# Lcrypto/mod-interleaveavx_multithreads-FAID

Hardware: AMD Instinct MI355X
Metric: decoded Gb/s @ 10 iters, 50G-PON LDPC; FER match vs AVX512 ref (higher is better)
Workload: dtype i8

## Files before the change

### include/lnsfaid.h

```cpp
#ifndef LNSFAID_H
#define LNSFAID_H

#include <stddef.h>
#include <stdint.h>

#ifdef __cplusplus
extern "C" {
#endif

#define LNSFAID_GROUP 32

#define LNSFAID_OK 0
#define LNSFAID_E_INVAL (-1)
#define LNSFAID_E_CODE (-2)
#define LNSFAID_E_NOMEM (-3)
#define LNSFAID_E_HIP (-4)
#define LNSFAID_E_NODEVICE (-5)
#define LNSFAID_E_INTERNAL (-6)

typedef struct lnsfaid_code {
    int32_t n_var;
    int32_t n_check;
    int32_t n_edges;
    int32_t z;
    int32_t puncture_tail;
    int32_t nb_degres;
    const int32_t* deg;
    const int32_t* deg_rows;
    const uint16_t* pos_vn;
} lnsfaid_code;

typedef struct lnsfaid_cfg {
    int32_t decode_method;
    int32_t max_iteration;
    int32_t factor_1;
    int32_t factor_2;
    int32_t floor_err_count;
    int32_t floor_iter_thresh;
    int32_t ef_elimination;
    int32_t max_bf_iter;
    int32_t bf_L0;
    int32_t bf_L1;
    int32_t bf_alpha;
    int32_t bf_delta;
    int32_t regular_col_weight;
    int32_t hard2_threshold;
    int32_t bf_vote_cap;
    int8_t v2c_map[6][4][8];
    int8_t v2c_map_ef[6][4][8];
} lnsfaid_cfg;

typedef struct lnsfaid_group_stats {
    int32_t iterations;
    int32_t bf_iterations;
} lnsfaid_group_stats;

typedef struct lnsfaid_codeword_stats {
    int32_t iterations;
    int32_t bf_iterations;
    int32_t unsatisfied;
} lnsfaid_codeword_stats;

typedef struct lnsfaid_ctx lnsfaid_ctx;


int lnsfaid_code_50gpon(lnsfaid_code* code, uint16_t* pos_vn, int32_t* deg3, int32_t* deg_rows3);

int lnsfaid_cfg_default(lnsfaid_cfg* cfg, int32_t decode_method, int32_t max_iteration);

#define LNSFAID_TABLES_FAID3 0
#define LNSFAID_TABLES_FAID32 1
#define LNSFAID_TABLES_FAID2 2
int lnsfaid_cfg_table_preset(lnsfaid_cfg* cfg, int32_t preset);

int lnsfaid_cfg_ef_elimination(lnsfaid_cfg* cfg, int32_t mode);


int lnsfaid_create(lnsfaid_ctx** ctx, const lnsfaid_code* code, const lnsfaid_cfg* cfg,
                   int32_t device, size_t max_groups);
void lnsfaid_destroy(lnsfaid_ctx* ctx);

int lnsfaid_set_cfg(lnsfaid_ctx* ctx, const lnsfaid_cfg* cfg);


int lnsfaid_decode(lnsfaid_ctx* ctx, const int8_t* fixInput, size_t n_groups,
                   int8_t* decodedBits, lnsfaid_group_stats* stats);

int lnsfaid_decode_device(lnsfaid_ctx* ctx, const int8_t* d_fixInput, size_t n_groups,
                          int8_t* d_decodedBits, lnsfaid_group_stats* d_stats);

#define LNSFAID_STOP_GROUP 0
#define LNSFAID_STOP_CODEWORD 1
int lnsfaid_set_early_stop(lnsfaid_ctx* ctx, int32_t rule);
int lnsfaid_early_stop(const lnsfaid_ctx* ctx);
int lnsfaid_decode_codewords(lnsfaid_ctx* ctx, const int8_t* fixInput, size_t n_groups, int8_t* decodedBits,
                             lnsfaid_codeword_stats* cw_stats);
int lnsfaid_decode_codewords_device(lnsfaid_ctx* ctx, const int8_t* d_fixInput, size_t n_groups, int8_t* d_decodedBits,
                                    lnsfaid_codeword_stats* d_cw_stats);

int lnsfaid_count_errors(lnsfaid_ctx* ctx, const int8_t* decodedBits, const int8_t* inputBits,
                         size_t n_groups, uint64_t out[4]);
int lnsfaid_count_errors_device(lnsfaid_ctx* ctx, const int8_t* d_decodedBits,
                                const int8_t* d_inputBits, size_t n_groups, uint64_t out[4]);

int lnsfaid_decode_packed(lnsfaid_ctx* ctx, const uint8_t* llr4, size_t n_groups, uint32_t* bits, lnsfaid_group_stats* stats);
int lnsfaid_decode_packed_device(lnsfaid_ctx* ctx, const uint8_t* d_llr4, size_t n_groups, uint32_t* d_bits,
                                 lnsfaid_group_stats* d_stats);
int lnsfaid_decode_codewords_packed(lnsfaid_ctx* ctx, const uint8_t* llr4, size_t n_groups, uint32_t* bits,
                                    lnsfaid_codeword_stats* cw_stats);
int lnsfaid_decode_codewords_packed_device(lnsfaid_ctx* ctx, const uint8_t* d_llr4, size_t n_groups, uint32_t* d_bits,
                                           lnsfaid_codeword_stats* d_cw_stats);
int lnsfaid_count_errors_packed(lnsfaid_ctx* ctx, const uint32_t* bits, const uint8_t* msg, size_t n_groups, uint64_t out[4]);
int lnsfaid_count_errors_packed_device(lnsfaid_ctx* ctx, const uint32_t* d_bits, const uint8_t* d_msg, size_t n_groups,
                                       uint64_t out[4]);
int lnsfaid_pack_llr4(const int8_t* fixInput, size_t n_values, uint8_t* llr4);
int lnsfaid_unpack_bits(const uint32_t* bits, size_t n_bits, int8_t* decodedBits);
int lnsfaid_pack_bits(const int8_t* inputBits, size_t n_bits, uint8_t* packed);


int lnsfaid_frontend_device(lnsfaid_ctx* ctx, const uint32_t* seeds, const uint64_t* draws_before, size_t n_streams,
                            int32_t mod_type, float sigma, float scale, const int8_t* codeword, int8_t* d_fixInput);
int lnsfaid_frontend_device_states(lnsfaid_ctx* ctx, const uint32_t* states, const uint64_t* draws_before, size_t n_streams,
                                   int32_t mod_type, float sigma, float scale, const int8_t* codeword, int8_t* d_fixInput);
uint64_t lnsfaid_frontend_draws_per_group(const lnsfaid_ctx* ctx, int32_t mod_type);

int lnsfaid_frontend_set_exact(lnsfaid_ctx* ctx, int32_t exact);
int lnsfaid_frontend_fastpath_bounds(lnsfaid_ctx* ctx, double measured[2], double assumed[2]);

int lnsfaid_frontend_set_interleave(lnsfaid_ctx* ctx, int32_t interleave_mod_type);

int lnsfaid_frontend_set_frames(lnsfaid_ctx* ctx, const int8_t* outputBits, const int8_t* inputBits, size_t n_streams);
int lnsfaid_frontend_input_bits(lnsfaid_ctx* ctx, const int8_t** d_inputBits);

int lnsfaid_demap_device(lnsfaid_ctx* ctx, const float* d_rx, size_t n_groups, int32_t mod_type, float scale, int8_t* d_fixInput);
int lnsfaid_demap_packed_device(lnsfaid_ctx* ctx, const float* d_rx, size_t n_groups, int32_t mod_type, float scale, uint8_t* d_llr4);
int lnsfaid_demap_host(int32_t n_var, int32_t n_check, int32_t interleave_mod_type, const float* rx, size_t n_groups,
                       int32_t mod_type, float scale, int8_t* fixInput);
int lnsfaid_demap_packed_host(int32_t n_var, int32_t n_check, int32_t interleave_mod_type, const float* rx, size_t n_groups,
                              int32_t mod_type, float scale, uint8_t* llr4);


int lnsfaid_code_parity_inverse(const lnsfaid_code* code, uint8_t* circ, size_t bytes);

int lnsfaid_encode_device(lnsfaid_ctx* ctx, const int8_t* d_inputBits, size_t n_groups, int8_t* d_outputBits);
int lnsfaid_encode(lnsfaid_ctx* ctx, const int8_t* inputBits, size_t n_groups, int8_t* outputBits);

int lnsfaid_frontend_random_frames(lnsfaid_ctx* ctx, const uint64_t* keys, size_t n_streams);

int lnsfaid_io_buffers(lnsfaid_ctx* ctx, int8_t** d_fixInput, int8_t** d_decodedBits, lnsfaid_group_stats** d_stats);

int lnsfaid_host_register(void* ptr, size_t bytes);
int lnsfaid_host_unregister(void* ptr);

int lnsfaid_read_stats(lnsfaid_ctx* ctx, lnsfaid_group_stats* stats, size_t n_groups);

#define LNSFAID_COMM_ID_BYTES 128
int lnsfaid_comm_unique_id(uint8_t id[LNSFAID_COMM_ID_BYTES]);
int lnsfaid_comm_init(lnsfaid_ctx* ctx, int32_t n_ranks, int32_t rank, const uint8_t id[LNSFAID_COMM_ID_BYTES]);
int lnsfaid_comm_attach(lnsfaid_ctx* ctx, void* nccl_comm);
int lnsfaid_comm_destroy(lnsfaid_ctx* ctx);
int lnsfaid_allreduce_counters(lnsfaid_ctx* ctx, uint64_t counters[4]);

int lnsfaid_select_kernel(lnsfaid_ctx* ctx, int32_t rows_per_lane);
int lnsfaid_kernel_rows_per_lane(const lnsfaid_ctx* ctx);

int lnsfaid_select_waves(lnsfaid_ctx* ctx, int32_t waves_per_codeword);
int lnsfaid_kernel_waves(const lnsfaid_ctx* ctx);

#define LNSFAID_MSG_REGISTERS 1
#define LNSFAID_MSG_HBM 2
int lnsfaid_select_message_store(lnsfaid_ctx* ctx, int32_t where);
int lnsfaid_message_store(const lnsfaid_ctx* ctx);

int lnsfaid_kernel_residency(lnsfaid_ctx* ctx, int32_t* workgroups_per_cu, int32_t* lds_limit);


int lnsfaid_kernel_time(lnsfaid_ctx* ctx, double* out_ms, uint64_t* out_launches, int32_t reset);

void* lnsfaid_stream(lnsfaid_ctx* ctx);

const char* lnsfaid_strerror(int err);
const char* lnsfaid_last_hip_error(void);
const char* lnsfaid_version(void);

#ifdef __cplusplus
}
#endif
#endif
```

### mod-interleaveavx_multithreads-faid_amd/csrc/lnsfaid_capi.hip

```cpp
#include <hip/hip_runtime.h>

#include <dlfcn.h>
#include <rccl/rccl.h>

#include <cstdio>
#include <cstdlib>
#include <cstring>
#include <new>
#include <vector>

#include "lnsfaid_device.h"
#include "lnsfaid_quantise.h"
#include "lnsfaid_swar.h"

extern "C" hipError_t lf_launch_decode(int method, int uniform_w, const LfKernelArgs* args, size_t lds_bytes,
                                       hipStream_t stream);
extern "C" const void* lf_decode_func(int method, int uniform_w);
extern "C" int lf_decode_threads(void);
extern "C" const void* lf_decode4_func(int method, int ef, int rm);
extern "C" int lf_decode4_threads(void);
extern "C" hipError_t lf_launch_decode4(int method, int ef, int rm, const LfKernelArgs* args, size_t lds_bytes, hipStream_t stream);
extern "C" int lf_decode4_rm_layers(void);
extern "C" const void* lf_decode4cw_func(int method, int ef, int rm);
extern "C" hipError_t lf_launch_decode4cw(int method, int ef, int rm, const LfCwArgs* args, size_t lds_bytes, hipStream_t stream);
extern "C" const void* lf_decode4p_func(int method, int ef, int rm, int per_codeword);
extern "C" hipError_t lf_launch_decode4p(int method, int ef, int rm, const LfKernelArgs* args, size_t lds_bytes, hipStream_t stream);
extern "C" hipError_t lf_launch_decode4pcw(int method, int ef, int rm, const LfCwArgs* args, size_t lds_bytes, hipStream_t stream);
extern "C" hipError_t lf_launch_unpack_llr4(const uint8_t* d_llr4, int8_t* d_fix, size_t n_values, hipStream_t stream);
extern "C" hipError_t lf_launch_pack_bits(const int8_t* d_decoded, uint32_t* d_bits, size_t n_values, hipStream_t stream);
extern "C" hipError_t lf_launch_count_errors_packed(const uint32_t* d_bits, const uint32_t* d_msg, int n_var, int k_info, size_t n_cw,
                                                    unsigned long long* out, hipStream_t stream);
extern "C" const void* lf_decode5_func(int method);
extern "C" int lf_decode5_threads(void);
extern "C" hipError_t lf_launch_decode5(int method, const LfKernelArgs* args, size_t lds_bytes, hipStream_t stream);
extern "C" hipError_t lf_launch_count_errors(const int8_t* decoded, const int8_t* input_bits, int n_var, int k_info,
                                             size_t n_cw, unsigned long long* out, hipStream_t stream);

extern "C" hipError_t lf_launch_frontend(const uint32_t* d_seeds, const unsigned long long* d_draws, int n_streams, int mod_type,
                                         float sigma_ch, float scale, const int8_t* d_codeword, const int8_t* d_frames, int n_var,
                                         int n_check, int interleave, int fast, int8_t* d_fix, hipStream_t stream);
extern "C" hipError_t lf_launch_demap(const float* d_rx, size_t n_groups, int mod_type, float scale, int n_var, int n_check,
                                      int interleave, int packed, void* d_out, hipStream_t stream);
extern "C" hipError_t lf_frontend_fastpath_scan(double* d_out2, hipStream_t stream);
extern "C" void lf_frontend_fastpath_assumed(double* eps2);
extern "C" hipError_t lf_launch_encode(const LfDevCode* d_code, int n_check, const uint32_t* d_bsup, const uint32_t* d_bsup_off,
                                       const int8_t* d_in, const unsigned long long* d_keys, size_t n_groups, int8_t* d_out,
                                       int8_t* d_info, hipStream_t stream);

#include <atomic>
#include <chrono>
#include <condition_variable>
#include <mutex>
#include <thread>
struct LfCombiner;
static thread_local char g_hip_err[256] = "";
static std::atomic<int> g_live_contexts(0);
#define LF_SPIN_CONTEXTS 4
static bool sync_blocking()
{
    static const char* e = getenv("LNSFAID_SYNC");
    if (e && e[0] == 's') return false;
    if (e && e[0] == 'b') return true;
    return g_live_contexts.load(std::memory_order_relaxed) > LF_SPIN_CONTEXTS;
}

static int hip_fail(hipError_t e, const char* what)
{
    snprintf(g_hip_err, sizeof(g_hip_err), "%s: %s", what, hipGetErrorString(e));
    return LNSFAID_E_HIP;
}
#define HIP_TRY(call)                                      \
    do {                                                   \
        hipError_t e_ = (call);                            \
        if (e_ != hipSuccess) return hip_fail(e_, #call);  \
    } while (0)

#define LF_IO_CHUNKS 8
#define LF_MAX_CHAIN 6

struct lnsfaid_ctx {
    int device = 0;
    size_t max_groups = 0;
    LfDevCode hcode;
    LfDevCfg hcfg;
    int n_var = 0, n_check = 0, k_info = 0;
    size_t lds_bytes = 0;
    hipStream_t stream = nullptr;
    hipEvent_t ev0 = nullptr, ev1 = nullptr;
    hipEvent_t ev_chain[LF_MAX_CHAIN + 1] = {};
    hipEvent_t ev_block = nullptr;
    uint32_t slot_seen[LF_MAX_CHAIN] = {};
    int predicted_launches = 1;
    hipStream_t s_in = nullptr, s_out = nullptr;
    hipEvent_t ev_in[LF_IO_CHUNKS] = {};
    LfDevCode* d_code = nullptr;
    LfDevCfg* d_cfg = nullptr;
    int8_t* d_en = nullptr;
    uint4* d_rows = nullptr;
    uint32_t* d_bits = nullptr;
    LfLaneState* d_lane = nullptr;
    int32_t* d_status[2] = { nullptr, nullptr };
    uint32_t* d_remaining = nullptr;
    int32_t* d_live = nullptr;
    unsigned long long* d_counters = nullptr;
    uint32_t* h_remaining = nullptr;
    unsigned long long* h_counters = nullptr;
    int8_t* d_io_in = nullptr;
    int8_t* d_io_out = nullptr;
    lnsfaid_group_stats* d_io_stats = nullptr;
    lnsfaid_codeword_stats* d_io_cw_stats = nullptr;
    uint8_t* d_pk_in = nullptr;
    uint32_t* d_pk_out = nullptr;
    lnsfaid_group_stats* d_pk_stats = nullptr;
    int early_stop = LNSFAID_STOP_GROUP;
    int rows_per_lane = 0;
    int waves_per_cw = 0;
    int msg_store = 0;
    struct LfCombiner* comb = nullptr;
    int comb_slot = -1;
    const void* checked_fn[4] = {};
    int resident_wg[4] = {}, lds_wg[4] = {};
    void* comm = nullptr;
    bool comm_owned = false;
    unsigned long long* d_reduce = nullptr;
    double kernel_ms = 0.0;
    uint64_t kernel_launches = 0;
    uint32_t* d_fe_seeds = nullptr;
    unsigned long long* d_fe_draws = nullptr;
    int8_t* d_fe_codeword = nullptr;
    int8_t* d_fe_frames = nullptr;
    int8_t* d_fe_input = nullptr;
    size_t fe_frames_streams = 0;
    int fe_interleave = 1;
    int fe_exact = 0;
    int enc_state = 0;
    uint32_t* d_enc_sup = nullptr;
    uint32_t* d_enc_off = nullptr;
    unsigned long long* d_fe_keys = nullptr;
};

static int stream_wait(lnsfaid_ctx* ctx)
{
    if (sync_blocking()) {
        HIP_TRY(hipEventRecord(ctx->ev_block, ctx->stream));
        HIP_TRY(hipEventSynchronize(ctx->ev_block));
    } else {
        HIP_TRY(hipStreamSynchronize(ctx->stream));
    }
    return LNSFAID_OK;
}

static int weight_class(int w) { return w == 3 ? 0 : (w == 6 ? 1 : (w == 11 ? 2 : 3)); }

static int build_code(const lnsfaid_code* code, LfDevCode* out)
{
    memset(out, 0, sizeof(*out));
    if (!code || !code->pos_vn || !code->deg || !code->deg_rows) return LNSFAID_E_INVAL;
    const int Z = code->z, N = code->n_var, M = code->n_check, E = code->n_edges;
    if (Z != LF_Z) return LNSFAID_E_CODE;
    if (N <= 0 || M <= 0 || N % Z || M % Z || M >= N) return LNSFAID_E_CODE;
    const int nbr = M / Z, nbc = N / Z, K = N - M;
    if (nbr > LF_MAX_BR || nbc > LF_MAX_BC) return LNSFAID_E_CODE;
    if (K % 4 || M % 4 || N % LF_T) return LNSFAID_E_CODE;
    if (code->puncture_tail < 0 || code->puncture_tail > N) return LNSFAID_E_CODE;
    std::vector<int> row_deg;
    row_deg.reserve(M);
    long e_total = 0;
    for (int k = 0; k < code->nb_degres; ++k) {
        if (code->deg_rows[k] < 0 || code->deg[k] < 2 || code->deg[k] > LF_MAX_DEG) return LNSFAID_E_CODE;
        for (int i = 0; i < code->deg_rows[k]; ++i) { row_deg.push_back(code->deg[k]); e_total += code->deg[k]; }
    }
    if ((int)row_deg.size() != M || e_total != E) return LNSFAID_E_CODE;

    size_t e = 0;
    for (int br = 0; br < nbr; ++br) {
        const int deg = row_deg[(size_t)br * Z];
        out->deg[br] = deg;
        const uint16_t* row0 = code->pos_vn + e;
        for (int j = 0; j < 64; ++j) out->sbtab[br][j] = 0u;
        for (int j = 0; j < 32; ++j) out->sbplain[br][j] = 0u;
        int prev_cb = -1;
        for (int j = 0; j < deg; ++j) {
            const int cb = row0[j] / Z, sh = row0[j] % Z;
            if (row0[j] >= N || cb <= prev_cb) return LNSFAID_E_CODE;
            prev_cb = cb;
            out->circ[br][j].sb = (uint32_t)cb * (uint32_t)Z + (uint32_t)sh;
            out->sbtab[br][LF_JCODE_A(j)] = out->sbtab[br][LF_JCODE_B(j)] = out->circ[br][j].sb;
            out->sbplain[br][j] = (((uint32_t)cb * (uint32_t)Z) << 16) | (((uint32_t)sh) << 2);
            out->s4tab[br][j] = ((uint32_t)sh) << 2;
            out->cbtab[br][j] = (uint32_t)cb * (uint32_t)Z;
            if (out->col_weight[cb] >= LF_MAX_COLW) return LNSFAID_E_CODE;
            out->colcirc[cb][out->col_weight[cb]++] = (uint32_t)br | ((uint32_t)sh << 8);
        }
        for (int i = 0; i < Z; ++i) {
            if (row_deg[(size_t)br * Z + i] != deg) return LNSFAID_E_CODE;
            for (int j = 0; j < deg; ++j) {
                const uint32_t sb = out->circ[br][j].sb;
                const int want = (int)(sb / (uint32_t)Z * (uint32_t)Z + (sb % (uint32_t)Z + (uint32_t)i) % (uint32_t)Z);
                if (code->pos_vn[e + (size_t)i * deg + j] != want) return LNSFAID_E_CODE;
            }
        }
        e += (size_t)deg * Z;
    }
    {
        const int nw = N / 32, pw = M / 32;
        const uint32_t hard0 = lf_lds_off_hard(N), zero = lf_lds_off_zero(N, nw, pw);
        if (lf_lds_bytes(N, nw, pw) > 0xffffu) return LNSFAID_E_CODE;
        for (int br = 0; br < LF_MAX_BR; ++br)
            for (int j = 0; j < LF_MAX_DEG; ++j)
                for (int k = 0; k < 8; ++k) {
                    uint2 e; e.x = zero | (zero << 16); e.y = 0;
                    if (br < nbr && j < out->deg[br]) {
                        const uint32_t sb = out->circ[br][j].sb, cb = sb / (uint32_t)Z, sh = sb % (uint32_t)Z;
                        const uint32_t o = (32u * (uint32_t)k + sh) & 255u, q = o >> 5;
                        e.x = (hard0 + 4u * (cb * 8u + q)) | ((hard0 + 4u * (cb * 8u + ((q + 1u) & 7u))) << 16);
                        e.y = o & 31u;
                    }
                    out->synw[br][j][k] = e;
                }
    }
    for (int br = 0; br < nbr; ++br)
        for (int j = 0; j < out->deg[br]; ++j)
            out->circ[br][j].wclass = (uint32_t)weight_class(out->col_weight[out->circ[br][j].sb / (uint32_t)Z]);
    out->n_var = N; out->n_check = M; out->k_info = K; out->nbr = nbr; out->nbc = nbc;
    out->puncture_tail = code->puncture_tail;
    out->n_words = N / 32; out->p_words = M / 32;
    return LNSFAID_OK;
}

static void build_wcols(LfDevCode* code, int W)
{
    code->n_wcols = 0;
    for (int cb = 0; cb < code->nbc; ++cb)
        if (code->col_weight[cb] == W) code->wcol[code->n_wcols++] = cb;
    bool seen[LF_MAX_BC] = {};
    for (int br = 0; br < LF_MAX_BR; ++br) {
        code->era_edges[br] = 0;
        for (int j = 0; br < code->nbr && j < code->deg[br]; ++j) {
            const int cb = (int)(code->circ[br][j].sb / LF_Z);
            if (code->col_weight[cb] == W && !seen[cb]) { seen[cb] = true; code->era_edges[br] |= 1u << j; }
        }
    }
}

static int build_cfg(const lnsfaid_cfg* cfg, LfDevCfg* out)
{
    if (!cfg) return LNSFAID_E_INVAL;
    if (cfg->decode_method < 0 || cfg->decode_method > 5) return LNSFAID_E_INVAL;
    if (cfg->max_iteration < 0 || cfg->max_iteration > (1 << 20)) return LNSFAID_E_INVAL;
    if (cfg->max_bf_iter < 0 || cfg->max_bf_iter > (1 << 20)) return LNSFAID_E_INVAL;
    if (cfg->regular_col_weight < 0 || cfg->regular_col_weight > LF_MAX_COLW) return LNSFAID_E_INVAL;
    memset(out, 0, sizeof(*out));
    out->method = cfg->decode_method;
    out->max_iter = cfg->max_iteration;
    out->factor_1 = cfg->decode_method == 0 ? (int16_t)cfg->factor_1 : (int8_t)cfg->factor_1;
    out->factor_2 = cfg->decode_method == 0 ? (int16_t)cfg->factor_2 : (int8_t)cfg->factor_2;
    out->floor_err_count = cfg->floor_err_count;
    out->floor_iter_thresh = cfg->floor_iter_thresh;
    out->ef = cfg->ef_elimination;
    out->max_bf = (cfg->decode_method == 0 || cfg->decode_method == 1) ? 0 : cfg->max_bf_iter;
    out->L0 = cfg->bf_L0; out->L1 = cfg->bf_L1; out->alpha = cfg->bf_alpha; out->delta = cfg->bf_delta;
    out->W = cfg->regular_col_weight;
    out->hard2_thr = cfg->hard2_threshold;
    out->vote_cap = (int8_t)cfg->bf_vote_cap;
    if ((cfg->decode_method == 1 || cfg->decode_method == 3 || cfg->decode_method == 4)
        && ((int8_t)cfg->factor_1 < 0 || (int8_t)cfg->factor_2 < 1)) return LNSFAID_E_INVAL;
    if (cfg->decode_method == 5 && cfg->ef_elimination != 1) return LNSFAID_E_INVAL;
    if (cfg->decode_method == 2 && (cfg->ef_elimination < 0 || cfg->ef_elimination > 2)) return LNSFAID_E_INVAL;
    if (cfg->decode_method != 2 && cfg->decode_method != 5 && cfg->ef_elimination != 0) return LNSFAID_E_INVAL;
    out->uniform_w = 1;
    for (int it = 0; it < 6; ++it)
        for (int w = 0; w < 4; ++w) {
            for (int a = 0; a < 8; ++a) {
                const int v = cfg->v2c_map[it][w][a], ve = cfg->v2c_map_ef[it][w][a];
                if ((cfg->decode_method == 2 || cfg->decode_method == 5) && (v < 0 || v > 7)) return LNSFAID_E_INVAL;
                if ((cfg->decode_method == 5 || cfg->ef_elimination >= 1) && (ve < 0 || ve > 7)) return LNSFAID_E_INVAL;
                uint32_t* l = a < 4 ? &out->lut_lo[it][w] : &out->lut_hi[it][w];
                uint32_t* le = a < 4 ? &out->lut_ef_lo[it][w] : &out->lut_ef_hi[it][w];
                *l |= (uint32_t)(v & 0xff) << (8 * (a & 3));
                *le |= (uint32_t)(ve & 0xff) << (8 * (a & 3));
                if (a > 0 && (v < cfg->v2c_map[it][w][a - 1] || ((cfg->decode_method == 5 || cfg->ef_elimination >= 1) && ve < cfg->v2c_map_ef[it][w][a - 1])))
                    out->uniform_w = 0;
            }
            if (out->lut_lo[it][w] != out->lut_lo[it][0] || out->lut_hi[it][w] != out->lut_hi[it][0]) out->uniform_w = 0;
            if ((cfg->decode_method == 5 || cfg->ef_elimination >= 1)
                && (out->lut_ef_lo[it][w] != out->lut_ef_lo[it][0] || out->lut_ef_hi[it][w] != out->lut_ef_hi[it][0]))
                out->uniform_w = 0;
        }
    if (cfg->decode_method == 0) {
        out->uniform_w = (out->factor_1 == out->factor_2) ? 1 : 0;
        out->nms_fits = sw_nms_fits(out->factor_1, out->factor_2) ? 1 : 0;
        if (out->nms_fits) sw_nms_tables(out->factor_1, out->nms_t);
    }
    if (cfg->decode_method == 2 && cfg->ef_elimination >= 1 && !out->uniform_w) return LNSFAID_E_INVAL;
    out->bf_fast = (out->W == 3 && ((int8_t)out->alpha == 0 || (int8_t)out->alpha == 1)) ? 1 : 0;
    return LNSFAID_OK;
}

static int check_code_for_method(const LfDevCode* code, int method)
{
    if (method == 3)
        for (int cb = 0; cb < code->nbc; ++cb)
            if (code->col_weight[cb] > 15) return LNSFAID_E_CODE;
    return LNSFAID_OK;
}

extern "C" int lnsfaid_comm_destroy(lnsfaid_ctx* ctx);
static int comb_join(lnsfaid_ctx* ctx);
static void comb_leave(lnsfaid_ctx* ctx, int slot);
extern "C" void lnsfaid_destroy(lnsfaid_ctx* ctx)
{
    if (!ctx) return;
    if (ctx->comb_slot >= 0) { comb_leave(ctx, ctx->comb_slot); ctx->comb_slot = -1; }
    g_live_contexts.fetch_sub(1, std::memory_order_relaxed);
    (void)hipSetDevice(ctx->device);
    if (ctx->stream) (void)hipStreamSynchronize(ctx->stream);
    (void)lnsfaid_comm_destroy(ctx);
    (void)hipFree(ctx->d_reduce);
    (void)hipFree(ctx->d_code); (void)hipFree(ctx->d_cfg); (void)hipFree(ctx->d_en); (void)hipFree(ctx->d_rows);
    (void)hipFree(ctx->d_bits); (void)hipFree(ctx->d_lane); (void)hipFree(ctx->d_status[0]); (void)hipFree(ctx->d_status[1]);
    (void)hipFree(ctx->d_remaining); (void)hipFree(ctx->d_live); (void)hipFree(ctx->d_counters);
    (void)hipFree(ctx->d_io_in); (void)hipFree(ctx->d_io_out); (void)hipFree(ctx->d_io_stats);
    (void)hipFree(ctx->d_io_cw_stats);
    (void)hipFree(ctx->d_pk_in); (void)hipFree(ctx->d_pk_out); (void)hipFree(ctx->d_pk_stats);
    (void)hipFree(ctx->d_fe_seeds); (void)hipFree(ctx->d_fe_draws); (void)hipFree(ctx->d_fe_codeword);
    (void)hipFree(ctx->d_fe_frames); (void)hipFree(ctx->d_fe_input);
    (void)hipFree(ctx->d_enc_sup); (void)hipFree(ctx->d_enc_off); (void)hipFree(ctx->d_fe_keys);
    if (ctx->h_remaining) (void)hipHostFree(ctx->h_remaining);
    if (ctx->h_counters) (void)hipHostFree(ctx->h_counters);
    if (ctx->ev0) (void)hipEventDestroy(ctx->ev0);
    if (ctx->ev1) (void)hipEventDestroy(ctx->ev1);
    for (auto e : ctx->ev_chain) if (e) (void)hipEventDestroy(e);
    if (ctx->ev_block) (void)hipEventDestroy(ctx->ev_block);
    if (ctx->stream) (void)hipStreamDestroy(ctx->stream);
    if (ctx->s_in) (void)hipStreamDestroy(ctx->s_in);
    if (ctx->s_out) (void)hipStreamDestroy(ctx->s_out);
    for (auto e : ctx->ev_in) if (e) (void)hipEventDestroy(e);
    delete ctx;
}

static int alloc_state(lnsfaid_ctx* ctx);
static int create_impl(lnsfaid_ctx* ctx, const lnsfaid_code* code, const lnsfaid_cfg* cfg)
{
    int rc = build_code(code, &ctx->hcode);
    if (rc) return rc;
    rc = build_cfg(cfg, &ctx->hcfg);
    if (rc) return rc;
    ctx->n_var = ctx->hcode.n_var; ctx->n_check = ctx->hcode.n_check; ctx->k_info = ctx->hcode.k_info;
    rc = check_code_for_method(&ctx->hcode, ctx->hcfg.method);
    if (rc) return rc;
    build_wcols(&ctx->hcode, ctx->hcfg.W);
    return alloc_state(ctx);
}

static int alloc_state(lnsfaid_ctx* ctx)
{
    ctx->n_var = ctx->hcode.n_var; ctx->n_check = ctx->hcode.n_check; ctx->k_info = ctx->hcode.k_info;
    ctx->lds_bytes = lf_lds_bytes(ctx->n_var, ctx->hcode.n_words, ctx->hcode.p_words);
    if (ctx->lds_bytes > 64 * 1024) return LNSFAID_E_CODE;

    int ndev = 0;
    if (hipGetDeviceCount(&ndev) != hipSuccess || ndev <= 0 || ctx->device < 0 || ctx->device >= ndev) {
        snprintf(g_hip_err, sizeof(g_hip_err), "no usable HIP device (count %d, asked for %d)", ndev, ctx->device);
        return LNSFAID_E_NODEVICE;
    }
    HIP_TRY(hipSetDevice(ctx->device));
    HIP_TRY(hipStreamCreateWithFlags(&ctx->stream, hipStreamNonBlocking));
    HIP_TRY(hipEventCreate(&ctx->ev0));
    HIP_TRY(hipEventCreate(&ctx->ev1));
    const size_t n_cw = ctx->max_groups * LNSFAID_GROUP;
    HIP_TRY(hipMalloc(&ctx->d_code, sizeof(LfDevCode)));
    HIP_TRY(hipMalloc(&ctx->d_cfg, sizeof(LfDevCfg)));
    HIP_TRY(hipMalloc(&ctx->d_en, n_cw * (size_t)ctx->n_var));
    HIP_TRY(hipMalloc(&ctx->d_rows, n_cw * (size_t)ctx->hcode.nbr * LF_T * sizeof(uint4)));
    HIP_TRY(hipMalloc(&ctx->d_bits, n_cw * (size_t)3 * ctx->hcode.n_words * sizeof(uint32_t)));
    HIP_TRY(hipMalloc(&ctx->d_lane, n_cw * sizeof(LfLaneState)));
    HIP_TRY(hipMalloc(&ctx->d_status[0], n_cw * sizeof(int32_t)));
    HIP_TRY(hipMalloc(&ctx->d_status[1], n_cw * sizeof(int32_t)));
    HIP_TRY(hipMalloc(&ctx->d_remaining, LF_MAX_CHAIN * sizeof(uint32_t)));
    HIP_TRY(hipMemset(ctx->d_remaining, 0, LF_MAX_CHAIN * sizeof(uint32_t)));
    for (auto& e : ctx->ev_chain) HIP_TRY(hipEventCreate(&e));
    HIP_TRY(hipEventCreateWithFlags(&ctx->ev_block, hipEventBlockingSync | hipEventDisableTiming));
    HIP_TRY(hipMalloc(&ctx->d_live, n_cw * sizeof(int32_t)));
    HIP_TRY(hipMalloc(&ctx->d_counters, 4 * sizeof(unsigned long long)));
    HIP_TRY(hipHostMalloc((void**)&ctx->h_remaining, LF_MAX_CHAIN * sizeof(uint32_t), hipHostMallocDefault));
    HIP_TRY(hipHostMalloc((void**)&ctx->h_counters, 4 * sizeof(unsigned long long), hipHostMallocDefault));
    HIP_TRY(hipMemcpy(ctx->d_code, &ctx->hcode, sizeof(LfDevCode), hipMemcpyHostToDevice));
    HIP_TRY(hipMemcpy(ctx->d_cfg, &ctx->hcfg, sizeof(LfDevCfg), hipMemcpyHostToDevice));
    return LNSFAID_OK;
}

extern "C" int lnsfaid_create(lnsfaid_ctx** out, const lnsfaid_code* code, const lnsfaid_cfg* cfg, int32_t device,
                              size_t max_groups)
{
    if (!out || !code || !cfg || max_groups == 0 || max_groups > ((size_t)1 << 24)) return LNSFAID_E_INVAL;
    *out = nullptr;
    lnsfaid_ctx* ctx = new (std::nothrow) lnsfaid_ctx();
    if (!ctx) return LNSFAID_E_NOMEM;
    ctx->device = device;
    ctx->max_groups = max_groups;
    if (const char* e = getenv("LNSFAID_ROWS_PER_LANE"))
        ctx->rows_per_lane = (e[0] == '2') ? 2 : 0;
    if (const char* e = getenv("LNSFAID_WAVES_PER_CODEWORD"))
        ctx->waves_per_cw = (e[0] == '2') ? 2 : 0;
    if (const char* e = getenv("LNSFAID_FRONTEND_EXACT"))
        ctx->fe_exact = (e[0] == '1') ? 1 : 0;
    if (const char* e = getenv("LNSFAID_MSG_STORE"))
        ctx->msg_store = (e[0] == 'h') ? LNSFAID_MSG_HBM : ((e[0] == 'r') ? LNSFAID_MSG_REGISTERS : 0);
    g_live_contexts.fetch_add(1, std::memory_order_relaxed);
    const int rc = create_impl(ctx, code, cfg);
    if (rc) { lnsfaid_destroy(ctx); return rc; }
    ctx->comb_slot = comb_join(ctx);
    *out = ctx;
    return LNSFAID_OK;
}

extern "C" int lnsfaid_set_cfg(lnsfaid_ctx* ctx, const lnsfaid_cfg* cfg)
{
    if (!ctx || !cfg) return LNSFAID_E_INVAL;
    LfDevCfg n;
    int rc = build_cfg(cfg, &n);
    if (rc) return rc;
    rc = check_code_for_method(&ctx->hcode, n.method);
    if (rc) return rc;
    if (memcmp(&n, &ctx->hcfg, sizeof(n)) == 0) return LNSFAID_OK;
    HIP_TRY(hipSetDevice(ctx->device));
    HIP_TRY(hipStreamSynchronize(ctx->stream));
    if (n.W != ctx->hcfg.W) {
        build_wcols(&ctx->hcode, n.W);
        HIP_TRY(hipMemcpy(ctx->d_code, &ctx->hcode, sizeof(LfDevCode), hipMemcpyHostToDevice));
    }
    ctx->hcfg = n;
    HIP_TRY(hipMemcpy(ctx->d_cfg, &ctx->hcfg, sizeof(LfDevCfg), hipMemcpyHostToDevice));
    return LNSFAID_OK;
}

static void apply_devcfg(lnsfaid_ctx* ctx, const LfDevCfg& n)
{
    (void)hipStreamSynchronize(ctx->stream);
    ctx->hcfg = n;
    (void)hipMemcpy(ctx->d_cfg, &ctx->hcfg, sizeof(LfDevCfg), hipMemcpyHostToDevice);
}

static bool kernel4_possible(const lnsfaid_ctx* ctx)
{
    const int m = ctx->hcfg.method;
    if (m < 0 || m > 5) return false;
    if (m == 0) return ctx->hcfg.nms_fits != 0;
    if ((m == 2 || m == 5) && !ctx->hcfg.uniform_w) return false;
    return true;
}
static bool use_kernel4(const lnsfaid_ctx* ctx)
{
    if (ctx->hcfg.method == 2 && ctx->hcfg.ef >= 1) return true;
    if (ctx->rows_per_lane == 2) return false;
    return kernel4_possible(ctx);
}

extern "C" int lnsfaid_select_kernel(lnsfaid_ctx* ctx, int32_t rows_per_lane)
{
    if (!ctx || (rows_per_lane != 0 && rows_per_lane != 2 && rows_per_lane != 4)) return LNSFAID_E_INVAL;
    if (rows_per_lane == 4 && !kernel4_possible(ctx)) return LNSFAID_E_INVAL;
    if (rows_per_lane == 2 && ctx->hcfg.method == 2 && ctx->hcfg.ef >= 1) return LNSFAID_E_INVAL;
    ctx->rows_per_lane = rows_per_lane;
    return LNSFAID_OK;
}

extern "C" int lnsfaid_kernel_rows_per_lane(const lnsfaid_ctx* ctx) { return ctx ? (use_kernel4(ctx) ? 4 : 2) : LNSFAID_E_INVAL; }

static bool kernel5_possible(const lnsfaid_ctx* ctx)
{
    const int m = ctx->hcfg.method;
    return kernel4_possible(ctx) && m >= 1 && m <= 5 && !(m == 2 && ctx->hcfg.ef == 2) && ctx->hcode.n_words >= 7 * 64;
}
static bool use_kernel5(const lnsfaid_ctx* ctx) { return ctx->waves_per_cw == 2 && use_kernel4(ctx) && kernel5_possible(ctx); }

extern "C" int lnsfaid_select_waves(lnsfaid_ctx* ctx, int32_t waves_per_codeword)
{
    if (!ctx || waves_per_codeword < 0 || waves_per_codeword > 2) return LNSFAID_E_INVAL;
    if (waves_per_codeword == 2 && !(use_kernel4(ctx) && kernel5_possible(ctx))) return LNSFAID_E_INVAL;
    ctx->waves_per_cw = waves_per_codeword;
    return LNSFAID_OK;
}

extern "C" int lnsfaid_kernel_waves(const lnsfaid_ctx* ctx) { return ctx ? (use_kernel5(ctx) ? 2 : 1) : LNSFAID_E_INVAL; }

static bool msg_registers_possible(const lnsfaid_ctx* ctx)
{
    if (ctx->hcfg.method == 0) return false;
    return ctx->hcode.nbr <= lf_decode4_rm_layers() && !(ctx->hcfg.method == 2 && ctx->hcfg.ef == 2);
}
static bool use_msg_registers(const lnsfaid_ctx* ctx)
{
    if (!msg_registers_possible(ctx) || use_kernel5(ctx)) return false;
    return ctx->msg_store != LNSFAID_MSG_HBM;
}

static bool cw_possible(const lnsfaid_ctx* ctx) { return ctx->waves_per_cw != 2 && use_kernel4(ctx); }

static bool packed_kernel(const lnsfaid_ctx* ctx) { return use_kernel4(ctx) && !use_kernel5(ctx); }

static const void* selected_kernel(const lnsfaid_ctx* ctx, int* threads, int rule, bool packed = false)
{
    if (packed) {
        *threads = lf_decode4_threads();
        return lf_decode4p_func(ctx->hcfg.method, ctx->hcfg.ef, use_msg_registers(ctx) ? 1 : 0, rule == LNSFAID_STOP_CODEWORD ? 1 : 0);
    }
    if (rule == LNSFAID_STOP_CODEWORD) {
        *threads = lf_decode4_threads();
        return cw_possible(ctx) ? lf_decode4cw_func(ctx->hcfg.method, ctx->hcfg.ef, use_msg_registers(ctx) ? 1 : 0) : nullptr;
    }
    if (use_kernel5(ctx)) {
        *threads = lf_decode5_threads();
        return lf_decode5_func(ctx->hcfg.method);
    }
    if (use_kernel4(ctx)) {
        *threads = lf_decode4_threads();
        return lf_decode4_func(ctx->hcfg.method, ctx->hcfg.ef, use_msg_registers(ctx) ? 1 : 0);
    }
    *threads = lf_decode_threads();
    return lf_decode_func(ctx->hcfg.method, ctx->hcfg.uniform_w);
}

extern "C" int lnsfaid_select_message_store(lnsfaid_ctx* ctx, int32_t where)
{
    if (!ctx || where < 0 || where > LNSFAID_MSG_HBM) return LNSFAID_E_INVAL;
    if (where == LNSFAID_MSG_REGISTERS && !msg_registers_possible(ctx)) return LNSFAID_E_INVAL;
    ctx->msg_store = where;
    return LNSFAID_OK;
}

extern "C" int lnsfaid_message_store(const lnsfaid_ctx* ctx)
{
    if (!ctx) return LNSFAID_E_INVAL;
    if (!use_kernel4(ctx)) return LNSFAID_MSG_HBM;
    return use_msg_registers(ctx) ? LNSFAID_MSG_REGISTERS : LNSFAID_MSG_HBM;
}

static int kernel_check(lnsfaid_ctx* ctx, int rule, bool packed = false)
{
    int threads = 0;
    const void* fn = selected_kernel(ctx, &threads, rule, packed);
    if (!fn) return rule == LNSFAID_STOP_CODEWORD ? LNSFAID_E_INVAL : LNSFAID_E_INTERNAL;
    const int slot = rule + (packed ? 2 : 0);
    if (fn == ctx->checked_fn[slot]) return LNSFAID_OK;
    hipFuncAttributes at;
    HIP_TRY(hipFuncGetAttributes(&at, fn));
    if (at.sharedSizeBytes != 0) {
        snprintf(g_hip_err, sizeof(g_hip_err), "decode kernel has %zu bytes of static LDS: its En image would not start at LDS offset 0",
                 (size_t)at.sharedSizeBytes);
        return LNSFAID_E_INTERNAL;
    }
    int wg = 0;
    HIP_TRY(hipOccupancyMaxActiveBlocksPerMultiprocessor(&wg, fn, threads, ctx->lds_bytes));
    hipDeviceProp_t prop;
    HIP_TRY(hipGetDeviceProperties(&prop, ctx->device));
    const size_t lds_cu = prop.maxSharedMemoryPerMultiProcessor ? prop.maxSharedMemoryPerMultiProcessor : 160 * 1024;
    const size_t gran = 512;
    int by_lds = (int)(lds_cu / ((ctx->lds_bytes + gran - 1) / gran * gran));
    const int by_waves = 32 / ((threads + 63) / 64);
    if (by_lds > by_waves) by_lds = by_waves;
    ctx->checked_fn[slot] = fn; ctx->resident_wg[slot] = wg; ctx->lds_wg[slot] = by_lds;
    static const bool trace = getenv("LNSFAID_TRACE") != nullptr;
    if (trace)
        fprintf(stderr, "[lnsfaid] decode kernel: %d threads, %d VGPRs, %zu B LDS per workgroup, %d workgroups per CU (LDS alone: %d)%s\n",
                threads, at.numRegs, ctx->lds_bytes, wg, by_lds, wg < by_lds ? "  ** residency lost **" : "");
    return LNSFAID_OK;
}

extern "C" int lnsfaid_kernel_residency(lnsfaid_ctx* ctx, int32_t* workgroups_per_cu, int32_t* lds_limit)
{
    if (!ctx) return LNSFAID_E_INVAL;
    HIP_TRY(hipSetDevice(ctx->device));
    const int rc = kernel_check(ctx, ctx->early_stop);
    if (rc) return rc;
    if (workgroups_per_cu) *workgroups_per_cu = ctx->resident_wg[ctx->early_stop];
    if (lds_limit) *lds_limit = ctx->lds_wg[ctx->early_stop];
    return LNSFAID_OK;
}

static int decode_device_impl(lnsfaid_ctx* ctx, const int8_t* d_fixInput, size_t n_groups, int8_t* d_decodedBits,
                              lnsfaid_group_stats* d_stats, bool status_preloaded, bool packed = false);
static int decode_cw_device_impl(lnsfaid_ctx* ctx, const int8_t* d_fixInput, size_t n_groups, int8_t* d_decodedBits,
                                 lnsfaid_group_stats* d_stats, lnsfaid_codeword_stats* d_cw_stats, bool status_preloaded,
                                 bool packed = false);
static int decode_device_rule(lnsfaid_ctx* ctx, const int8_t* d_fixInput, size_t n_groups, int8_t* d_decodedBits, lnsfaid_group_stats* d_stats,
                              lnsfaid_codeword_stats* d_cw_stats, int rule, bool status_preloaded)
{
    if (rule == LNSFAID_STOP_CODEWORD)
        return decode_cw_device_impl(ctx, d_fixInput, n_groups, d_decodedBits, d_stats, d_cw_stats, status_preloaded);
    return decode_device_impl(ctx, d_fixInput, n_groups, d_decodedBits, d_stats, status_preloaded);
}
extern "C" int lnsfaid_decode_device(lnsfaid_ctx* ctx, const int8_t* d_fixInput, size_t n_groups, int8_t* d_decodedBits,
                                     lnsfaid_group_stats* d_stats)
{
    if (!ctx) return LNSFAID_E_INVAL;
    return decode_device_rule(ctx, d_fixInput, n_groups, d_decodedBits, d_stats, nullptr, ctx->early_stop, false);
}
extern "C" int lnsfaid_decode_codewords_device(lnsfaid_ctx* ctx, const int8_t* d_fixInput, size_t n_groups, int8_t* d_decodedBits,
                                               lnsfaid_codeword_stats* d_cw_stats)
{
    return decode_cw_device_impl(ctx, d_fixInput, n_groups, d_decodedBits, nullptr, d_cw_stats, false);
}

extern "C" int lnsfaid_set_early_stop(lnsfaid_ctx* ctx, int32_t rule)
{
    if (!ctx || (rule != LNSFAID_STOP_GROUP && rule != LNSFAID_STOP_CODEWORD)) return LNSFAID_E_INVAL;
    ctx->early_stop = rule;
    return LNSFAID_OK;
}
extern "C" int lnsfaid_early_stop(const lnsfaid_ctx* ctx) { return ctx ? ctx->early_stop : LNSFAID_E_INVAL; }

static int decode_cw_device_impl(lnsfaid_ctx* ctx, const int8_t* d_fixInput, size_t n_groups, int8_t* d_decodedBits,
                                 lnsfaid_group_stats* d_stats, lnsfaid_codeword_stats* d_cw_stats, bool status_preloaded, bool packed)
{
    if (!ctx || (n_groups && (!d_fixInput || !d_decodedBits))) return LNSFAID_E_INVAL;
    if (n_groups > ctx->max_groups) return LNSFAID_E_INVAL;
    if (!cw_possible(ctx)) return LNSFAID_E_INVAL;
    if (n_groups == 0) return LNSFAID_OK;
    HIP_TRY(hipSetDevice(ctx->device));
    {
        const int rc = kernel_check(ctx, LNSFAID_STOP_CODEWORD, packed);
        if (rc) return rc;
    }
    const size_t n_cw = n_groups * LNSFAID_GROUP;
    LfCwArgs a;
    a.code = ctx->d_code; a.cfg = ctx->d_cfg;
    a.fix_input = d_fixInput; a.decoded = d_decodedBits;
    a.st_rows = ctx->d_rows;
    a.skip = status_preloaded ? ctx->d_status[0] : nullptr;
    a.stats = d_stats; a.cw_stats = d_cw_stats; a.n_cw = (int32_t)n_cw;
    if (d_stats) HIP_TRY(hipMemsetAsync(d_stats, 0, n_groups * sizeof(lnsfaid_group_stats), ctx->stream));
    static const bool trace = getenv("LNSFAID_TRACE") != nullptr;
    HIP_TRY(hipEventRecord(ctx->ev_chain[0], ctx->stream));
    if (packed) HIP_TRY(lf_launch_decode4pcw(ctx->hcfg.method, ctx->hcfg.ef, use_msg_registers(ctx) ? 1 : 0, &a, ctx->lds_bytes, ctx->stream));
    else HIP_TRY(lf_launch_decode4cw(ctx->hcfg.method, ctx->hcfg.ef, use_msg_registers(ctx) ? 1 : 0, &a, ctx->lds_bytes, ctx->stream));
    HIP_TRY(hipEventRecord(ctx->ev_chain[1], ctx->stream));
    { const int rcw = stream_wait(ctx); if (rcw) return rcw; }
    float ms = 0.f;
    HIP_TRY(hipEventElapsedTime(&ms, ctx->ev_chain[0], ctx->ev_chain[1]));
    ctx->kernel_ms += ms;
    ctx->kernel_launches += 1;
    if (trace) fprintf(stderr, "[lnsfaid] per-codeword launch: %.3f ms, %zu codewords\n", ms, n_cw);
    return LNSFAID_OK;
}

static int decode_device_impl(lnsfaid_ctx* ctx, const int8_t* d_fixInput, size_t n_groups, int8_t* d_decodedBits,
                              lnsfaid_group_stats* d_stats, bool status_preloaded, bool packed)
{
    if (!ctx || (n_groups && (!d_fixInput || !d_decodedBits))) return LNSFAID_E_INVAL;
    if (n_groups > ctx->max_groups) return LNSFAID_E_INVAL;
    if (n_groups == 0) return LNSFAID_OK;
    HIP_TRY(hipSetDevice(ctx->device));
    {
        const int rc = kernel_check(ctx, LNSFAID_STOP_GROUP, packed);
        if (rc) return rc;
    }
    const size_t n_cw = n_groups * LNSFAID_GROUP;
#ifdef LF4_LIVE_PROOF
    HIP_TRY(hipMemsetAsync(ctx->d_live, 0, n_cw * sizeof(int32_t), ctx->stream));
#endif

    LfKernelArgs a;
    a.code = ctx->d_code; a.cfg = ctx->d_cfg;
    a.fix_input = d_fixInput; a.decoded = d_decodedBits;
    a.st_en = ctx->d_en; a.st_rows = ctx->d_rows; a.st_bits = ctx->d_bits; a.st_lane = ctx->d_lane;
    a.live = ctx->d_live; a.stats = d_stats; a.n_cw = (int32_t)n_cw;

    const long max_launches = 2L * ((long)ctx->hcfg.max_iter + ctx->hcfg.max_bf + 2) + 2 + LF_MAX_CHAIN;
    static const bool trace = getenv("LNSFAID_TRACE") != nullptr;
    int cur = 0;
    long launch = 0, needed = 0;
    bool done = false;
    while (!done) {
        if (launch >= max_launches) return LNSFAID_E_INTERNAL;
        int chain = launch == 0 ? ctx->predicted_launches : 1;
        if (chain < 1) chain = 1;
        if (chain > LF_MAX_CHAIN) chain = LF_MAX_CHAIN;
        for (int j = 0; j < chain; ++j) {
            a.status_cur = (launch + j == 0 && !status_preloaded) ? nullptr : ctx->d_status[cur];
            a.status_next = ctx->d_status[cur ^ 1];
            a.remaining = ctx->d_remaining + j;
            HIP_TRY(hipEventRecord(ctx->ev_chain[j], ctx->stream));
            if (packed) HIP_TRY(lf_launch_decode4p(ctx->hcfg.method, ctx->hcfg.ef, use_msg_registers(ctx) ? 1 : 0, &a, ctx->lds_bytes, ctx->stream));
            else if (use_kernel5(ctx)) HIP_TRY(lf_launch_decode5(ctx->hcfg.method, &a, ctx->lds_bytes, ctx->stream));
            else if (use_kernel4(ctx)) HIP_TRY(lf_launch_decode4(ctx->hcfg.method, ctx->hcfg.ef, use_msg_registers(ctx) ? 1 : 0, &a, ctx->lds_bytes, ctx->stream));
            else HIP_TRY(lf_launch_decode(ctx->hcfg.method, ctx->hcfg.uniform_w, &a, ctx->lds_bytes, ctx->stream));
            cur ^= 1;
        }
        HIP_TRY(hipEventRecord(ctx->ev_chain[chain], ctx->stream));
        HIP_TRY(hipMemcpyAsync(ctx->h_remaining, ctx->d_remaining, (size_t)chain * sizeof(uint32_t), hipMemcpyDeviceToHost, ctx->stream));
        { const int rcw = stream_wait(ctx); if (rcw) return rcw; }
        for (int j = 0; j < chain; ++j) {
            const uint32_t left = ctx->h_remaining[j] - ctx->slot_seen[j];
            ctx->slot_seen[j] = ctx->h_remaining[j];
            float ms = 0.f;
            HIP_TRY(hipEventElapsedTime(&ms, ctx->ev_chain[j], ctx->ev_chain[j + 1]));
            ctx->kernel_ms += ms;
            ctx->kernel_launches += 1;
            if (trace) fprintf(stderr, "[lnsfaid] launch %ld: %.3f ms, %u codewords left%s\n", launch + j, ms, left, done ? " (queued ahead, batch already complete)" : "");
            if (!done && left == 0) { done = true; needed = launch + j + 1; }
        }
        launch += chain;
    }
    ctx->predicted_launches = (int)needed;
    return LNSFAID_OK;
}

static int ensure_io(lnsfaid_ctx* ctx)
{
    if (ctx->d_io_in) return LNSFAID_OK;
    const size_t bytes = ctx->max_groups * LNSFAID_GROUP * (size_t)ctx->n_var;
    HIP_TRY(hipMalloc(&ctx->d_io_in, bytes));
    HIP_TRY(hipMalloc(&ctx->d_io_out, bytes));
    HIP_TRY(hipMalloc(&ctx->d_io_stats, ctx->max_groups * sizeof(lnsfaid_group_stats)));
    return LNSFAID_OK;
}

#define LF_COMB_SLOTS 128
#define LF_COMB_QUIET_US 150
#define LF_COMB_WINDOW_US 1500
#define LF_COMB_DEVICES 16
#define LF_COMB_WORKERS 4
#define LF_COMB_MIN_MEMBERS 4
enum { LF_SLOT_FREE = 0, LF_SLOT_IDLE, LF_SLOT_PENDING, LF_SLOT_RUNNING, LF_SLOT_DONE };
struct LfSlot {
    int state = LF_SLOT_FREE;
    int rc = 0;
    LfDevCfg cfg;
    int rule = LNSFAID_STOP_GROUP;
    lnsfaid_group_stats stats;
};
struct LfCombiner {
    int device = 0;
    std::mutex m;
    std::condition_variable cv_work, cv_done;
    std::thread worker[LF_COMB_WORKERS];
    bool stop = false, dead = false;
    bool gathering = false;
    int running = 0;
    lnsfaid_ctx* pool[LF_COMB_WORKERS] = {};
    LfDevCode code;
    size_t group_bytes = 0;
    int8_t *h_in = nullptr, *h_out = nullptr;
    int8_t *d_in_map = nullptr, *d_out_map = nullptr;
    int32_t* h_status = nullptr;
    lnsfaid_group_stats* h_stats = nullptr;
    LfSlot slots[LF_COMB_SLOTS];
    int members = 0, pending = 0;
    char err[256] = "";
    uint64_t batches = 0, calls = 0;
    double gather_ms = 0, device_ms = 0;
};
static std::mutex g_comb_mutex;
static LfCombiner* g_comb[LF_COMB_DEVICES] = {};

static int comb_workers()
{
    static const int n = [] {
        const char* e = getenv("LNSFAID_COMB_WORKERS");
        const int v = e ? atoi(e) : 2;
        return v < 1 ? 1 : (v > LF_COMB_WORKERS ? LF_COMB_WORKERS : v);
    }();
    return n;
}

static int comb_batches()
{
    static const int v = [] {
        const char* e = getenv("LNSFAID_COMB_BATCHES");
        const int n = e ? atoi(e) : 0;
        return n > 64 ? 64 : n;
    }();
    return v > comb_workers() ? v : comb_workers();
}

static bool comb_enabled()
{
    static const char* e = getenv("LNSFAID_COALESCE");
    return !(e && e[0] == '0');
}

static void apply_devcfg(lnsfaid_ctx* ctx, const LfDevCfg& n);

static void comb_run_batch(LfCombiner* cb, int w, const int* batch, int nb)
{
    lnsfaid_ctx* P = cb->pool[w];
    int32_t* h_status = cb->h_status + (size_t)w * LF_COMB_SLOTS * LNSFAID_GROUP;
    lnsfaid_group_stats* h_stats = cb->h_stats + (size_t)w * LF_COMB_SLOTS;
    int rc = LNSFAID_OK;
    auto fail = [&](hipError_t e, const char* what) { if (rc == LNSFAID_OK && e != hipSuccess) rc = hip_fail(e, what); };
    int lo = LF_COMB_SLOTS, hi = -1;
    for (int i = 0; i < nb; ++i) { lo = batch[i] < lo ? batch[i] : lo; hi = batch[i] > hi ? batch[i] : hi; }
    const size_t n = (size_t)hi + 1;
    for (size_t g = 0; g < n; ++g) {
        bool active = false;
        for (int i = 0; i < nb; ++i) active = active || (size_t)batch[i] == g;
        for (int l = 0; l < LNSFAID_GROUP; ++l) h_status[g * LNSFAID_GROUP + l] = active ? 0 : LF_DONE;
    }
    fail(hipSetDevice(cb->device), "hipSetDevice");
    if (rc == LNSFAID_OK && memcmp(&P->hcfg, &cb->slots[batch[0]].cfg, sizeof(LfDevCfg)) != 0) apply_devcfg(P, cb->slots[batch[0]].cfg);
    const size_t gb = cb->group_bytes, span = (size_t)(hi - lo + 1);
    fail(hipMemcpyAsync(P->d_status[0], h_status, n * LNSFAID_GROUP * sizeof(int32_t), hipMemcpyHostToDevice, P->stream), "status upload");
    static const bool copy_mode = getenv("LNSFAID_COMB_COPY") != nullptr;
    const int8_t* k_in = cb->d_in_map;
    int8_t* k_out = cb->d_out_map;
    if (copy_mode || !k_in || !k_out) {
        fail(hipMemcpyAsync(P->d_io_in + (size_t)lo * gb, cb->h_in + (size_t)lo * gb, span * gb, hipMemcpyHostToDevice, P->stream), "fixInput upload");
        k_in = P->d_io_in; k_out = P->d_io_out;
    }
    if (rc == LNSFAID_OK) rc = decode_device_rule(P, k_in, n, k_out, P->d_io_stats, nullptr, cb->slots[batch[0]].rule, true);
    if (rc == LNSFAID_OK) {
        if (k_out == P->d_io_out)
            fail(hipMemcpyAsync(cb->h_out + (size_t)lo * gb, P->d_io_out + (size_t)lo * gb, span * gb, hipMemcpyDeviceToHost, P->stream), "decodedBits download");
        fail(hipMemcpyAsync(h_stats + lo, P->d_io_stats + lo, span * sizeof(lnsfaid_group_stats), hipMemcpyDeviceToHost, P->stream), "stats download");
        if (rc == LNSFAID_OK) rc = stream_wait(P);
    }
    std::lock_guard<std::mutex> lk(cb->m);
    if (rc != LNSFAID_OK) snprintf(cb->err, sizeof(cb->err), "%s", g_hip_err);
    for (int i = 0; i < nb; ++i) {
        LfSlot& s = cb->slots[batch[i]];
        s.rc = rc;
        s.stats = h_stats[batch[i]];
        s.state = LF_SLOT_DONE;
    }
    cb->running -= nb;
    cb->batches += 1; cb->calls += (uint64_t)nb;
    cb->cv_done.notify_all();
    cb->cv_work.notify_all();
}

static void comb_worker(LfCombiner* cb, int w)
{
    std::unique_lock<std::mutex> lk(cb->m);
    for (;;) {
        cb->cv_work.wait(lk, [&] { return cb->stop || (cb->pending > 0 && !cb->gathering); });
        if (cb->stop) break;
        cb->gathering = true;
        const auto t_first = std::chrono::steady_clock::now();
        const auto deadline = t_first + std::chrono::microseconds(LF_COMB_WINDOW_US);
        for (;;) {
            const int share = (cb->members + comb_batches() - 1) / comb_batches();
            if (cb->stop || cb->pending >= share || cb->pending + cb->running >= cb->members) break;
            const int seen = cb->pending, seen_running = cb->running;
            auto quiet = std::chrono::steady_clock::now() + std::chrono::microseconds(LF_COMB_QUIET_US);
            if (quiet > deadline) quiet = deadline;
            cb->cv_work.wait_until(lk, quiet, [&] { return cb->pending != seen || cb->running != seen_running || cb->stop; });
            if (cb->pending == seen && cb->running == seen_running) break;
        }
        if (cb->stop) { cb->gathering = false; break; }
        cb->gather_ms += std::chrono::duration<double, std::milli>(std::chrono::steady_clock::now() - t_first).count();
        int batch[LF_COMB_SLOTS], nb = 0;
        const int cap = cb->members > 8 * comb_workers() ? (cb->members + comb_batches() - 1) / comb_batches() : LF_COMB_SLOTS;
        const LfDevCfg* cfg = nullptr;
        int rule = LNSFAID_STOP_GROUP;
        for (int i = 0; i < LF_COMB_SLOTS && nb < cap; ++i) {
            LfSlot& s = cb->slots[i];
            if (s.state != LF_SLOT_PENDING) continue;
            if (!cfg) { cfg = &s.cfg; rule = s.rule; }
            if (memcmp(cfg, &s.cfg, sizeof(LfDevCfg)) != 0 || s.rule != rule) continue;
            s.state = LF_SLOT_RUNNING;
            batch[nb++] = i;
        }
        cb->pending -= nb;
        cb->running += nb;
        cb->gathering = false;
        cb->cv_work.notify_all();
        if (nb == 0) continue;
        if (!cb->pool[w]) {
            lk.unlock();
            int rc = LNSFAID_OK;
            lnsfaid_ctx* P = new (std::nothrow) lnsfaid_ctx();
            if (!P) rc = LNSFAID_E_NOMEM;
            if (!rc) {
                P->device = cb->device; P->max_groups = LF_COMB_SLOTS;
                P->hcode = cb->code; P->hcfg = cb->slots[batch[0]].cfg;
                g_live_contexts.fetch_add(1, std::memory_order_relaxed);
                rc = alloc_state(P);
                if (!rc) rc = ensure_io(P);
                if (rc) { lnsfaid_destroy(P); P = nullptr; }
            }
            lk.lock();
            if (rc) {
                cb->dead = true;
                for (int i = 0; i < nb; ++i) { cb->slots[batch[i]].rc = rc; cb->slots[batch[i]].state = LF_SLOT_DONE; }
                cb->running -= nb;
                cb->cv_done.notify_all();
                continue;
            }
            cb->pool[w] = P;
        }
        lk.unlock();
        const auto t_dev = std::chrono::steady_clock::now();
        comb_run_batch(cb, w, batch, nb);
        lk.lock();
        cb->device_ms += std::chrono::duration<double, std::milli>(std::chrono::steady_clock::now() - t_dev).count();
    }
}

static int comb_join(lnsfaid_ctx* ctx)
{
    if (!comb_enabled() || ctx->max_groups != 1 || ctx->device < 0 || ctx->device >= LF_COMB_DEVICES) return -1;
    std::lock_guard<std::mutex> g(g_comb_mutex);
    LfCombiner* cb = g_comb[ctx->device];
    if (!cb) {
        cb = new (std::nothrow) LfCombiner();
        if (!cb) return -1;
        cb->device = ctx->device;
        cb->code = ctx->hcode;
        cb->group_bytes = (size_t)LNSFAID_GROUP * (size_t)ctx->n_var;
        g_comb[ctx->device] = cb;
    }
    std::lock_guard<std::mutex> lk(cb->m);
    if (cb->dead || memcmp(&cb->code, &ctx->hcode, sizeof(LfDevCode)) != 0) return -1;
    if (cb->members >= 1 && !cb->h_in) {
        const size_t bytes = (size_t)LF_COMB_SLOTS * cb->group_bytes;
        if (hipSetDevice(cb->device) != hipSuccess
            || hipHostMalloc((void**)&cb->h_in, bytes, hipHostMallocMapped) != hipSuccess
            || hipHostMalloc((void**)&cb->h_out, bytes, hipHostMallocMapped) != hipSuccess
            || hipHostMalloc((void**)&cb->h_status, (size_t)LF_COMB_WORKERS * LF_COMB_SLOTS * LNSFAID_GROUP * sizeof(int32_t), hipHostMallocDefault) != hipSuccess
            || hipHostMalloc((void**)&cb->h_stats, (size_t)LF_COMB_WORKERS * LF_COMB_SLOTS * sizeof(lnsfaid_group_stats), hipHostMallocDefault) != hipSuccess) {
            (void)hipGetLastError();
            if (cb->h_in) (void)hipHostFree(cb->h_in);
            if (cb->h_out) (void)hipHostFree(cb->h_out);
            if (cb->h_status) (void)hipHostFree(cb->h_status);
            if (cb->h_stats) (void)hipHostFree(cb->h_stats);
            cb->h_in = cb->h_out = nullptr; cb->h_status = nullptr; cb->h_stats = nullptr;
            cb->dead = true;
            return -1;
        }
        if (hipHostGetDevicePointer((void**)&cb->d_in_map, cb->h_in, 0) != hipSuccess
            || hipHostGetDevicePointer((void**)&cb->d_out_map, cb->h_out, 0) != hipSuccess) {
            (void)hipGetLastError();
            cb->d_in_map = cb->d_out_map = nullptr;
        }
        for (int w = 0; w < comb_workers(); ++w) cb->worker[w] = std::thread(comb_worker, cb, w);
    }
    for (int i = 0; i < LF_COMB_SLOTS; ++i)
        if (cb->slots[i].state == LF_SLOT_FREE) { cb->slots[i].state = LF_SLOT_IDLE; cb->members += 1; ctx->comb = cb; return i; }
    return -1;
}

static void comb_leave(lnsfaid_ctx* ctx, int slot)
{
    LfCombiner* cb = nullptr;
    {
        std::lock_guard<std::mutex> g(g_comb_mutex);
        cb = ctx->comb;
        if (!cb) return;
        bool last;
        {
            std::lock_guard<std::mutex> lk(cb->m);
            cb->slots[slot].state = LF_SLOT_FREE;
            cb->members -= 1;
            last = cb->members == 0;
            if (last) cb->stop = true;
            cb->cv_work.notify_all();
        }
        if (!last) return;
        if (g_comb[cb->device] == cb) g_comb[cb->device] = nullptr;
    }
    for (auto& th : cb->worker) if (th.joinable()) th.join();
    static const bool trace = getenv("LNSFAID_TRACE") != nullptr;
    if (trace && cb->batches)
        fprintf(stderr, "[lnsfaid] call combiner of device %d: %llu calls in %llu batches (%.1f per batch); per batch %.3f ms gathering, %.3f ms copies + decode\n",
                cb->device, (unsigned long long)cb->calls, (unsigned long long)cb->batches, (double)cb->calls / (double)cb->batches,
                cb->gather_ms / (double)cb->batches, cb->device_ms / (double)cb->batches);
    for (auto P : cb->pool) if (P) lnsfaid_destroy(P);
    if (cb->h_in) { (void)hipHostFree(cb->h_in); (void)hipHostFree(cb->h_out); (void)hipHostFree(cb->h_status); (void)hipHostFree(cb->h_stats); }
    delete cb;
}

static int comb_decode(lnsfaid_ctx* ctx, const int8_t* fixInput, int8_t* decodedBits, lnsfaid_group_stats* stats, int rule, int* rc_out)
{
    if (ctx->comb_slot < 0 || ctx->rows_per_lane != 0 || ctx->msg_store != 0 || ctx->waves_per_cw != 0) return 0;
    LfCombiner* cb = ctx->comb;
    const int slot = ctx->comb_slot;
    {
        std::lock_guard<std::mutex> lk(cb->m);
        if (cb->dead || cb->members < LF_COMB_MIN_MEMBERS || !cb->h_in) return 0;
        if (memcmp(&cb->code, &ctx->hcode, sizeof(LfDevCode)) != 0) return 0;
    }
    memcpy(cb->h_in + (size_t)slot * cb->group_bytes, fixInput, cb->group_bytes);
    int rc;
    {
        std::unique_lock<std::mutex> lk(cb->m);
        LfSlot& s = cb->slots[slot];
        s.cfg = ctx->hcfg;
        s.rule = rule;
        s.state = LF_SLOT_PENDING;
        cb->pending += 1;
        cb->cv_work.notify_all();
        if (!cb->cv_done.wait_for(lk, std::chrono::seconds(120), [&] { return s.state == LF_SLOT_DONE; })) {
            snprintf(g_hip_err, sizeof(g_hip_err), "call combiner: no result after 120 s");
            *rc_out = LNSFAID_E_INTERNAL;
            return 1;
        }
        rc = s.rc;
        if (rc != LNSFAID_OK) snprintf(g_hip_err, sizeof(g_hip_err), "%s", cb->err);
        if (stats) *stats = s.stats;
        s.state = LF_SLOT_IDLE;
    }
    if (rc == LNSFAID_OK) memcpy(decodedBits, cb->h_out + (size_t)slot * cb->group_bytes, cb->group_bytes);
    *rc_out = rc;
    return 1;
}


extern "C" int lnsfaid_frontend_set_interleave(lnsfaid_ctx* ctx, int32_t interleave_mod_type)
{
    if (!ctx || interleave_mod_type < 1 || ctx->n_var % interleave_mod_type != 0) return LNSFAID_E_INVAL;
    ctx->fe_interleave = interleave_mod_type;
    return LNSFAID_OK;
}

static int alloc_fe_frames(lnsfaid_ctx* ctx)
{
    if (!ctx->d_fe_frames) {
        HIP_TRY(hipMalloc(&ctx->d_fe_frames, ctx->max_groups * LNSFAID_GROUP * (size_t)ctx->n_var));
        HIP_TRY(hipMalloc(&ctx->d_fe_input, ctx->max_groups * LNSFAID_GROUP * (size_t)ctx->k_info));
    }
    return LNSFAID_OK;
}

extern "C" int lnsfaid_frontend_set_frames(lnsfaid_ctx* ctx, const int8_t* outputBits, const int8_t* inputBits, size_t n_streams)
{
    if (!ctx || n_streams > ctx->max_groups) return LNSFAID_E_INVAL;
    if (!outputBits || n_streams == 0) { ctx->fe_frames_streams = 0; return LNSFAID_OK; }
    if (!inputBits) return LNSFAID_E_INVAL;
    HIP_TRY(hipSetDevice(ctx->device));
    { const int rc = alloc_fe_frames(ctx); if (rc) return rc; }
    HIP_TRY(hipMemcpyAsync(ctx->d_fe_frames, outputBits, n_streams * LNSFAID_GROUP * (size_t)ctx->n_var, hipMemcpyHostToDevice, ctx->stream));
    HIP_TRY(hipMemcpyAsync(ctx->d_fe_input, inputBits, n_streams * LNSFAID_GROUP * (size_t)ctx->k_info, hipMemcpyHostToDevice, ctx->stream));
    HIP_TRY(hipStreamSynchronize(ctx->stream));
    ctx->fe_frames_streams = n_streams;
    return LNSFAID_OK;
}

extern "C" int lnsfaid_frontend_input_bits(lnsfaid_ctx* ctx, const int8_t** d_inputBits)
{
    if (!ctx || !d_inputBits) return LNSFAID_E_INVAL;
    *d_inputBits = ctx->fe_frames_streams ? ctx->d_fe_input : nullptr;
    return LNSFAID_OK;
}

extern "C" int lnsfaid_io_buffers(lnsfaid_ctx* ctx, int8_t** d_fixInput, int8_t** d_decodedBits, lnsfaid_group_stats** d_stats)
{
    if (!ctx) return LNSFAID_E_INVAL;
    HIP_TRY(hipSetDevice(ctx->device));
    const int rc = ensure_io(ctx);
    if (rc) return rc;
    if (d_fixInput) *d_fixInput = ctx->d_io_in;
    if (d_decodedBits) *d_decodedBits = ctx->d_io_out;
    if (d_stats) *d_stats = ctx->d_io_stats;
    return LNSFAID_OK;
}

extern "C" int lnsfaid_read_stats(lnsfaid_ctx* ctx, lnsfaid_group_stats* stats, size_t n_groups)
{
    if (!ctx || (n_groups && !stats) || n_groups > ctx->max_groups) return LNSFAID_E_INVAL;
    if (n_groups == 0) return LNSFAID_OK;
    HIP_TRY(hipSetDevice(ctx->device));
    const int rc = ensure_io(ctx);
    if (rc) return rc;
    HIP_TRY(hipMemcpyAsync(stats, ctx->d_io_stats, n_groups * sizeof(lnsfaid_group_stats), hipMemcpyDeviceToHost, ctx->stream));
    HIP_TRY(hipStreamSynchronize(ctx->stream));
    return LNSFAID_OK;
}

static bool host_pinned(const void* p)
{
    hipPointerAttribute_t at;
    if (hipPointerGetAttributes(&at, p) != hipSuccess) { (void)hipGetLastError(); return false; }
    return at.type == hipMemoryTypeHost;
}

static int decode_host_impl(lnsfaid_ctx* ctx, const int8_t* fixInput, size_t n_groups, int8_t* decodedBits, lnsfaid_group_stats* stats,
                            lnsfaid_codeword_stats* cw_stats, int rule)
{
    if (!ctx || (n_groups && (!fixInput || !decodedBits))) return LNSFAID_E_INVAL;
    if (n_groups > ctx->max_groups) return LNSFAID_E_INVAL;
    if (rule == LNSFAID_STOP_CODEWORD && !cw_possible(ctx)) return LNSFAID_E_INVAL;
    if (n_groups == 0) return LNSFAID_OK;
    if (!cw_stats) {
        int rcc = 0;
        if (comb_decode(ctx, fixInput, decodedBits, stats, rule, &rcc)) return rcc;
    }
    HIP_TRY(hipSetDevice(ctx->device));
    int rc = ensure_io(ctx);
    if (rc) return rc;
    if (cw_stats && !ctx->d_io_cw_stats)
        HIP_TRY(hipMalloc(&ctx->d_io_cw_stats, ctx->max_groups * LNSFAID_GROUP * sizeof(lnsfaid_codeword_stats)));
    lnsfaid_codeword_stats* d_cw = cw_stats ? ctx->d_io_cw_stats : nullptr;
    const size_t group_bytes = LNSFAID_GROUP * (size_t)ctx->n_var;
    const size_t bytes = n_groups * group_bytes;
    size_t chunk = ((n_groups + LF_IO_CHUNKS - 1) / LF_IO_CHUNKS + 63) / 64 * 64;
    if (chunk >= n_groups || !host_pinned(fixInput) || !host_pinned(decodedBits)) {
        HIP_TRY(hipMemcpyAsync(ctx->d_io_in, fixInput, bytes, hipMemcpyHostToDevice, ctx->stream));
        rc = decode_device_rule(ctx, ctx->d_io_in, n_groups, ctx->d_io_out, ctx->d_io_stats, d_cw, rule, false);
        if (rc) return rc;
        HIP_TRY(hipMemcpyAsync(decodedBits, ctx->d_io_out, bytes, hipMemcpyDeviceToHost, ctx->stream));
    } else {
        if (!ctx->s_in) {
            HIP_TRY(hipStreamCreateWithFlags(&ctx->s_in, hipStreamNonBlocking));
            HIP_TRY(hipStreamCreateWithFlags(&ctx->s_out, hipStreamNonBlocking));
            for (auto& e : ctx->ev_in) HIP_TRY(hipEventCreateWithFlags(&e, hipEventDisableTiming));
        }
        const size_t n_chunks = (n_groups + chunk - 1) / chunk;
        for (size_t c = 0; c < n_chunks; ++c) {
            const size_t g0 = c * chunk, ng = g0 + chunk <= n_groups ? chunk : n_groups - g0;
            HIP_TRY(hipMemcpyAsync(ctx->d_io_in + g0 * group_bytes, fixInput + g0 * group_bytes, ng * group_bytes, hipMemcpyHostToDevice, ctx->s_in));
            HIP_TRY(hipEventRecord(ctx->ev_in[c], ctx->s_in));
        }
        for (size_t c = 0; c < n_chunks; ++c) {
            const size_t g0 = c * chunk, ng = g0 + chunk <= n_groups ? chunk : n_groups - g0;
            HIP_TRY(hipStreamWaitEvent(ctx->stream, ctx->ev_in[c], 0));
            rc = decode_device_rule(ctx, ctx->d_io_in + g0 * group_bytes, ng, ctx->d_io_out + g0 * group_bytes, ctx->d_io_stats + g0,
                                    d_cw ? d_cw + g0 * LNSFAID_GROUP : nullptr, rule, false);
            if (rc) { (void)hipStreamSynchronize(ctx->s_in); (void)hipStreamSynchronize(ctx->s_out); return rc; }
            HIP_TRY(hipMemcpyAsync(decodedBits + g0 * group_bytes, ctx->d_io_out + g0 * group_bytes, ng * group_bytes, hipMemcpyDeviceToHost, ctx->s_out));
        }
        HIP_TRY(hipStreamSynchronize(ctx->s_out));
    }
    if (stats)
        HIP_TRY(hipMemcpyAsync(stats, ctx->d_io_stats, n_groups * sizeof(lnsfaid_group_stats), hipMemcpyDeviceToHost,
                               ctx->stream));
    if (cw_stats)
        HIP_TRY(hipMemcpyAsync(cw_stats, d_cw, n_groups * LNSFAID_GROUP * sizeof(lnsfaid_codeword_stats), hipMemcpyDeviceToHost,
                               ctx->stream));
    { const int rcw = stream_wait(ctx); if (rcw) return rcw; }
    return LNSFAID_OK;
}

extern "C" int lnsfaid_decode(lnsfaid_ctx* ctx, const int8_t* fixInput, size_t n_groups, int8_t* decodedBits,
                              lnsfaid_group_stats* stats)
{
    if (!ctx) return LNSFAID_E_INVAL;
    return decode_host_impl(ctx, fixInput, n_groups, decodedBits, stats, nullptr, ctx->early_stop);
}

extern "C" int lnsfaid_decode_codewords(lnsfaid_ctx* ctx, const int8_t* fixInput, size_t n_groups, int8_t* decodedBits,
                                        lnsfaid_codeword_stats* cw_stats)
{
    return decode_host_impl(ctx, fixInput, n_groups, decodedBits, nullptr, cw_stats, LNSFAID_STOP_CODEWORD);
}

extern "C" int lnsfaid_host_register(void* ptr, size_t bytes)
{
    if (!ptr || !bytes) return LNSFAID_E_INVAL;
    HIP_TRY(hipHostRegister(ptr, bytes, hipHostRegisterPortable));
    return LNSFAID_OK;
}

extern "C" int lnsfaid_host_unregister(void* ptr)
{
    if (!ptr) return LNSFAID_E_INVAL;
    HIP_TRY(hipHostUnregister(ptr));
    return LNSFAID_OK;
}

extern "C" int lnsfaid_count_errors_device(lnsfaid_ctx* ctx, const int8_t* d_decodedBits, const int8_t* d_inputBits,
                                           size_t n_groups, uint64_t out[4])
{
    if (!ctx || !out || (n_groups && !d_decodedBits)) return LNSFAID_E_INVAL;
    if (n_groups == 0) return LNSFAID_OK;
    HIP_TRY(hipSetDevice(ctx->device));
    HIP_TRY(hipMemsetAsync(ctx->d_counters, 0, 4 * sizeof(unsigned long long), ctx->stream));
    HIP_TRY(lf_launch_count_errors(d_decodedBits, d_inputBits, ctx->n_var, ctx->k_info, n_groups * LNSFAID_GROUP,
                                   ctx->d_counters, ctx->stream));
    HIP_TRY(hipMemcpyAsync(ctx->h_counters, ctx->d_counters, 4 * sizeof(unsigned long long), hipMemcpyDeviceToHost,
                           ctx->stream));
    { const int rcw = stream_wait(ctx); if (rcw) return rcw; }
    for (int i = 0; i < 4; ++i) out[i] += ctx->h_counters[i];
    return LNSFAID_OK;
}

extern "C" int lnsfaid_count_errors(lnsfaid_ctx* ctx, const int8_t* decodedBits, const int8_t* inputBits, size_t n_groups,
                                    uint64_t out[4])
{
    if (!ctx || !out || (n_groups && !decodedBits)) return LNSFAID_E_INVAL;
    if (n_groups > ctx->max_groups) return LNSFAID_E_INVAL;
    if (n_groups == 0) return LNSFAID_OK;
    HIP_TRY(hipSetDevice(ctx->device));
    int rc = ensure_io(ctx);
    if (rc) return rc;
    const size_t n_cw = n_groups * LNSFAID_GROUP;
    HIP_TRY(hipMemcpyAsync(ctx->d_io_out, decodedBits, n_cw * (size_t)ctx->n_var, hipMemcpyHostToDevice, ctx->stream));
    const int8_t* d_in = nullptr;
    if (inputBits) {
        HIP_TRY(hipMemcpyAsync(ctx->d_io_in, inputBits, n_cw * (size_t)ctx->k_info, hipMemcpyHostToDevice, ctx->stream));
        d_in = ctx->d_io_in;
    }
    return lnsfaid_count_errors_device(ctx, ctx->d_io_out, d_in, n_groups, out);
}

static bool dword_aligned(const void* p) { return ((uintptr_t)p & 3u) == 0u; }

static int ensure_packed_io(lnsfaid_ctx* ctx)
{
    if (ctx->d_pk_in) return LNSFAID_OK;
    HIP_TRY(hipMalloc(&ctx->d_pk_in, ctx->max_groups * LNSFAID_GROUP * (size_t)ctx->n_var / 2));
    HIP_TRY(hipMalloc(&ctx->d_pk_out, ctx->max_groups * LNSFAID_GROUP * (size_t)ctx->n_var / 8));
    HIP_TRY(hipMalloc(&ctx->d_pk_stats, ctx->max_groups * sizeof(lnsfaid_group_stats)));
    return LNSFAID_OK;
}

static int decode_packed_rule(lnsfaid_ctx* ctx, const uint8_t* d_llr4, size_t n_groups, uint32_t* d_bits, lnsfaid_group_stats* d_stats,
                              lnsfaid_codeword_stats* d_cw_stats, int rule)
{
    if (rule == LNSFAID_STOP_CODEWORD)
        return decode_cw_device_impl(ctx, (const int8_t*)d_llr4, n_groups, (int8_t*)d_bits, d_stats, d_cw_stats, false, true);
    if (packed_kernel(ctx)) return decode_device_impl(ctx, (const int8_t*)d_llr4, n_groups, (int8_t*)d_bits, d_stats, false, true);
    int rc = ensure_io(ctx);
    if (rc) return rc;
    const size_t n_values = n_groups * LNSFAID_GROUP * (size_t)ctx->n_var;
    HIP_TRY(lf_launch_unpack_llr4(d_llr4, ctx->d_io_in, n_values, ctx->stream));
    rc = decode_device_impl(ctx, ctx->d_io_in, n_groups, ctx->d_io_out, d_stats, false);
    if (rc) return rc;
    HIP_TRY(lf_launch_pack_bits(ctx->d_io_out, d_bits, n_values, ctx->stream));
    return stream_wait(ctx);
}

static int decode_packed_device_impl(lnsfaid_ctx* ctx, const uint8_t* d_llr4, size_t n_groups, uint32_t* d_bits, lnsfaid_group_stats* d_stats,
                                     lnsfaid_codeword_stats* d_cw_stats, int rule)
{
    if (!ctx || (n_groups && (!d_llr4 || !d_bits))) return LNSFAID_E_INVAL;
    if (n_groups > ctx->max_groups) return LNSFAID_E_INVAL;
    if (rule == LNSFAID_STOP_CODEWORD && !cw_possible(ctx)) return LNSFAID_E_INVAL;
    if (n_groups == 0) return LNSFAID_OK;
    if (!dword_aligned(d_llr4) || !dword_aligned(d_bits) || !dword_aligned(d_stats) || !dword_aligned(d_cw_stats)) return LNSFAID_E_INVAL;
    HIP_TRY(hipSetDevice(ctx->device));
    return decode_packed_rule(ctx, d_llr4, n_groups, d_bits, d_stats, d_cw_stats, rule);
}

extern "C" int lnsfaid_decode_packed_device(lnsfaid_ctx* ctx, const uint8_t* d_llr4, size_t n_groups, uint32_t* d_bits,
                                            lnsfaid_group_stats* d_stats)
{
    if (!ctx) return LNSFAID_E_INVAL;
    return decode_packed_device_impl(ctx, d_llr4, n_groups, d_bits, d_stats, nullptr, ctx->early_stop);
}

extern "C" int lnsfaid_decode_codewords_packed_device(lnsfaid_ctx* ctx, const uint8_t* d_llr4, size_t n_groups, uint32_t* d_bits,
                                                      lnsfaid_codeword_stats* d_cw_stats)
{
    return decode_packed_device_impl(ctx, d_llr4, n_groups, d_bits, nullptr, d_cw_stats, LNSFAID_STOP_CODEWORD);
}

static int decode_packed_host_impl(lnsfaid_ctx* ctx, const uint8_t* llr4, size_t n_groups, uint32_t* bits, lnsfaid_group_stats* stats,
                                   lnsfaid_codeword_stats* cw_stats, int rule)
{
    if (!ctx || (n_groups && (!llr4 || !bits))) return LNSFAID_E_INVAL;
    if (n_groups > ctx->max_groups) return LNSFAID_E_INVAL;
    if (rule == LNSFAID_STOP_CODEWORD && !cw_possible(ctx)) return LNSFAID_E_INVAL;
    if (n_groups == 0) return LNSFAID_OK;
    HIP_TRY(hipSetDevice(ctx->device));
    int rc = ensure_packed_io(ctx);
    if (rc) return rc;
    if (cw_stats && !ctx->d_io_cw_stats)
        HIP_TRY(hipMalloc(&ctx->d_io_cw_stats, ctx->max_groups * LNSFAID_GROUP * sizeof(lnsfaid_codeword_stats)));
    lnsfaid_codeword_stats* d_cw = cw_stats ? ctx->d_io_cw_stats : nullptr;
    const size_t in_bytes = LNSFAID_GROUP * (size_t)ctx->n_var / 2, out_words = LNSFAID_GROUP * (size_t)ctx->n_var / 32;
    size_t chunk = ((n_groups + LF_IO_CHUNKS - 1) / LF_IO_CHUNKS + 63) / 64 * 64;
    if (chunk >= n_groups || !host_pinned(llr4) || !host_pinned(bits)) {
        HIP_TRY(hipMemcpyAsync(ctx->d_pk_in, llr4, n_groups * in_bytes, hipMemcpyHostToDevice, ctx->stream));
        rc = decode_packed_rule(ctx, ctx->d_pk_in, n_groups, ctx->d_pk_out, ctx->d_pk_stats, d_cw, rule);
        if (rc) return rc;
        HIP_TRY(hipMemcpyAsync(bits, ctx->d_pk_out, n_groups * out_words * sizeof(uint32_t), hipMemcpyDeviceToHost, ctx->stream));
    } else {
        if (!ctx->s_in) {
            HIP_TRY(hipStreamCreateWithFlags(&ctx->s_in, hipStreamNonBlocking));
            HIP_TRY(hipStreamCreateWithFlags(&ctx->s_out, hipStreamNonBlocking));
            for (auto& e : ctx->ev_in) HIP_TRY(hipEventCreateWithFlags(&e, hipEventDisableTiming));
        }
        const size_t n_chunks = (n_groups + chunk - 1) / chunk;
        for (size_t c = 0; c < n_chunks; ++c) {
            const size_t g0 = c * chunk, ng = g0 + chunk <= n_groups ? chunk : n_groups - g0;
            HIP_TRY(hipMemcpyAsync(ctx->d_pk_in + g0 * in_bytes, llr4 + g0 * in_bytes, ng * in_bytes, hipMemcpyHostToDevice, ctx->s_in));
            HIP_TRY(hipEventRecord(ctx->ev_in[c], ctx->s_in));
// ... 550 lines not shown
```

### mod-interleaveavx_multithreads-faid_amd/csrc/lnsfaid_device.h

```cpp
#ifndef LNSFAID_DEVICE_H
#define LNSFAID_DEVICE_H

#include <stdint.h>

#include "lnsfaid.h"

#define LF_Z 256
#define LF_T 128
#define LF_MAX_BR 32
#define LF_MAX_DEG 24
#define LF_MAX_BC 256
#define LF_MAX_COLW 16

#define LF_DONE 0x40000000
#define LF_PROG_MASK 0x0fffffff

#define LF_JCODE_A(j) ((j) < 16 ? (j) : (j) + 16)
#define LF_JCODE_B(j) ((j) < 16 ? (j) + 16 : (j) + 32)

struct LfCirc {
    uint32_t sb;
    uint32_t wclass;
};

struct LfDevCode {
    int32_t n_var, n_check, k_info, nbr, nbc, puncture_tail, n_words , p_words ;
    int32_t n_wcols;
    int32_t deg[LF_MAX_BR];
    LfCirc circ[LF_MAX_BR][LF_MAX_DEG];
    uint32_t sbtab[LF_MAX_BR][64];
    uint32_t sbplain[LF_MAX_BR][32];
    uint32_t s4tab[LF_MAX_BR][LF_MAX_DEG];
    uint32_t cbtab[LF_MAX_BR][LF_MAX_DEG];
    uint2 synw[LF_MAX_BR][LF_MAX_DEG][8];
    int32_t col_weight[LF_MAX_BC];
    int32_t wcol[LF_MAX_BC];
    uint32_t era_edges[LF_MAX_BR];
    uint32_t colcirc[LF_MAX_BC][LF_MAX_COLW];
};

struct LfDevCfg {
    int32_t method, max_iter, factor_1, factor_2, floor_err_count, floor_iter_thresh, ef, max_bf;
    int32_t L0, L1, alpha, delta, W, hard2_thr, vote_cap;
    int32_t uniform_w;
    int32_t bf_fast;
    int32_t nms_fits;
    uint32_t nms_t[4];
    uint32_t lut_lo[6][4], lut_hi[6][4];
    uint32_t lut_ef_lo[6][4], lut_ef_hi[6][4];
};

struct LfLaneState {
    int32_t Th, l0, l1, t;
};

struct LfKernelArgs {
    const LfDevCode* code;
    const LfDevCfg* cfg;
    const int8_t* fix_input;
    int8_t* decoded;
    int8_t* st_en;
    uint4* st_rows;
    uint32_t* st_bits;
    LfLaneState* st_lane;
    const int32_t* status_cur;
    int32_t* status_next;
    uint32_t* remaining;
    int32_t* live;
    lnsfaid_group_stats* stats;
    int32_t n_cw;
};

struct LfCwArgs {
    const LfDevCode* code;
    const LfDevCfg* cfg;
    const int8_t* fix_input;
    int8_t* decoded;
    uint4* st_rows;
    const int32_t* skip;
    lnsfaid_group_stats* stats;
    lnsfaid_codeword_stats* cw_stats;
    int32_t n_cw;
};

static inline __host__ __device__ uint32_t lf_lds_off_hard(int n_var) { return ((uint32_t)n_var + 15u) & ~15u; }
static inline __host__ __device__ uint32_t lf_lds_off_p(int n_var, int n_words) { return lf_lds_off_hard(n_var) + (uint32_t)n_words * 4u; }
static inline __host__ __device__ uint32_t lf_lds_off_stat(int n_var, int n_words, int p_words)
{
    return (lf_lds_off_p(n_var, n_words) + ((uint32_t)p_words + 2u) * 4u + 7u) & ~7u;
}
#define LF_ZERO_SLOT 7
static inline __host__ __device__ uint32_t lf_lds_off_zero(int n_var, int n_words, int p_words)
{
    return lf_lds_off_stat(n_var, n_words, p_words) + (LNSFAID_GROUP + LF_ZERO_SLOT) * 4u;
}
static inline __host__ __device__ uint32_t lf_lds_bytes(int n_var, int n_words, int p_words)
{
    return lf_lds_off_stat(n_var, n_words, p_words) + (LNSFAID_GROUP + 8) * 4u;
}

#endif
```

### mod-interleaveavx_multithreads-faid_amd/csrc/lnsfaid_rows4.h

```cpp
#ifndef LNSFAID_ROWS4_H
#define LNSFAID_ROWS4_H

#include "lnsfaid_device.h"
#include "lnsfaid_phases.h"
#include "lnsfaid_swar.h"

#define LF_T4 64

#define LF4_OMS(M) ((M) == 1 || (M) == 3 || (M) == 4)

struct DevTab4 {
    CCode c;
    int br;
    uint32_t sbv;
    __device__ __forceinline__ uint32_t sb(int j) const { return c->circ[br][j].sb; }
    __device__ __forceinline__ uint32_t s4(int j) const { return c->s4tab[br][j]; }
    __device__ __forceinline__ uint32_t cb256(int j) const { return c->cbtab[br][j]; }
    __device__ __forceinline__ uint32_t sb_dyn4(uint32_t idx4) const
    {
        return (uint32_t)__builtin_amdgcn_ds_bpermute((int)idx4, (int)sbv);
    }
};

typedef __attribute__((address_space(3))) uint32_t lds4_u32;
__device__ __forceinline__ uint32_t lds4_rd(uint32_t a) { return *(const lds4_u32*)(size_t)a; }
__device__ __forceinline__ void lds4_wr(uint32_t a, uint32_t v) { *(lds4_u32*)(size_t)a = v; }

template <int B>
__device__ __forceinline__ void copy_in(uint32_t* dst, const uint32_t* __restrict__ src, int n, int tid)
{
    for (int i0 = 0; i0 < n; i0 += B * LF_T4) {
        uint32_t w[B];
#pragma unroll
        for (int u = 0; u < B; ++u) { const int i = i0 + u * LF_T4 + tid; w[u] = i < n ? src[i] : 0u; }
#pragma unroll
        for (int u = 0; u < B; ++u) { const int i = i0 + u * LF_T4 + tid; if (i < n) dst[i] = w[u]; }
    }
}

template <int B>
__device__ __forceinline__ void copy_out(uint32_t* __restrict__ dst, const uint32_t* src, int n, int tid)
{
    for (int i0 = 0; i0 < n; i0 += B * LF_T4) {
        uint32_t w[B];
#pragma unroll
        for (int u = 0; u < B; ++u) { const int i = i0 + u * LF_T4 + tid; w[u] = i < n ? src[i] : 0u; }
#pragma unroll
        for (int u = 0; u < B; ++u) { const int i = i0 + u * LF_T4 + tid; if (i < n) dst[i] = w[u]; }
    }
}

__device__ __forceinline__ uint32_t hard_flags(uint32_t x) { return x + 0x07070707u; }

template <int J>
__device__ __forceinline__ uint32_t plane_exchange(uint32_t x, uint32_t l5)
{
    constexpr uint32_t m_lo = J == 16 ? 0x0000ffffu : J == 8 ? 0x00ff00ffu : J == 4 ? 0x0f0f0f0fu : J == 2 ? 0x33333333u : 0x55555555u;
    uint32_t t;
    if (J == 1) t = (uint32_t)__builtin_amdgcn_mov_dpp((int)x, 0xb1, 0xf, 0xf, false);
    else if (J == 2) t = (uint32_t)__builtin_amdgcn_mov_dpp((int)x, 0x4e, 0xf, 0xf, false);
    else t = (uint32_t)__builtin_amdgcn_ds_swizzle((int)x, 0x1f | (J << 10));
    const bool up = (l5 & (uint32_t)J) != 0u;
    const uint32_t r = __builtin_amdgcn_alignbit(t, t, up ? (uint32_t)J : 32u - (uint32_t)J);
    const uint32_t keep = up ? ~m_lo : m_lo;
    return (x & keep) | (r & ~keep);
}

template <bool CONF>
__device__ __forceinline__ void build_plane4(CCode c, uint32_t* plane, int thr, int lane)
{
    const int nbc = c->nbc;
    const int th = thr < 1 ? 0 : (thr > 32 ? 32 : thr);
    const uint32_t th4 = (uint32_t)th * 0x01010101u;
    const uint32_t b8 = (uint32_t)(128 - SW_BIAS_EN) * 0x01010101u, b7 = (uint32_t)(127 - SW_BIAS_EN) * 0x01010101u;
    const uint32_t l5 = (uint32_t)lane & 31u;
    const int word_of_lane = (int)((l5 & 7u) * 8u + 2u * (l5 >> 3) + ((uint32_t)lane >> 5));
    for (int cb0 = 0; cb0 < nbc; cb0 += 8) {
        uint32_t x[8];
#pragma unroll
        for (int u = 0; u < 8; ++u)
            x[u] = lds4_rd((uint32_t)(cb0 + u < nbc ? cb0 + u : nbc - 1) * 256u + 4u * (uint32_t)lane);
        __builtin_amdgcn_sched_barrier(0);
        uint32_t g = 0;
#pragma unroll
        for (int u = 0; u < 8; ++u) {
            uint32_t fl;
            if (CONF) fl = th == 0 ? 0x80808080u : (((x[u] + b8) - th4) | ~(x[u] + b7 + th4));
            else fl = hard_flags(x[u]);
            g |= (fl >> (7 - u)) & (0x01010101u << u);
        }
        g = plane_exchange<16>(g, l5);
        g = plane_exchange<8>(g, l5);
        g = plane_exchange<4>(g, l5);
        g = plane_exchange<2>(g, l5);
        g = plane_exchange<1>(g, l5);
        if (cb0 + (int)(l5 & 7u) < nbc) plane[cb0 * 8 + word_of_lane] = g;
    }
    LF_WG_SYNC();
}

__device__ __forceinline__ bool layer0_dirty4(CCode c, int lane)
{
    const int deg = c->deg[0];
    const uint32_t tid4 = (uint32_t)lane << 2;
    uint32_t x4[LF_MAX_DEG], d[LF_MAX_DEG];
#pragma unroll
    for (int j = 0; j < LF_MAX_DEG; ++j) x4[j] = j < deg ? tid4 + c->s4tab[0][j] : 0u;
    __builtin_amdgcn_sched_barrier(0);
#pragma unroll
    for (int j = 0; j < LF_MAX_DEG; ++j)
        if (j < deg) d[j] = lds4_rd((x4[j] & 0xfcu) | c->cbtab[0][j]);
    __builtin_amdgcn_sched_barrier(0);
    uint32_t acc = 0;
#pragma unroll
    for (int j = 0; j < LF_MAX_DEG; ++j)
        if (j < deg) acc ^= hard_flags(__builtin_amdgcn_alignbyte(d[j], d[j], x4[j] >> 8));
    return __ballot((acc & 0x80808080u) != 0u) != 0ull;
}

__device__ __forceinline__ void publish_pass(int32_t* live, int cw, int t, int tid)
{
#ifdef LF4_LIVE_PROOF
    if (tid == 0) __hip_atomic_store(&live[cw], t, __ATOMIC_RELAXED, __HIP_MEMORY_SCOPE_AGENT);
#endif
}
__device__ __forceinline__ bool group_passed(const int32_t* live, int g, int t, int tid)
{
#ifndef LF4_LIVE_PROOF
    return false;
#else
    int v = 0;
    if (tid < LNSFAID_GROUP) v = __hip_atomic_load(&live[g * LNSFAID_GROUP + tid], __ATOMIC_RELAXED, __HIP_MEMORY_SCOPE_AGENT);
    return __ballot(v >= t) != 0ull;
#endif
}

__device__ __forceinline__ void write_decoded(const uint32_t* sHard, int8_t* g_out, int N, int tid)
{
    const int nw = N >> 5;
    if (((size_t)g_out) & 15u) {
        uint32_t* out32 = (uint32_t*)g_out;
        for (int i = tid; i < (N >> 2); i += LF_T4) out32[i] = (((sHard[i >> 3] >> ((i & 7) * 4)) & 15u) * 0x00204081u) & 0x01010101u;
        return;
    }
    uint4* out = (uint4*)g_out;
    for (int r0 = 0; r0 * LF_T4 < nw; r0 += 9) {
        uint32_t w[9];
#pragma unroll
        for (int u = 0; u < 9; ++u) { const int i = (r0 + u) * LF_T4 + tid; w[u] = i < nw ? sHard[i] : 0u; }
#pragma unroll
        for (int u = 0; u < 9; ++u) {
            const int i = (r0 + u) * LF_T4 + tid;
            if (i < nw) {
                uint32_t d[8];
#pragma unroll
                for (int q = 0; q < 8; ++q) d[q] = (((w[u] >> (4 * q)) & 15u) * 0x00204081u) & 0x01010101u;
                out[2 * i] = make_uint4(d[0], d[1], d[2], d[3]);
                out[2 * i + 1] = make_uint4(d[4], d[5], d[6], d[7]);
            }
        }
    }
}

__device__ void build_erasure_plane4(CCode c, const LfDevCode* gc, uint32_t* plane, const uint32_t* sP, int W, int tid)
{
    const int units = c->n_wcols * 4;
    for (int u = tid; u < units; u += LF_T4) {
        const int cb = gc->wcol[u >> 2];
        const uint32_t win = (uint32_t)(u & 3);
        uint32_t lo = 0xffffffffu, hi = 0xffffffffu;
        for (int k = 0; k < W; ++k) {
            const uint32_t cc = gc->colcirc[cb][k];
            uint32_t a, b;
            window64(sP + (cc & 0xffu) * 8u, (64u * win - ((cc >> 8) & 0xffu)) & 255u, a, b);
            lo &= a; hi &= b;
        }
        plane[cb * 8 + 2 * (int)win] = lo;
        plane[cb * 8 + 2 * (int)win + 1] = hi;
    }
    LF_WG_SYNC();
}


#define LF4_RM_LAYERS 12
static_assert(LF4_RM_LAYERS * 16 <= LF_SYN_ROUNDS * 64, "the RM instances assume that the syndrome walk tables fit the register cache");
typedef uint32_t lf4_vec __attribute__((ext_vector_type(LF4_RM_LAYERS)));
struct SwRegs {
    lf4_vec x0, x1, x2, cw, pa0, pa1;
};
__device__ __forceinline__ SwRow regs_get(const SwRegs& R, int br)
{
    SwRow r;
    r.x[0] = R.x0[br]; r.x[1] = R.x1[br]; r.x[2] = R.x2[br]; r.cw = R.cw[br]; r.pa[0] = R.pa0[br]; r.pa[1] = R.pa1[br];
    return r;
}
__device__ __forceinline__ void regs_put(SwRegs& R, int br, const SwRow& r)
{
    R.x0[br] = r.x[0]; R.x1[br] = r.x[1]; R.x2[br] = r.x[2]; R.cw[br] = r.cw; R.pa0[br] = r.pa[0]; R.pa1[br] = r.pa[1];
}

template <int METHOD, bool ERA, bool RM>
__device__ __forceinline__ void main_step4(CCode c, CCfg f, const LfDevCode* gc, SwRow* __restrict__ rows, SwRegs& R, int lane, int it, const uint32_t* sP,
                           bool have_par, bool lme, uint32_t era_plane)
{
    it = __builtin_amdgcn_readfirstlane(it);
    const SwK K = sw_consts((uint32_t)it);
    const bool fresh = (it == 1);
    const int rem = f->max_iter - it;
    const int itx = (it >= 1 && it <= 5) ? it - 1 : 5;
    SwParams p;
    p.lut_lo = f->lut_lo[itx][0]; p.lut_hi = f->lut_hi[itx][0];
    p.ef_lo = f->lut_ef_lo[itx][0]; p.ef_hi = f->lut_ef_hi[itx][0];
    p.f1 = f->factor_1; p.f2 = f->factor_2;
    p.window = rem <= f->floor_iter_thresh;
    p.ef_tables = f->ef >= 1;
    if (LF4_OMS(METHOD)) sw_oms_tables(p);
    if (METHOD == 0) { p.nms_t[0] = f->nms_t[0]; p.nms_t[1] = f->nms_t[1]; p.nms_t[2] = f->nms_t[2]; p.nms_t[3] = f->nms_t[3]; }
    const int nbr = c->nbr;
    const SwLds lds = SwLds();
    const SwRow zero = { { 0u, 0u, 0u }, 0u, { 0u, 0u } };
    if (RM) {
        uint32_t tabv = gc->sbplain[0][lane & 31];
#pragma nounroll
        for (int br = 0; br < nbr; ++br) {
            const int brn = br + 1 < nbr ? br + 1 : 0;
            const uint32_t tabn = gc->sbplain[brn][lane & 31];
            const int deg = c->deg[br];
            uint32_t rowpar = 0;
            if (have_par) {
#pragma unroll
                for (int k = 0; k < 4; ++k) {
                    const uint32_t wv = sP[br * 8 + 2 * k + (lane >> 5)];
                    rowpar |= ((wv >> (lane & 31)) & 1u) ? (0xffu << (8 * k)) : 0u;
                }
            }
            DevTab4 tab;
            tab.c = c; tab.br = br; tab.sbv = tabv;
            const SwRow cur = regs_get(R, br);
            SwRow st;
            const uint32_t era_edges = ERA ? c->era_edges[br] : 0u;
            if (ERA) st = sw_layer_step<METHOD, 0, ERA>(lds, tab, p, K, (uint32_t)lane, deg, cur, fresh, rowpar, lme, era_edges, era_plane);
            else if (deg == 23) st = sw_layer_step<METHOD, 23>(lds, tab, p, K, (uint32_t)lane, deg, cur, fresh, rowpar, lme);
            else if (deg == 22) st = sw_layer_step<METHOD, 22>(lds, tab, p, K, (uint32_t)lane, deg, cur, fresh, rowpar, lme);
            else st = sw_layer_step<METHOD, 0>(lds, tab, p, K, (uint32_t)lane, deg, cur, fresh, rowpar, lme);
            __builtin_amdgcn_sched_barrier(0);
            regs_put(R, br, st);
            __builtin_amdgcn_sched_barrier(0);
            tabv = tabn;
        }
        return;
    }
    SwRow cur = zero;
    if (!fresh) cur = rows[lane];
    uint32_t tabv = gc->sbplain[0][lane & 31];
    __builtin_amdgcn_s_waitcnt(0x0f70);
    for (int br = 0; br < nbr; ++br) {
        const int brn = br + 1 < nbr ? br + 1 : 0;
        const SwRow nxt = rows[brn * LF_T4 + lane];
        const uint32_t tabn = gc->sbplain[brn][lane & 31];
        const int deg = c->deg[br];
        uint32_t rowpar = 0;
        if (have_par) {
#pragma unroll
            for (int k = 0; k < 4; ++k) {
                const uint32_t wv = sP[br * 8 + 2 * k + (lane >> 5)];
                rowpar |= ((wv >> (lane & 31)) & 1u) ? (0xffu << (8 * k)) : 0u;
            }
        }
        DevTab4 tab;
        tab.c = c; tab.br = br; tab.sbv = tabv;
        SwRow st;
        const uint32_t era_edges = ERA ? c->era_edges[br] : 0u;
        if (ERA) st = sw_layer_step<METHOD, 0, ERA>(lds, tab, p, K, (uint32_t)lane, deg, cur, fresh, rowpar, lme, era_edges, era_plane);
        else if (deg == 23) st = sw_layer_step<METHOD, 23>(lds, tab, p, K, (uint32_t)lane, deg, cur, fresh, rowpar, lme);
        else if (deg == 22) st = sw_layer_step<METHOD, 22>(lds, tab, p, K, (uint32_t)lane, deg, cur, fresh, rowpar, lme);
        else st = sw_layer_step<METHOD, 0>(lds, tab, p, K, (uint32_t)lane, deg, cur, fresh, rowpar, lme);
        cur = fresh ? zero : nxt;
        tabv = tabn;
        asm volatile("" : "+v"(cur.x[0]), "+v"(cur.x[1]), "+v"(cur.x[2]), "+v"(cur.cw), "+v"(cur.pa[0]), "+v"(cur.pa[1]), "+v"(tabv));
        __builtin_amdgcn_sched_barrier(0);
        if (rem > 0) rows[br * LF_T4 + lane] = st;
    }
}

__device__ __forceinline__ void regs_store(const SwRegs& R, SwRow* __restrict__ rows, int nbr, int lane)
{
#pragma unroll
    for (int br = 0; br < LF4_RM_LAYERS; ++br)
        if (br < nbr) rows[br * LF_T4 + lane] = regs_get(R, br);
}
__device__ __forceinline__ void regs_load(SwRegs& R, const SwRow* __restrict__ rows, int nbr, int lane)
{
    SwRow r[LF4_RM_LAYERS];
#pragma unroll
    for (int br = 0; br < LF4_RM_LAYERS; ++br) r[br] = rows[(br < nbr ? br : nbr - 1) * LF_T4 + lane];
#pragma unroll
    for (int br = 0; br < LF4_RM_LAYERS; ++br) regs_put(R, br, r[br]);
}
__device__ __forceinline__ void regs_clear(SwRegs& R)
{
    const lf4_vec z = (lf4_vec)(0u);
    R.x0 = z; R.x1 = z; R.x2 = z; R.cw = z; R.pa0 = z; R.pa1 = z;
}

#define LF4_STAGE_INPUT() \
                                                 \
        const int8_t* gi = a.fix_input + (size_t)g * (size_t)LNSFAID_GROUP * (size_t)N;                                                                   \
        const int8_t* src_i = gi + (size_t)lane_in_group * (size_t)K;                                                                                     \
        const int8_t* src_p = gi + (size_t)LNSFAID_GROUP * (size_t)K + (size_t)lane_in_group * (size_t)M;                                                 \
        const int first_erased = N - c->puncture_tail;                                                                                                    \
        const int nbc = c->nbc;                                                                                                                           \
        if ((((size_t)a.fix_input) & 3u) == 0u) {                                                                                                         \
                                           \
            constexpr int SB = 23;                                                                                                                        \
            const uint32_t base_d = ((16u * (uint32_t)tid) & 0xffu) + ((uint32_t)tid >> 4);                                                               \
            const SwLds lds = SwLds();                                                                                                                    \
            for (int cb0 = 0; cb0 < nbc; cb0 += SB) {                                                                                                     \
                uint32_t w[SB];                                                                                                                           \
_Pragma("unroll")                                                                                                                                         \
                for (int u = 0; u < SB; ++u) {                                                                                                            \
                    const int cb = cb0 + u;                                                                                                               \
                    if (cb < nbc) {                                                                                                          \
                        const int8_t* col = cb * LF_Z < K ? src_i + cb * LF_Z : src_p + (cb * LF_Z - K);                                                  \
                        w[u] = ((const uint32_t*)col)[tid];                                                                                               \
                    }                                                                                                                                     \
                }                                                                                                                                         \
_Pragma("unroll")                                                                                                                                         \
                for (int u = 0; u < SB; ++u) {                                                                                                            \
                    const int cb = cb0 + u;                                                                                                               \
                    if (cb < nbc) {                                                                                                                       \
                        uint32_t x = w[u];                                                                                                                \
                        const int lim = first_erased - cb * LF_Z;                                        \
                        if (lim < LF_Z) {                                                                                                                 \
_Pragma("unroll")                                                                                                                                         \
                            for (int k = 0; k < 4; ++k) if (4 * tid + k >= lim) x &= ~(0xffu << (8 * k));                                                 \
                        }                                                                                                                                 \
                        x = ((x & 0x7f7f7f7fu) + (uint32_t)SW_BIAS_EN * 0x01010101u) ^ (x & 0x80808080u);  \
                        const uint32_t ad = (uint32_t)cb * 256u + base_d;                                                                                 \
                        lds.wr8(ad, x); lds.wr8(ad + 4u, x >> 8); lds.wr8(ad + 8u, x >> 16); lds.wr8(ad + 12u, x >> 24);                                  \
                    }                                                                                                                                     \
                }                                                                                                                                         \
            }                                                                                                                                             \
        } else {                                                                                                                                          \
            for (int cb = 0; cb < nbc; ++cb) {                                                         \
                uint32_t w = 0;                                                                                                                           \
_Pragma("unroll")                                                                                                                                         \
                for (int k = 0; k < 4; ++k) {                                                                                                             \
                    const int v = cb * LF_Z + tid + 64 * k;                                                                                               \
                    int x = v < K ? src_i[v] : src_p[v - K];                                                                                              \
                    if (v >= first_erased) x = 0;                                                                                                         \
                    w |= (uint32_t)((x + SW_BIAS_EN) & 0xff) << (8 * k);                                                                                  \
                }                                                                                                                                         \
                lds4_wr((uint32_t)cb * 256u + 4u * (uint32_t)tid, w);                                                                                     \
            }                                                                                                                                             \
        }                                                                                                                                                 \

#define LF4_LAYERED_LOOP() \
        while (prog < t_end && !(max_bf > 0 && prog >= t_bf0)) {                                                                                                                                         \
                                                                                                                         \
            int tid_i = tid;                                                                                                                                                                             \
            asm volatile("" : "+v"(tid_i));                                                                                                                                                              \
            if (METHOD == 0) {                                                                                           \
                main_step4<METHOD, false, RM>(c, f, a.code, g_rows, R, tid_i, prog, sP, false, false, 0u);                                                                                               \
                prog++;                                                                                                                                                                                  \
                continue;                                                                                                                                                                                \
            }                                                                                                                                                                                            \
            bool lme = false, have_par = false;                                                                                                                                                          \
                                                                                                              \
            const bool needs_checksums = max_iter - prog <= f->floor_iter_thresh;                                                                          \
                                                                                              \
            const bool must_know = needs_checksums || LF4_ON_FRONT;                                                                                                                                      \
            if (must_know && (needs_checksums || !layer0_dirty4(c, tid_i))) {                                                                                                                            \
                build_plane4<false>(c, sHard, 0, tid_i);                                                                                                                                                 \
                int unsat;                                                                                                                                                                               \
                if (RM || syn_cache_fits(c->nbr)) {  \
                    SynCache sc;                                                                                                                                                                         \
                    syn_cache_load(a.code, c->nbr, tid_i, sc);                                                                                                                                           \
                    unsat = syndrome<LF_T4, false, true>(c, a.code, sP, tid_i, pA, pB, sRed, &sc);                                                                                                       \
                } else {                                                                                                                                                                                 \
                    unsat = syndrome<LF_T4, false>(c, a.code, sP, tid_i, pA, pB, sRed);                                                                                                                  \
                }                                                                                                                                                                                        \
                                                                                                           \
                if (unsat == 0 && LF4_CLEAN_STOPS(tid_i)) {                                                                                                                                              \
                                                                                                                                                    \
                    LF4_ON_STOP(tid_i)                                                                                                                                                                   \
                    parked = true;                                                                                                                                                                       \
                    break;                                                                                                                                                                               \
                }                                                                                                                                                                                        \
                if (LF4_OMS(METHOD)) lme = imin(unsat, 255) < (int)(uint8_t)f->floor_err_count;                                                                                \
                else lme = imin(unsat, 127) < (int)(int8_t)f->floor_err_count;                                                                                                \
                have_par = true;                                                                                                                                                                         \
            }                                                                                                                                                                                            \
            LF4_ON_PASS(tid_i)                                                                                                                                                                           \
            if (EF2 && f->ef == 2 && needs_checksums && have_par && lme) {                                                                                                                               \
                                                                                      \
                build_erasure_plane4(c, a.code, sHard, sP, f->W, tid_i);                                                                                                                                 \
                main_step4<METHOD, EF2, RM>(c, f, a.code, g_rows, R, tid_i, prog, sP, true, lme, lf_lds_off_hard(N));                                                                                    \
            } else {                                                                                                                                                                                     \
                main_step4<METHOD, false, RM>(c, f, a.code, g_rows, R, tid_i, prog, sP, have_par && needs_checksums, lme, 0u);                                                                           \
            }                                                                                                                                                                                            \
            prog++;                                                                                                                                                                                      \
        }                                                                                                                                                                                                \

#define LF4_ENTER_BF() \
        if (!parked && prog < t_end) {                                                                                          \
                                      \
            uint32_t conf[LF_MAX_BC * 8 / LF_T4];                           \
            if (METHOD == 5) {                                                                                                  \
                build_plane4<true>(c, sHard, f->hard2_thr, tid);                       \
_Pragma("unroll")                                                                                                               \
                for (int k = 0; k < LF_MAX_BC * 8 / LF_T4; ++k) conf[k] = (tid + k * LF_T4 < nw) ? sHard[tid + k * LF_T4] : 0u; \
                LF_WG_SYNC();                                                                                                   \
            }                                                                                                                   \
            build_plane4<false>(c, sHard, 0, tid);                                                                              \
                                                        \
            copy_out<9>(sHard0, sHard, nw, tid);                                                                                \
            if (METHOD == 5) {                                                                                                  \
_Pragma("unroll")                                                                                                               \
                for (int k = 0; k < LF_MAX_BC * 8 / LF_T4; ++k) if (tid + k * LF_T4 < nw) sHard2[tid + k * LF_T4] = conf[k];    \
            }                                                                                                                   \
            ls.Th = (int8_t)f->W; ls.l0 = 0; ls.l1 = 0; ls.t = 1;                                                               \
            in_bf = true;                                                                                                       \
            LF_WG_SYNC();                                                                                                       \
        }                                                                                                                       \

#define LF4_BF_LOOPS() \
    if (in_bf && !parked) {                                                                                                                 \
        if ((RM || syn_cache_fits(c->nbr)) && (METHOD == 3 || bf_cache_fits(c, f))) {                                                       \
            SynCache sc;                                                                                                                    \
            BfCache bc;                                                                                                                     \
            syn_cache_load(a.code, c->nbr, tid, sc);                                                                                        \
            if (METHOD != 3) bf_cache_load(c, a.code, tid, bc);                                                                             \
            while (prog < t_end) {                                                                                                          \
                const int unsat = syndrome<LF_T4, false, true>(c, a.code, sP, tid, pA, pB, sRed, &sc);                                      \
                if (unsat == 0 && LF4_CLEAN_STOPS(tid)) { parked = true; break; }                                                           \
                LF4_ON_PASS(tid)                                                                                                            \
                if (METHOD == 3) bf_step_plain<LF_T4>(c, f, a.code, sHard, sHard2 + nw , sP, tid, sRed); \
                else bf_step<LF_T4, METHOD, true>(c, f, a.code, sHard, sHard0, sHard2, sP, tid, ls, sRed, &bc);                             \
                prog++;                                                                                                                     \
            }                                                                                                                               \
        } else {                                                                                                                            \
            while (prog < t_end) {                                                                                                          \
                const int unsat = syndrome<LF_T4, false>(c, a.code, sP, tid, pA, pB, sRed);                                                 \
                if (unsat == 0 && LF4_CLEAN_STOPS(tid)) { parked = true; break; }                                                           \
                LF4_ON_PASS(tid)                                                                                                            \
                if (METHOD == 3) bf_step_plain<LF_T4>(c, f, a.code, sHard, sHard2 + nw , sP, tid, sRed); \
                else bf_step<LF_T4, METHOD>(c, f, a.code, sHard, sHard0, sHard2, sP, tid, ls, sRed);                                        \
                prog++;                                                                                                                     \
            }                                                                                                                               \
        }                                                                                                                                   \
    }                                                                                                                                       \

#endif
```

### mod-interleaveavx_multithreads-faid_amd/csrc/lnsfaid_swar.h

```cpp
#ifndef LNSFAID_SWAR_H
#define LNSFAID_SWAR_H

#include <stdint.h>

#if defined(__HIPCC__)
#define SW_DEV 1
#define SW_FN __device__ __forceinline__
#define SW_HD __host__ __device__ __forceinline__
#else
#define SW_DEV 0
#define SW_FN static inline
#define SW_HD static inline
#endif

#define SW_MAX_DEG 24
#ifndef SW_ILP
#define SW_ILP 4
#endif

#if SW_DEV
#define SW_SCHED_FENCE() __builtin_amdgcn_sched_barrier(0)
#else
#define SW_SCHED_FENCE() ((void)0)
#endif
// ... 61 lines not shown
#endif
}

#define SW_T2N_LO 0xf900fafbu
#define SW_T2N_HI 0xf8000000u

struct SwK {
    uint32_t c78, c0642, cfc, sel_sign, tt_lo, tt_hi, oh_lo, oh_hi;
    uint32_t cbit[8];
    uint32_t c7f;
    uint32_t c70;
    uint32_t n_lo, n_hi;
    uint32_t c55, c33, c0f;
    uint32_t cm27;
};
SW_FN SwK sw_consts(uint32_t dep = 0u)
{
    SwK k;
    k.c78 = sw_vconst(0x78787878u, dep); k.c0642 = sw_vconst(0x06040200u, dep); k.cfc = sw_vconst(0xfcu, dep);
    k.sel_sign = sw_vconst(0x0b090a08u, dep);
    k.tt_lo = sw_vconst(0x07030100u, dep); k.tt_hi = sw_vconst(0xff3f1f0fu, dep);
    k.oh_lo = sw_vconst(0x08040201u, dep); k.oh_hi = sw_vconst(0x80402010u, dep);
    for (int e = 0; e < 8; ++e) k.cbit[e] = sw_vconst(0x01010101u << e, dep);
    k.c7f = sw_vconst(0x7f7f7f7fu, dep);
    k.c70 = sw_vconst(0x70707070u, dep);
    k.n_lo = sw_vconst(SW_T2N_LO, dep); k.n_hi = sw_vconst(SW_T2N_HI, dep);
    k.c55 = sw_vconst(0x55555555u, dep); k.c33 = sw_vconst(0x33333333u, dep); k.c0f = sw_vconst(0x0f0f0f0fu, dep);
    k.cm27 = sw_vconst(0u - 0x27272727u, dep);
    return k;
}

SW_FN uint32_t sw_mask7(uint32_t x, uint32_t sel_sign) { return sw_perm(x, x << 8, sel_sign); }
#define SW_SEL_SIGN 0x0b090a08u

SW_FN uint32_t sw_popcount7(uint32_t x)
{
    x &= 0x7f7f7f7fu;
    x = x - ((x >> 1) & 0x55555555u);
    x = (x & 0x33333333u) + ((x >> 2) & 0x33333333u);
    return (x + (x >> 4)) & 0x0f0f0f0fu;
}
SW_FN uint32_t sw_therm2num(uint32_t x, uint32_t n_lo, uint32_t n_hi)
{
    const uint32_t a = sw_perm(n_hi, n_lo, x & 0x0f0f0f0fu);
    const uint32_t b = sw_perm(n_hi, n_lo, (x >> 4) & 0x07070707u);
    return a ^ b;
}
SW_FN uint32_t sw_zero_mask(uint32_t x, uint32_t sel_sign) { return ~sw_mask7(x + 0x7f7f7f7fu, sel_sign); }

SW_FN uint32_t sw_gather4(uint32_t g0, uint32_t g1, uint32_t g2, uint32_t g3)
{
    const uint32_t lo = (g1 << 8) | g0, hi = (g3 << 8) | g2;
    return (hi << 16) | lo;
}
SW_FN uint32_t sw_opaque(uint32_t x)
{
#if SW_DEV
    asm("" : "+v"(x));
#endif
    return x;
}
SW_FN uint32_t sw_node_addr(uint32_t x) { return sw_perm(x, x, 0x0c0c0300u) | ((x >> 8) & 3u); }

SW_FN uint32_t sw_table_pick(uint32_t rowmask, uint32_t w_hi, uint32_t w_lo, uint32_t t_hi, uint32_t t_lo, uint32_t m)
{
    return sw_bitop3<SW_TT_SEL>(rowmask, sw_perm(w_hi, w_lo, m), sw_perm(t_hi, t_lo, m));
}
SW_FN uint32_t sw_word_pick(uint32_t nm3, uint32_t nm4, uint32_t x0, uint32_t x1, uint32_t x2)
{
    return sw_bitop3<SW_TT_SEL>(nm4, sw_bitop3<SW_TT_SEL>(nm3, x0, x1), x2);
}
SW_FN void sw_word_deal(uint32_t keep, uint32_t nm3, uint32_t nm4, uint32_t oh[3])
{
    oh[0] = sw_bitop3<SW_TT_AND3>(keep, nm3, nm4);
    oh[1] = sw_bitop3<0x20>(keep, nm3, nm4);
    oh[2] = keep & ~nm4;
}
SW_FN uint32_t sw_argmin_selector(uint32_t w, uint32_t oh8, uint32_t c7f, uint32_t c01, uint32_t c0642)
{
    return sw_bitop3<SW_TT_ANDOR>(((w & oh8) + c7f) >> 7, c01, c0642);
}

struct SwRow {
    uint32_t x[3];
    uint32_t cw;
    uint32_t pa[2];
};

struct SwParams {
    uint32_t lut_lo, lut_hi;
    uint32_t ef_lo, ef_hi;
    int32_t f1, f2;
    int32_t window;
    int32_t ef_tables;
    uint32_t nms_t[4];
    uint32_t oms_lo[2], oms_hi[2];
};

#if SW_DEV
struct SwLds {
    typedef __attribute__((address_space(3))) uint32_t lds_u32;
    typedef __attribute__((address_space(3))) uint8_t lds_u8;
    SW_FN uint32_t rd32(uint32_t a) const { return *(const lds_u32*)(size_t)a; }
    SW_FN void wr32(uint32_t a, uint32_t v) const { *(lds_u32*)(size_t)a = v; }
    SW_FN uint32_t rd8(uint32_t a) const { return *(const lds_u8*)(size_t)a; }
    SW_FN void wr8(uint32_t a, uint32_t v) const { *(lds_u8*)(size_t)a = (uint8_t)v; }
};
#else
struct SwLds {
    uint8_t* base;
    uint32_t rd32(uint32_t a) const { return (uint32_t)base[a] | ((uint32_t)base[a + 1] << 8) | ((uint32_t)base[a + 2] << 16) | ((uint32_t)base[a + 3] << 24); }
    void wr32(uint32_t a, uint32_t v) const { base[a] = (uint8_t)v; base[a + 1] = (uint8_t)(v >> 8); base[a + 2] = (uint8_t)(v >> 16); base[a + 3] = (uint8_t)(v >> 24); }
    uint32_t rd8(uint32_t a) const { return base[a]; }
    void wr8(uint32_t a, uint32_t v) const { base[a] = (uint8_t)v; }
};
#endif

#define SW_BIAS_EN 120

SW_FN uint32_t sw_en_pos(uint32_t v) { return (v & ~255u) | ((v & 63u) << 2) | ((v >> 6) & 3u); }

#define SW_OMS(M) ((M) == 1 || (M) == 3 || (M) == 4)
#define SW_MINSUM(M) ((M) == 0 || SW_OMS(M))

SW_FN int sw_oms_offset(int x, bool window, bool F, int f1, int f2)
{
    if (window && F) {
        if (x < f2) x += 1;
        if (x <= f1) x += 1;
    } else {
        if (x > f1) x -= 1;
        if (x >= f2) x -= 1;
    }
    return x;
}

SW_FN void sw_oms_tables(SwParams& p)
{
    for (int r = 0; r < 2; ++r) {
        uint32_t lo = 0, hi = 0;
        for (int x = 0; x < 8; ++x) {
            const int a = sw_oms_offset(x, r != 0, r != 0, p.f1, p.f2);
            const uint32_t v = (uint32_t)((a > 7 ? 7 : a) & 0xff);
            if (x < 4) lo |= v << (8 * x); else hi |= v << (8 * (x - 4));
        }
        p.oms_lo[r] = lo; p.oms_hi[r] = hi;
    }
}

SW_HD int sw_nms_cste(int m, int factor)
{
    const uint16_t p = (uint16_t)((uint16_t)m * (uint16_t)(int16_t)factor);
    const int16_t q = (int16_t)(p >> 5);
    const int r = q > 127 ? 127 : q;
    return r > 7 ? 7 : r;
}
SW_HD bool sw_nms_fits(int f1, int f2)
{
    if (f1 != f2) return false;
    for (int m = 1; m < 32; ++m)
        if (sw_nms_cste(m, f1) < sw_nms_cste(m - 1, f1)) return false;
    return sw_nms_cste(15, f1) == 7;
}
SW_HD void sw_nms_tables(int factor, uint32_t nms_t[4])
{
    for (int w = 0; w < 4; ++w) nms_t[w] = 0;
    for (int m = 0; m < 16; ++m) {
        const int c = sw_nms_cste(m, factor);
        const uint32_t code = c >= 7 ? 0xffu : ((1u << c) - 1u);
        nms_t[m >> 2] |= code << (8 * (m & 3));
    }
}

struct SwUpd {
    uint32_t za[2], sb[2];
    uint32_t oc[2], hi[2];
};
template <bool MINSUM, bool FLIP = true>
SW_FN SwUpd sw_update_consts(uint32_t c, uint32_t flip, uint32_t bias)
{
    const uint32_t za_p = 0x1f1f1f1fu - bias, za_n = za_p - c;
    const uint32_t sb_p = 0x27272727u - c, sb_n = 0x27272727u;
    const uint32_t oc_p = 0x3f3f3f3fu - c, oc_n = MINSUM ? 0x3f3f3f3fu : oc_p;
    const uint32_t hi_p = 0xbebebebeu - c, hi_n = MINSUM ? 0xbebebebeu : hi_p;
    SwUpd u;
    if (!FLIP) {
        u.za[1] = za_p; u.za[0] = za_n; u.sb[1] = sb_p; u.sb[0] = sb_n; u.oc[1] = oc_p; u.oc[0] = oc_n; u.hi[1] = hi_p; u.hi[0] = hi_n;
        return u;
    }
    u.za[1] = sw_bitop3<SW_TT_SEL>(flip, za_n, za_p); u.za[0] = sw_bitop3<SW_TT_SEL>(flip, za_p, za_n);
    u.sb[1] = sw_bitop3<SW_TT_SEL>(flip, sb_n, sb_p); u.sb[0] = sw_bitop3<SW_TT_SEL>(flip, sb_p, sb_n);
    if (MINSUM) {
        u.oc[1] = sw_bitop3<SW_TT_SEL>(flip, oc_n, oc_p); u.oc[0] = sw_bitop3<SW_TT_SEL>(flip, oc_p, oc_n);
        u.hi[1] = sw_bitop3<SW_TT_SEL>(flip, hi_n, hi_p); u.hi[0] = sw_bitop3<SW_TT_SEL>(flip, hi_p, hi_n);
    } else {
        u.oc[1] = u.oc[0] = oc_p; u.hi[1] = u.hi[0] = hi_p;
    }
    return u;
}
template <bool MINSUM>
SW_FN uint32_t sw_update(uint32_t tb, uint32_t ms, const SwUpd& u, uint32_t sel_sign, uint32_t c80)
{
    const uint32_t za = sw_bitop3<SW_TT_SEL>(ms, u.za[1], u.za[0]);
    const uint32_t sb = sw_bitop3<SW_TT_SEL>(ms, u.sb[1], u.sb[0]);
    const uint32_t oc = MINSUM ? sw_bitop3<SW_TT_SEL>(ms, u.oc[1], u.oc[0]) : u.oc[1];
    const uint32_t hi = MINSUM ? sw_bitop3<SW_TT_SEL>(ms, u.hi[1], u.hi[0]) : u.hi[1];
    const uint32_t zb = tb + za;
    const uint32_t mo = sw_mask7(zb - oc, sel_sign);
    const uint32_t mq = sw_mask7(zb, sel_sign);
    return sw_bitop3<SW_TT_SEL>(mo, hi, sw_bitop3<SW_TT_SEL>(mq, zb, c80)) - sb;
}

struct SwUpd2 {
    uint32_t c, fm, zc, oc, hi;
};
template <bool MINSUM>
SW_FN SwUpd2 sw_update2_consts(uint32_t c, uint32_t fm, uint32_t bias)
{
    SwUpd2 u;
    u.c = c; u.fm = fm;
    u.zc = 0x1f1f1f1fu - bias - c;
    u.oc = MINSUM ? 0u - 0x3f3f3f3fu : 0x3f3f3f3fu - c;
    u.hi = MINSUM ? 0xbebebebeu : 0xbebebebeu - c;
    return u;
}
SW_FN uint32_t sw_upd2_d(uint32_t ms, const SwUpd2& u) { return sw_bitop3<SW_TT_XORAND>(ms, u.fm, u.c); }
SW_FN uint32_t sw_upd2_zb(uint32_t tb, uint32_t d, const SwUpd2& u) { return tb + d + u.zc; }
template <bool MINSUM>
SW_FN uint32_t sw_upd2_out(uint32_t zb, uint32_t d, const SwUpd2& u)
{
    const uint32_t ov = MINSUM ? zb + d + u.oc : zb - u.oc;
    return sw_bitop3<0xcf>(zb, ov, ov);
}
template <bool MINSUM>
SW_FN uint32_t sw_upd2_limit(uint32_t ms, uint32_t d, const SwUpd2& u, uint32_t c80)
{
    return sw_bitop3<SW_TT_ANDOR>(ms, MINSUM ? u.hi - d : u.hi, c80);
}
SW_FN uint32_t sw_upd2_en(uint32_t mout, uint32_t lim, uint32_t zb, uint32_t d, uint32_t cm27) { return sw_bitop3<SW_TT_SEL>(mout, lim, zb) + d + cm27; }
template <bool MINSUM>
SW_FN uint32_t sw_update2(uint32_t tb, uint32_t ms, const SwUpd2& u, uint32_t sel_sign, uint32_t c80, uint32_t cm27)
{
    const uint32_t d = sw_upd2_d(ms, u);
    const uint32_t zb = sw_upd2_zb(tb, d, u);
    const uint32_t mout = sw_mask7(sw_upd2_out<MINSUM>(zb, d, u), sel_sign);
    return sw_upd2_en(mout, sw_upd2_limit<MINSUM>(ms, d, u, c80), zb, d, cm27);
}

SW_FN void sw_min_edge(uint32_t& t1, uint32_t& t2, uint32_t ta[5], uint32_t u, int j)
{
    t2 = sw_bitop3<SW_TT_A_AND_BORC>(t2, t1, u);
    t1 &= u;
#pragma unroll
    for (int b = 0; b < 5; ++b)
        if (((j >> b) & 1) == (b >= 3 ? 1 : 0)) ta[b] &= u;
}
SW_FN void sw_min_quad(uint32_t& t1, uint32_t& t2, uint32_t ta[5], uint32_t v0, uint32_t v1, uint32_t v2, uint32_t v3, int j0)
{
    const uint32_t p0 = v0 & v1, p1 = v2 & v3, q = p0 & p1;
    const uint32_t o0 = v0 | v1, o1 = v2 | v3;
    const uint32_t m2 = sw_bitop3<SW_TT_A_AND_BORC>(o0, p0, p1);
    const uint32_t y = sw_bitop3<SW_TT_A_AND_BORC>(t2, t1, q);
    t2 = sw_bitop3<SW_TT_AND3>(y, m2, o1);
    t1 &= q;
    ta[0] = sw_bitop3<SW_TT_AND3>(ta[0], v0, v2);
    ta[1] &= p0;
    if (((j0 >> 2) & 1) == 0) ta[2] &= q;
    if (((j0 >> 3) & 1) == 1) ta[3] &= q;
    if (((j0 >> 4) & 1) == 1) ta[4] &= q;
}

SW_FN void sw_sign_edge(uint32_t ns[3], uint32_t ms, int j, uint32_t cbit) { ns[j >> 3] = sw_bitop3<SW_TT_ANDNOT_OR>(ns[j >> 3], ms, cbit); }
template <int NJ>
SW_FN void sw_sign_quad(uint32_t ns[3], const uint32_t* ms, int j0, int deg, bool fixed, uint32_t c55, uint32_t c33, uint32_t c0f)
{
    uint32_t m[4];
#pragma unroll
    for (int g = 0; g < 4; ++g) m[g] = (j0 + g < NJ && (fixed || j0 + g < deg)) ? ms[j0 + g < NJ ? j0 + g : 0] : 0u;
    const bool has1 = j0 + 1 < NJ, has2 = j0 + 2 < NJ, has3 = j0 + 3 < NJ;
    const uint32_t a = has1 ? sw_bitop3<SW_TT_SEL>(c55, m[0], m[1]) : m[0];
    const uint32_t b = has3 ? sw_bitop3<SW_TT_SEL>(c55, m[2], m[3]) : m[2];
    const uint32_t q = has2 ? sw_bitop3<SW_TT_SEL>(c33, a, b) : a;
    ns[j0 >> 3] = (j0 & 4) ? sw_bitop3<SW_TT_SEL>(c0f, ns[j0 >> 3], q) : q;
}

SW_FN uint32_t sw_plane_bit(const SwLds& lds, uint32_t era_plane, uint32_t a)
{
    const uint32_t v = (a & ~255u) | ((a >> 2) & 63u) | ((a & 3u) << 6);
    return (lds.rd32(era_plane + ((v >> 5) << 2)) >> (v & 31u)) & 1u;
}

#if SW_DEV
#define SW_MFN __device__ __forceinline__
#else
#define SW_MFN inline
#endif
struct SwNoXch {
    SW_MFN void put(int, uint32_t) const {}
    SW_MFN uint32_t get(int) const { return 0u; }
    SW_MFN void barrier() const {}
};
#define SW_OWN(j) (WAVES == 1 || (((j) & 1) == WAVE))

template <int METHOD, int DEG, bool ERA = false, int WAVES = 1, int WAVE = 0, class Tab, class Xch = SwNoXch>
SW_FN SwRow sw_layer_step(const SwLds& lds, const Tab& tab, const SwParams& p, const SwK& K, uint32_t lane, int deg, SwRow cur, bool fresh,
                          uint32_t rowpar, bool lme, uint32_t era_edges = 0u, uint32_t era_plane = 0u, const Xch& xch = Xch())
{
    static_assert(WAVES == 1 || !ERA, "the erasing variant is built for one wave per codeword only");
    static_assert(!ERA || METHOD == 2, "the erasure exists in Decode_FAID only");
    constexpr int NJ = DEG > 0 ? DEG : SW_MAX_DEG;
    constexpr bool MINSUM = SW_MINSUM(METHOD);
    constexpr bool QUADS = WAVES == 1 && SW_ILP == 4 && DEG > 0;
    constexpr bool NSTREE = WAVES == 1 && SW_ILP == 4;
    const uint32_t c01 = K.cbit[0], c80 = K.cbit[7], c7f = K.c7f, c78 = K.c78, c0642 = K.c0642, cfc = K.cfc, sel_sign = K.sel_sign;
    const uint32_t tid4 = lane << 2;
    uint32_t s4j[NJ], cbj[NJ];
#pragma unroll
    for (int j = 0; j < NJ; ++j) { s4j[j] = (DEG > 0 || j < deg) ? tab.s4(j) : 0u; cbj[j] = (DEG > 0 || j < deg) ? tab.cb256(j) : 0u; }

    const uint32_t c2o = cur.cw & 0x07070707u, c1o = (cur.cw >> 3) & 0x07070707u;
    const uint32_t kp = 0x08080808u - c2o, kn = 0x08080808u + c2o;
    const uint32_t bias = MINSUM ? 0u : 0x06040200u;
    const uint32_t kt_lo = sw_perm(kn, kp, 0x05010400u) + (MINSUM ? 0u : 0x02020000u), kt_hi = sw_perm(kn, kp, 0x07030602u) + (MINSUM ? 0u : 0x06060404u);
    const uint32_t tt_lo = K.tt_lo, tt_hi = K.tt_hi;

    uint32_t padd = 0, psub = 0;
#ifndef SW_EXP_NO_OLDPATCH
    if (!fresh && WAVE == 0) {
        const uint32_t a0 = cur.pa[0] & 0xffffu, a1 = cur.pa[0] >> 16, a2 = cur.pa[1] & 0xffffu, a3 = cur.pa[1] >> 16;
        SW_SCHED_FENCE();
        const uint32_t g0 = lds.rd8(a0), g1 = lds.rd8(a1), g2 = lds.rd8(a2), g3 = lds.rd8(a3);
        const uint32_t mneg = sw_mask7(cur.cw << 1, sel_sign);
        padd = sw_bitop3<SW_TT_SEL>(mneg, c1o, c2o); psub = sw_bitop3<SW_TT_SEL>(mneg, c2o, c1o);
        SW_SCHED_FENCE();
        const uint32_t r = sw_gather4(g0, g1, g2, g3) + padd - psub;
        const uint32_t rh = sw_opaque(r >> 8);
        lds.wr8(a0, r); lds.wr8(a1, rh); lds.wr8(a2, r >> 16); lds.wr8(a3, rh >> 16);
    }
#endif
    if (WAVES == 2) xch.barrier();

    SW_SCHED_FENCE();
    uint32_t tb[NJ], ts[NJ], ms[NJ], ad[NJ], rq[NJ], ld[NJ];
    uint32_t t1 = 0xffffffffu, t2 = 0xffffffffu, ta[5] = { 0xffffffffu, 0xffffffffu, 0xffffffffu, 0xffffffffu, 0xffffffffu };
    uint32_t sx = 0;

#pragma unroll
    for (int j = 0; j < NJ; ++j) {
        if ((DEG > 0 || j < deg) && SW_OWN(j)) {
            const uint32_t x4 = tid4 + s4j[j];
#if SW_DEV
            uint32_t a;
            asm("v_and_or_b32 %0, %1, %2, %3" : "=v"(a) : "v"(x4), "v"(cfc), "s"(cbj[j]));
#else
            const uint32_t a = (x4 & cfc) | cbj[j];
#endif
            ad[j] = a; rq[j] = x4 >> 8;
        }
    }
#pragma unroll
    for (int j = 0; j < NJ; ++j)
        if ((DEG > 0 || j < deg) && SW_OWN(j)) ld[j] = lds.rd32(ad[j]);
    SW_SCHED_FENCE();
#pragma unroll
    for (int j0 = 0; j0 < NJ; j0 += SW_ILP) {
        uint32_t r_[SW_ILP], x_[SW_ILP], s_[SW_ILP], k_[SW_ILP], a_[SW_ILP], i_[SW_ILP], u_[SW_ILP];
#define SW_EDGES(...) _Pragma("unroll") for (int g = 0; g < SW_ILP; ++g) { const int j = j0 + g; if (j < NJ && (DEG > 0 || j < deg) && SW_OWN(j)) { __VA_ARGS__ } }
        _Pragma("unroll") for (int g = SW_ILP - 1; g >= 0; --g) { const int j = j0 + g; if (j < NJ && (DEG > 0 || j < deg) && SW_OWN(j)) r_[g] = sw_alignbyte(ld[j], ld[j], rq[j]); }
        SW_EDGES(x_[g] = (j & 7) ? cur.x[j >> 3] >> (j & 7) : cur.x[j >> 3];)
        SW_EDGES(s_[g] = sw_bitop3<SW_TT_ANDOR>(x_[g], c01, c0642);)
        SW_EDGES(k_[g] = sw_perm(kt_hi, kt_lo, s_[g]);)
        SW_EDGES(tb[j] = r_[g] + k_[g];)
        if (ERA) {
            SW_EDGES(x_[g] &= c01;)
            SW_EDGES(
                if ((era_edges >> j) & 1u) {
                    uint32_t em = 0, match = 0;
                    _Pragma("unroll") for (int k = 0; k < 4; ++k) {
                        const uint32_t a = ad[j] + ((rq[j] + (uint32_t)k) & 3u);
                        em |= sw_plane_bit(lds, era_plane, a) ? (0xffu << (8 * k)) : 0u;
                        const uint32_t pold = (k & 1) ? cur.pa[k >> 1] >> 16 : cur.pa[k >> 1] & 0xffffu;
                        match |= (!fresh && a == pold) ? (0xffu << (8 * k)) : 0u;
                    }
                    const uint32_t en_true = r_[g] - (padd & match) + (psub & match);
                    const uint32_t neg01 = ~((en_true + 0x08080808u) >> 7) & c01;
                    tb[j] = sw_bitop3<SW_TT_SEL>(em, c80 + bias, tb[j]);
                    x_[g] = sw_bitop3<SW_TT_SEL>(em, neg01, x_[g]);
                })
        }
        SW_EDGES(ts[j] = MINSUM ? tb[j] : tb[j] - (ERA ? (x_[g] | c0642) : s_[g]);)
        SW_EDGES(ms[j] = sw_mask7(ts[j], sel_sign);)
        SW_EDGES(a_[g] = sw_bitop3<SW_TT_XOR3>(ts[j], c7f, ms[j]);)
        if (METHOD == 0) {
            uint32_t h_[SW_ILP];
            SW_EDGES(i_[g] = sw_bitop3<SW_TT_NANDOR>(ms[j], c01, K.c70);)
            SW_EDGES(a_[g] = (a_[g] + i_[g]) & 0x8f8f8f8fu;)
            SW_EDGES(h_[g] = sw_mask7(a_[g] << 4, sel_sign);)
            SW_EDGES(a_[g] &= 0x87878787u;)
            SW_EDGES(i_[g] = sw_perm(p.nms_t[3], p.nms_t[2], a_[g]);)
            SW_EDGES(u_[g] = sw_perm(p.nms_t[1], p.nms_t[0], a_[g]);)
            SW_EDGES(u_[g] = sw_bitop3<SW_TT_SEL>(h_[g], i_[g], u_[g]);)
        } else {
            SW_EDGES(i_[g] = MINSUM ? sw_bitop3<SW_TT_NANDOR>(ms[j], c01, c78) : sw_bitop3<SW_TT_XNOR_AND>(x_[g], ms[j], c01);)
            SW_EDGES(a_[g] = (MINSUM ? a_[g] + i_[g] : a_[g] + i_[g] + c78) & 0x87878787u;)
            SW_EDGES(u_[g] = sw_perm(tt_hi, tt_lo, a_[g]);)
        }
        SW_EDGES(
            if (WAVES == 2) sx ^= ts[j];
            else if (j & 1) sx = sw_bitop3<SW_TT_XOR3>(sx, ts[j - 1], ts[j]); else if (j == (DEG > 0 ? DEG : deg) - 1) sx ^= ts[j];)
        if (QUADS) {
            uint32_t v_[4];
            _Pragma("unroll") for (int g = 0; g < 4; ++g) v_[g] = j0 + g < NJ ? u_[g] : 0xffffffffu;
            sw_min_quad(t1, t2, ta, v_[0], v_[1], v_[2], v_[3], j0);
        } else {
            SW_EDGES(sw_min_edge(t1, t2, ta, u_[g], j);)
        }
    }

    if (WAVES == 2) {
        if (WAVE == 1) {
            xch.put(0, t1); xch.put(1, t2); xch.put(2, ta[1]); xch.put(3, ta[2]); xch.put(4, ta[3]); xch.put(5, ta[4]); xch.put(6, sx);
        }
        xch.barrier();
        if (WAVE == 0) {
            const uint32_t o1 = xch.get(0), o2 = xch.get(1);
            ta[0] = t1;
            t2 = sw_bitop3<SW_TT_AND3>(t2, o2, t1 | o1);
            t1 &= o1;
            ta[1] &= xch.get(2); ta[2] &= xch.get(3); ta[3] &= xch.get(4); ta[4] &= xch.get(5);
            sx ^= xch.get(6);
        }
    }
    uint32_t c2n_x = 0, fm_x = 0;
    if (WAVES == 2 && WAVE == 1) {
        xch.barrier();
        c2n_x = xch.get(0); fm_x = xch.get(1);
    }

    const uint32_t n_lo = WAVES == 2 ? SW_T2N_LO : K.n_lo, n_hi = WAVES == 2 ? SW_T2N_HI : K.n_hi;
    const uint32_t min1 = sw_therm2num(t1, n_lo, n_hi), min2 = sw_therm2num(t2, n_lo, n_hi);
    uint32_t c1n, c2n;
    if (METHOD == 0) {
        c2n = min1;
        c1n = min2;
    } else if (SW_OMS(METHOD)) {
        const bool win = p.window && lme;
        const uint32_t w_lo = win ? p.oms_lo[1] : p.oms_lo[0], w_hi = win ? p.oms_hi[1] : p.oms_hi[0];
        c2n = sw_table_pick(rowpar, w_hi, w_lo, p.oms_hi[0], p.oms_lo[0], min1);
        c1n = sw_table_pick(rowpar, w_hi, w_lo, p.oms_hi[0], p.oms_lo[0], min2);
    } else {
        const bool win = (METHOD == 5 || p.ef_tables) && p.window && lme;
        const uint32_t w_lo = win ? p.ef_lo : p.lut_lo, w_hi = win ? p.ef_hi : p.lut_hi;
        c2n = sw_table_pick(rowpar, w_hi, w_lo, p.lut_hi, p.lut_lo, min1);
        c1n = sw_table_pick(rowpar, w_hi, w_lo, p.lut_hi, p.lut_lo, min2);
    }
#if SW_DEV
    asm volatile("" : "+v"(c1n), "+v"(c2n));
#endif
    const uint32_t fm = (WAVES == 2 && WAVE == 1) ? fm_x : sw_mask7(sx, sel_sign);
    if (WAVES == 2 && WAVE == 1) { c2n = c2n_x; c1n = 0u; }

    uint32_t idx = 0, ne7_3 = 0, ne7_4 = 0;
#pragma unroll
    for (int b = 4; b >= 0; --b) {
        const uint32_t dd = sw_bitop3<SW_TT_XORAND>(ta[b], t1, c7f);
        const uint32_t ne7 = dd + c7f;
        const uint32_t ne = ne7 >> (7 - b);
        if (b == 4) ne7_4 = ne7;
        if (b == 3) ne7_3 = ne7;
        if (b == 4) idx = (DEG == 0 && deg <= 16) ? 0u : ~ne & (0x01010101u << 4);
        else if (b == 3) idx = (DEG == 0 && deg <= 8) ? idx : sw_bitop3<0xf2>(idx, ne | (idx >> 1), 0x01010101u << 3);
        else idx = sw_bitop3<SW_TT_ANDNOT_OR>(idx, ne, 0x01010101u << b);
    }

    uint32_t pa[4], sbk[4], gk0 = 0, gk1 = 0, gk2 = 0, gk3 = 0, xb = 0;
    const uint32_t idx4 = idx << 2;
#pragma unroll
#ifdef SW_EXP_NO_ARGMIN
    for (int k = 0; k < 4; ++k) sbk[k] = (cbj[k] << 16) | s4j[k];
#else
    for (int k = 0; k < 4; ++k) sbk[k] = WAVE == 0 ? tab.sb_dyn4((idx4 >> (8 * k)) & 0x7cu) : 0u;
#endif
    SW_SCHED_FENCE();

    const SwUpd2 u2 = sw_update2_consts<MINSUM>(c2n, fm, bias);
    const uint32_t cm27 = WAVES == 2 ? 0u - 0x27272727u : K.cm27;
    uint32_t ns[3] = { 0u, 0u, 0u };
    uint32_t cbit[8];
#pragma unroll
    for (int e = 0; e < 8; ++e) cbit[e] = K.cbit[e];
#define SW_PASS2_ARITH(J0, EN)                                                                                       \
    {                                                                                                                \
        const int j0 = (J0);                                                                                         \
        uint32_t d_[SW_ILP], zb[SW_ILP], mo[SW_ILP], lm[SW_ILP];                                                     \
        SW_EDGES(d_[g] = sw_upd2_d(ms[j], u2);)                                                                      \
        SW_EDGES(zb[g] = sw_upd2_zb(tb[j], d_[g], u2);)                                                              \
        SW_EDGES(mo[g] = sw_upd2_out<MINSUM>(zb[g], d_[g], u2);)                                                     \
        SW_EDGES(mo[g] = sw_mask7(mo[g], sel_sign);)                                              \
        SW_EDGES(lm[g] = sw_upd2_limit<MINSUM>(ms[j], d_[g], u2, c80);)                                              \
        SW_EDGES(EN[g] = sw_upd2_en(mo[g], lm[g], zb[g], d_[g], cm27);)                                              \
        SW_EDGES(EN[g] = sw_alignbyte(EN[g], EN[g], 4u - rq[j]);)                                                    \
        if (NSTREE) sw_sign_quad<NJ>(ns, ms, j0, deg, DEG > 0, K.c55, K.c33, K.c0f);                                 \
        else SW_EDGES(sw_sign_edge(ns, ms[j], j, cbit[j & 7]);)                                                      \
    }
#define SW_PASS2_STORE(J0, EN)                                                                                       \
    {                                                                                                                \
        const int j0 = (J0);                                                                                         \
        SW_EDGES(lds.wr32(ad[j], EN[g]);)                                                                            \
    }
    uint32_t en0[SW_ILP], en1[SW_ILP];
    SW_PASS2_ARITH(0, en0)
    SW_SCHED_FENCE();
#pragma unroll
    for (int k = 0; k < 4; ++k)
        pa[k] = sw_node_addr(tid4 + sbk[k] + ((uint32_t)k << 8));
#ifdef SW_EXP_NO_ARGMIN
    gk0 = ld[0] & 0xffu; gk1 = ld[1] & 0xffu; gk2 = ld[2] & 0xffu; gk3 = ld[3] & 0xffu;
#else
    if (WAVE == 0) { gk0 = lds.rd8(pa[0]); gk1 = lds.rd8(pa[1]); gk2 = lds.rd8(pa[2]); gk3 = lds.rd8(pa[3]); }
#endif
    if (WAVES == 2 && WAVE == 0) {
        xch.put(0, c2n); xch.put(1, fm);
        xch.barrier();
    }
    SW_SCHED_FENCE();
    SW_PASS2_STORE(0, en0)
    if (SW_ILP < NJ) { SW_PASS2_ARITH(SW_ILP, en1) SW_PASS2_STORE(SW_ILP, en1) }
    SW_SCHED_FENCE();
    const uint32_t oh8 = sw_perm(K.oh_hi, K.oh_lo, idx & 0x07070707u);
    const uint32_t nm4 = (DEG == 0 && deg <= 16) ? 0xffffffffu : sw_mask7(ne7_4, sel_sign);
    const uint32_t nm3 = (DEG == 0 && deg <= 8) ? 0xffffffffu : sw_mask7(ne7_3, sel_sign);
    const uint32_t selA = sw_argmin_selector(sw_word_pick(nm3, nm4, cur.x[0], cur.x[1], cur.x[2]), oh8, c7f, c01, c0642);
    if (ERA) xb = selA & c01;
    const uint32_t gb = sw_gather4(gk0, gk1, gk2, gk3);
    uint32_t tbA = gb + sw_perm(kt_hi, kt_lo, selA);
    if (ERA) {
        uint32_t em = 0, match = 0;
#pragma unroll
        for (int k = 0; k < 4; ++k) {
            const uint32_t ik = (idx >> (8 * k)) & 31u;
            if ((era_edges >> ik) & 1u) em |= sw_plane_bit(lds, era_plane, pa[k]) ? (0xffu << (8 * k)) : 0u;
            const uint32_t pold = (k & 1) ? cur.pa[k >> 1] >> 16 : cur.pa[k >> 1] & 0xffffu;
            match |= (!fresh && pa[k] == pold) ? (0xffu << (8 * k)) : 0u;
        }
        const uint32_t en_true = gb - (padd & match) + (psub & match);
        tbA = sw_bitop3<SW_TT_SEL>(em, c80 + bias, tbA);
        xb = sw_bitop3<SW_TT_SEL>(em, ~((en_true + 0x08080808u) >> 7) & c01, xb);
    }
    const uint32_t tsA = MINSUM ? tbA : tbA - (ERA ? (xb | c0642) : selA);
    const uint32_t msA = sw_mask7(tsA, sel_sign);
    const uint32_t negA = ~(msA ^ fm);
    const SwUpd2 u1 = sw_update2_consts<MINSUM>(c1n, fm, bias);
    const uint32_t enA = sw_update2<MINSUM>(tbA, msA, u1, sel_sign, c80, cm27);

#pragma unroll
    for (int jg = 2 * SW_ILP; jg < NJ; jg += SW_ILP) {
        uint32_t en[SW_ILP];
        SW_PASS2_ARITH(jg, en)
        SW_PASS2_STORE(jg, en)
    }
#undef SW_EDGES
#undef SW_PASS2_ARITH
#undef SW_PASS2_STORE
    if (WAVES == 2) {
        if (WAVE == 1) { xch.put(0, ns[0]); xch.put(1, ns[1]); xch.put(2, ns[2]); }
        xch.barrier();
        if (WAVE == 1) { SwRow none = { { 0u, 0u, 0u }, 0u, { 0u, 0u } }; return none; }
        ns[0] |= xch.get(0); ns[1] |= xch.get(1); ns[2] |= xch.get(2);
    }
#ifndef SW_EXP_NO_ARGMIN
    {
        const uint32_t eh = sw_opaque(enA >> 8);
        lds.wr8(pa[0], enA); lds.wr8(pa[1], eh); lds.wr8(pa[2], enA >> 16); lds.wr8(pa[3], eh >> 16);
    }
#endif

    SwRow out;
    const int n = DEG > 0 ? DEG : deg;
#pragma unroll
    for (int g = 0; g < 3; ++g) {
        const int cnt = n - 8 * g < 0 ? 0 : (n - 8 * g > 8 ? 8 : n - 8 * g);
        const uint32_t valid = 0x01010101u * ((1u << cnt) - 1u);
        out.x[g] = ~(ns[g] ^ fm) & valid;
    }
    if (!MINSUM) {
        const uint32_t z2 = sw_zero_mask(c2n, sel_sign), nz1 = ~sw_zero_mask(c1n, sel_sign);
        const uint32_t keep = oh8 & nz1;
        uint32_t oh[3];
        sw_word_deal(keep, nm3, nm4, oh);
#pragma unroll
        for (int g = 0; g < 3; ++g) out.x[g] &= ~z2 | oh[g];
    }
    out.cw = c2n | (c1n << 3) | (negA & 0x40404040u);
    out.pa[0] = pa[0] | (pa[1] << 16);
    out.pa[1] = pa[2] | (pa[3] << 16);
    return out;
}

#endif
```

### mod-interleaveavx_multithreads-faid_amd/pyabi.py

```python
import ctypes as C
import os

HERE = os.path.dirname(os.path.abspath(__file__))
LIB_PATH = os.path.join(HERE, "csrc", "liblnsfaid.so")

GROUP = 32
MSG_REGISTERS, MSG_HBM = 1, 2
STOP_GROUP, STOP_CODEWORD = 0, 1


class Code(C.Structure):
    _fields_ = [
        ("n_var", C.c_int32),
        ("n_check", C.c_int32),
        ("n_edges", C.c_int32),
        ("z", C.c_int32),
        ("puncture_tail", C.c_int32),
        ("nb_degres", C.c_int32),
        ("deg", C.POINTER(C.c_int32)),
        ("deg_rows", C.POINTER(C.c_int32)),
        ("pos_vn", C.POINTER(C.c_uint16)),
    ]


class Cfg(C.Structure):
    _fields_ = [
        ("decode_method", C.c_int32),
        ("max_iteration", C.c_int32),
        ("factor_1", C.c_int32),
        ("factor_2", C.c_int32),
        ("floor_err_count", C.c_int32),
        ("floor_iter_thresh", C.c_int32),
        ("ef_elimination", C.c_int32),
        ("max_bf_iter", C.c_int32),
        ("bf_L0", C.c_int32),
        ("bf_L1", C.c_int32),
        ("bf_alpha", C.c_int32),
        ("bf_delta", C.c_int32),
        ("regular_col_weight", C.c_int32),
        ("hard2_threshold", C.c_int32),
        ("bf_vote_cap", C.c_int32),
        ("v2c_map", C.c_int8 * 8 * 4 * 6),
        ("v2c_map_ef", C.c_int8 * 8 * 4 * 6),
    ]


class GroupStats(C.Structure):
    _fields_ = [("iterations", C.c_int32), ("bf_iterations", C.c_int32)]


class CodewordStats(C.Structure):
    _fields_ = [("iterations", C.c_int32), ("bf_iterations", C.c_int32), ("unsatisfied", C.c_int32)]


SYMBOLS = {
    "lnsfaid_code_50gpon": (C.c_int, [C.POINTER(Code), C.POINTER(C.c_uint16), C.POINTER(C.c_int32), C.POINTER(C.c_int32)]),
    "lnsfaid_cfg_default": (C.c_int, [C.POINTER(Cfg), C.c_int32, C.c_int32]),
    "lnsfaid_cfg_table_preset": (C.c_int, [C.POINTER(Cfg), C.c_int32]),
    "lnsfaid_cfg_ef_elimination": (C.c_int, [C.POINTER(Cfg), C.c_int32]),
    "lnsfaid_create": (C.c_int, [C.POINTER(C.c_void_p), C.POINTER(Code), C.POINTER(Cfg), C.c_int32, C.c_size_t]),
    "lnsfaid_destroy": (None, [C.c_void_p]),
    "lnsfaid_set_cfg": (C.c_int, [C.c_void_p, C.POINTER(Cfg)]),
    "lnsfaid_decode": (C.c_int, [C.c_void_p, C.c_void_p, C.c_size_t, C.c_void_p, C.c_void_p]),
    "lnsfaid_decode_device": (C.c_int, [C.c_void_p, C.c_void_p, C.c_size_t, C.c_void_p, C.c_void_p]),
    "lnsfaid_set_early_stop": (C.c_int, [C.c_void_p, C.c_int32]),
    "lnsfaid_early_stop": (C.c_int, [C.c_void_p]),
    "lnsfaid_decode_codewords": (C.c_int, [C.c_void_p, C.c_void_p, C.c_size_t, C.c_void_p, C.c_void_p]),
    "lnsfaid_decode_codewords_device": (C.c_int, [C.c_void_p, C.c_void_p, C.c_size_t, C.c_void_p, C.c_void_p]),
    "lnsfaid_count_errors": (C.c_int, [C.c_void_p, C.c_void_p, C.c_void_p, C.c_size_t, C.POINTER(C.c_uint64)]),
    "lnsfaid_count_errors_device": (C.c_int, [C.c_void_p, C.c_void_p, C.c_void_p, C.c_size_t, C.POINTER(C.c_uint64)]),
    "lnsfaid_decode_packed": (C.c_int, [C.c_void_p, C.c_void_p, C.c_size_t, C.c_void_p, C.c_void_p]),
    "lnsfaid_decode_packed_device": (C.c_int, [C.c_void_p, C.c_void_p, C.c_size_t, C.c_void_p, C.c_void_p]),
    "lnsfaid_decode_codewords_packed": (C.c_int, [C.c_void_p, C.c_void_p, C.c_size_t, C.c_void_p, C.c_void_p]),
    "lnsfaid_decode_codewords_packed_device": (C.c_int, [C.c_void_p, C.c_void_p, C.c_size_t, C.c_void_p, C.c_void_p]),
    "lnsfaid_count_errors_packed": (C.c_int, [C.c_void_p, C.c_void_p, C.c_void_p, C.c_size_t, C.POINTER(C.c_uint64)]),
    "lnsfaid_count_errors_packed_device": (C.c_int, [C.c_void_p, C.c_void_p, C.c_void_p, C.c_size_t, C.POINTER(C.c_uint64)]),
    "lnsfaid_pack_llr4": (C.c_int, [C.c_void_p, C.c_size_t, C.c_void_p]),
    "lnsfaid_unpack_bits": (C.c_int, [C.c_void_p, C.c_size_t, C.c_void_p]),
    "lnsfaid_pack_bits": (C.c_int, [C.c_void_p, C.c_size_t, C.c_void_p]),
    "lnsfaid_frontend_device": (C.c_int, [C.c_void_p, C.POINTER(C.c_uint32), C.POINTER(C.c_uint64), C.c_size_t, C.c_int32,
                                          C.c_float, C.c_float, C.c_void_p, C.c_void_p]),
    "lnsfaid_frontend_device_states": (C.c_int, [C.c_void_p, C.POINTER(C.c_uint32), C.POINTER(C.c_uint64), C.c_size_t, C.c_int32,
                                                 C.c_float, C.c_float, C.c_void_p, C.c_void_p]),
    "lnsfaid_frontend_draws_per_group": (C.c_uint64, [C.c_void_p, C.c_int32]),
    "lnsfaid_frontend_set_interleave": (C.c_int, [C.c_void_p, C.c_int32]),
    "lnsfaid_demap_device": (C.c_int, [C.c_void_p, C.c_void_p, C.c_size_t, C.c_int32, C.c_float, C.c_void_p]),
    "lnsfaid_demap_packed_device": (C.c_int, [C.c_void_p, C.c_void_p, C.c_size_t, C.c_int32, C.c_float, C.c_void_p]),
    "lnsfaid_demap_host": (C.c_int, [C.c_int32, C.c_int32, C.c_int32, C.c_void_p, C.c_size_t, C.c_int32, C.c_float, C.c_void_p]),
    "lnsfaid_demap_packed_host": (C.c_int, [C.c_int32, C.c_int32, C.c_int32, C.c_void_p, C.c_size_t, C.c_int32, C.c_float, C.c_void_p]),
    "lnsfaid_frontend_set_frames": (C.c_int, [C.c_void_p, C.c_void_p, C.c_void_p, C.c_size_t]),
    "lnsfaid_frontend_input_bits": (C.c_int, [C.c_void_p, C.POINTER(C.c_void_p)]),
    "lnsfaid_code_parity_inverse": (C.c_int, [C.POINTER(Code), C.c_void_p, C.c_size_t]),
    "lnsfaid_encode_device": (C.c_int, [C.c_void_p, C.c_void_p, C.c_size_t, C.c_void_p]),
    "lnsfaid_encode": (C.c_int, [C.c_void_p, C.c_void_p, C.c_size_t, C.c_void_p]),
    "lnsfaid_frontend_random_frames": (C.c_int, [C.c_void_p, C.POINTER(C.c_uint64), C.c_size_t]),
    "lnsfaid_io_buffers": (C.c_int, [C.c_void_p, C.POINTER(C.c_void_p), C.POINTER(C.c_void_p), C.POINTER(C.c_void_p)]),
    "lnsfaid_read_stats": (C.c_int, [C.c_void_p, C.c_void_p, C.c_size_t]),
    "lnsfaid_host_register": (C.c_int, [C.c_void_p, C.c_size_t]),
    "lnsfaid_host_unregister": (C.c_int, [C.c_void_p]),
    "lnsfaid_comm_unique_id": (C.c_int, [C.c_void_p]),
    "lnsfaid_comm_init": (C.c_int, [C.c_void_p, C.c_int32, C.c_int32, C.c_void_p]),
    "lnsfaid_comm_attach": (C.c_int, [C.c_void_p, C.c_void_p]),
    "lnsfaid_comm_destroy": (C.c_int, [C.c_void_p]),
    "lnsfaid_allreduce_counters": (C.c_int, [C.c_void_p, C.POINTER(C.c_uint64)]),
    "lnsfaid_select_kernel": (C.c_int, [C.c_void_p, C.c_int32]),
    "lnsfaid_kernel_rows_per_lane": (C.c_int, [C.c_void_p]),
    "lnsfaid_select_waves": (C.c_int, [C.c_void_p, C.c_int32]),
    "lnsfaid_frontend_set_exact": (C.c_int, [C.c_void_p, C.c_int32]),
    "lnsfaid_frontend_fastpath_bounds": (C.c_int, [C.c_void_p, C.POINTER(C.c_double), C.POINTER(C.c_double)]),
    "lnsfaid_kernel_waves": (C.c_int, [C.c_void_p]),
    "lnsfaid_select_message_store": (C.c_int, [C.c_void_p, C.c_int32]),
    "lnsfaid_message_store": (C.c_int, [C.c_void_p]),
    "lnsfaid_kernel_residency": (C.c_int, [C.c_void_p, C.POINTER(C.c_int32), C.POINTER(C.c_int32)]),
    "lnsfaid_kernel_time": (C.c_int, [C.c_void_p, C.POINTER(C.c_double), C.POINTER(C.c_uint64), C.c_int32]),
    "lnsfaid_stream": (C.c_void_p, [C.c_void_p]),
    "lnsfaid_strerror": (C.c_char_p, [C.c_int]),
    "lnsfaid_last_hip_error": (C.c_char_p, []),
    "lnsfaid_version": (C.c_char_p, []),
}


def bind(lib, symbols):
    for name, (res, args) in symbols.items():
        fn = getattr(lib, name)
        fn.restype = res
        fn.argtypes = args
    return lib


_lib = None


def load():
    global _lib
    if _lib is None:
        if not os.path.exists(LIB_PATH):
            raise RuntimeError(
                "HIP extension %s is missing: run `python -c 'import __graft_entry__ as g; g.build()'` "
                "(no CPU fallback exists in the product path)" % LIB_PATH)
        _lib = bind(C.CDLL(LIB_PATH), SYMBOLS)
    return _lib


class Code50GPON:

    def __init__(self, lib=None):
        lib = lib or load()
        self.pos_vn = (C.c_uint16 * 70400)()
        self.deg = (C.c_int32 * 3)()
        self.deg_rows = (C.c_int32 * 3)()
        self.code = Code()
        rc = lib.lnsfaid_code_50gpon(C.byref(self.code), self.pos_vn, self.deg, self.deg_rows)
        if rc != 0:
            raise RuntimeError("lnsfaid_code_50gpon failed: %d" % rc)

    @property
    def N(self):
        return self.code.n_var

    @property
    def M(self):
        return self.code.n_check

    @property
    def K(self):
        return self.code.n_var - self.code.n_check


def default_cfg(method, max_iter, lib=None):
    lib = lib or load()
    cfg = Cfg()
    rc = lib.lnsfaid_cfg_default(C.byref(cfg), method, max_iter)
    if rc != 0:
        raise ValueError("lnsfaid_cfg_default(%d, %d) failed: %d" % (method, max_iter, rc))
    return cfg


def pack_llr4(fix_input, lib=None):
    import numpy as np
    lib = lib or load()
    fix_input = np.ascontiguousarray(fix_input, dtype=np.int8)
    out = np.empty(fix_input.size // 2, dtype=np.uint8)
    rc = lib.lnsfaid_pack_llr4(fix_input.ctypes.data, fix_input.size, out.ctypes.data)
    if rc != 0:
        raise ValueError("lnsfaid_pack_llr4 failed: %d" % rc)
    return out


def unpack_bits(bits, lib=None):
    import numpy as np
    lib = lib or load()
    bits = np.ascontiguousarray(bits, dtype=np.uint32)
    out = np.empty(bits.size * 32, dtype=np.int8)
    rc = lib.lnsfaid_unpack_bits(bits.ctypes.data, out.size, out.ctypes.data)
    if rc != 0:
        raise ValueError("lnsfaid_unpack_bits failed: %d" % rc)
    return out


def pack_bits(input_bits, lib=None):
    import numpy as np
    lib = lib or load()
    input_bits = np.ascontiguousarray(input_bits, dtype=np.int8)
    out = np.empty(input_bits.size // 8, dtype=np.uint8)
    rc = lib.lnsfaid_pack_bits(input_bits.ctypes.data, input_bits.size, out.ctypes.data)
    if rc != 0:
        raise ValueError("lnsfaid_pack_bits failed: %d" % rc)
    return out


def _demap_host(fn_name, packed, n_var, n_check, interleave, rx, n_groups, mod_type, scale, lib):
    import numpy as np
    lib = lib or load()
    rx = np.ascontiguousarray(rx, dtype=np.float32)
    floats = n_groups * GROUP * n_var * (1 if mod_type == 1 else 2) // max(mod_type, 1)
    if rx.size != floats:
        raise ValueError("%s: rx has %d floats, %d groups of mod_type %d take %d" % (fn_name, rx.size, n_groups, mod_type, floats))
    out = np.empty(n_groups * GROUP * n_var // (2 if packed else 1), dtype=np.uint8 if packed else np.int8)
    rc = getattr(lib, fn_name)(n_var, n_check, interleave, rx.ctypes.data, n_groups, mod_type, scale, out.ctypes.data)
    if rc != 0:
        raise ValueError("%s failed: %d" % (fn_name, rc))
    return out


def demap_host(n_var, n_check, interleave, rx, n_groups, mod_type, scale, lib=None):
    return _demap_host("lnsfaid_demap_host", False, n_var, n_check, interleave, rx, n_groups, mod_type, scale, lib)


def demap_packed_host(n_var, n_check, interleave, rx, n_groups, mod_type, scale, lib=None):
    return _demap_host("lnsfaid_demap_packed_host", True, n_var, n_check, interleave, rx, n_groups, mod_type, scale, lib)


class Decoder:

    def __init__(self, code50, cfg, device=0, max_groups=64, lib=None):
        self.lib = lib or load()
        self.code50 = code50
        self.ctx = C.c_void_p()
        rc = self.lib.lnsfaid_create(C.byref(self.ctx), C.byref(code50.code), C.byref(cfg), device, max_groups)
        if rc != 0:
            raise RuntimeError("lnsfaid_create failed: %d (%s; hip: %s)" % (
                rc, self.lib.lnsfaid_strerror(rc).decode(), self.lib.lnsfaid_last_hip_error().decode()))

    def _check(self, rc, what):
        if rc != 0:
            raise RuntimeError("%s failed: %d (%s; hip: %s)" % (
                what, rc, self.lib.lnsfaid_strerror(rc).decode(), self.lib.lnsfaid_last_hip_error().decode()))

    def set_cfg(self, cfg):
        self._check(self.lib.lnsfaid_set_cfg(self.ctx, C.byref(cfg)), "lnsfaid_set_cfg")

    def decode(self, fix_input, n_groups):
        import numpy as np
        N = self.code50.N
        assert fix_input.dtype == np.int8 and fix_input.size == n_groups * GROUP * N and fix_input.flags.c_contiguous
        out = np.empty(n_groups * GROUP * N, dtype=np.int8)
        stats = np.zeros((n_groups, 2), dtype=np.int32)
        self._check(self.lib.lnsfaid_decode(self.ctx, fix_input.ctypes.data, n_groups, out.ctypes.data,
                                            stats.ctypes.data), "lnsfaid_decode")
        return out, stats

    def set_early_stop(self, rule):
        self._check(self.lib.lnsfaid_set_early_stop(self.ctx, rule), "lnsfaid_set_early_stop")

    def early_stop(self):
        return self.lib.lnsfaid_early_stop(self.ctx)

    def decode_codewords(self, fix_input, n_groups, with_stats=True):
        import numpy as np
        N = self.code50.N
        assert fix_input.dtype == np.int8 and fix_input.size == n_groups * GROUP * N and fix_input.flags.c_contiguous
        out = np.empty(n_groups * GROUP * N, dtype=np.int8)
        cw = np.zeros((n_groups * GROUP, 3), dtype=np.int32) if with_stats else None
        self._check(self.lib.lnsfaid_decode_codewords(self.ctx, fix_input.ctypes.data, n_groups, out.ctypes.data,
                                                      cw.ctypes.data if with_stats else None), "lnsfaid_decode_codewords")
        return out, cw

    def decode_codewords_device(self, d_fix_ptr, n_groups, d_out_ptr, d_cw_stats_ptr=None):
        self._check(self.lib.lnsfaid_decode_codewords_device(self.ctx, d_fix_ptr, n_groups, d_out_ptr, d_cw_stats_ptr),
                    "lnsfaid_decode_codewords_device")

    def decode_device(self, d_fix_ptr, n_groups, d_out_ptr, d_stats_ptr=None):
        self._check(self.lib.lnsfaid_decode_device(self.ctx, d_fix_ptr, n_groups, d_out_ptr, d_stats_ptr),
                    "lnsfaid_decode_device")

    def count_errors(self, decoded, input_bits, n_groups):
        out = (C.c_uint64 * 4)()
        ip = input_bits.ctypes.data if input_bits is not None else None
        self._check(self.lib.lnsfaid_count_errors(self.ctx, decoded.ctypes.data, ip, n_groups, out), "lnsfaid_count_errors")
        return list(out)

    def count_errors_device(self, d_decoded_ptr, d_input_ptr, n_groups):
        out = (C.c_uint64 * 4)()
        self._check(self.lib.lnsfaid_count_errors_device(self.ctx, d_decoded_ptr, d_input_ptr, n_groups, out),
                    "lnsfaid_count_errors_device")
        return list(out)

    def decode_packed(self, llr4, n_groups):
        import numpy as np
        N = self.code50.N
        assert llr4.dtype == np.uint8 and llr4.size == n_groups * GROUP * N // 2 and llr4.flags.c_contiguous
        out = np.empty(n_groups * GROUP * N // 32, dtype=np.uint32)
        stats = np.zeros((n_groups, 2), dtype=np.int32)
        self._check(self.lib.lnsfaid_decode_packed(self.ctx, llr4.ctypes.data, n_groups, out.ctypes.data, stats.ctypes.data),
                    "lnsfaid_decode_packed")
        return out, stats

    def decode_codewords_packed(self, llr4, n_groups, with_stats=True):
        import numpy as np
        N = self.code50.N
        assert llr4.dtype == np.uint8 and llr4.size == n_groups * GROUP * N // 2 and llr4.flags.c_contiguous
        out = np.empty(n_groups * GROUP * N // 32, dtype=np.uint32)
        cw = np.zeros((n_groups * GROUP, 3), dtype=np.int32) if with_stats else None
        self._check(self.lib.lnsfaid_decode_codewords_packed(self.ctx, llr4.ctypes.data, n_groups, out.ctypes.data,
                                                             cw.ctypes.data if with_stats else None), "lnsfaid_decode_codewords_packed")
        return out, cw

    def decode_packed_device(self, d_llr4_ptr, n_groups, d_bits_ptr, d_stats_ptr=None):
        self._check(self.lib.lnsfaid_decode_packed_device(self.ctx, d_llr4_ptr, n_groups, d_bits_ptr, d_stats_ptr),
                    "lnsfaid_decode_packed_device")

    def decode_codewords_packed_device(self, d_llr4_ptr, n_groups, d_bits_ptr, d_cw_stats_ptr=None):
        self._check(self.lib.lnsfaid_decode_codewords_packed_device(self.ctx, d_llr4_ptr, n_groups, d_bits_ptr, d_cw_stats_ptr),
                    "lnsfaid_decode_codewords_packed_device")

    def count_errors_packed(self, bits, msg, n_groups):
        out = (C.c_uint64 * 4)()
        mp = msg.ctypes.data if msg is not None else None
        self._check(self.lib.lnsfaid_count_errors_packed(self.ctx, bits.ctypes.data, mp, n_groups, out), "lnsfaid_count_errors_packed")
        return list(out)

    def count_errors_packed_device(self, d_bits_ptr, d_msg_ptr, n_groups):
        out = (C.c_uint64 * 4)()
        self._check(self.lib.lnsfaid_count_errors_packed_device(self.ctx, d_bits_ptr, d_msg_ptr, n_groups, out),
                    "lnsfaid_count_errors_packed_device")
        return list(out)

    def demap_device(self, d_rx_ptr, n_groups, mod_type, scale, d_fix_ptr):
        self._check(self.lib.lnsfaid_demap_device(self.ctx, d_rx_ptr, n_groups, mod_type, scale, d_fix_ptr), "lnsfaid_demap_device")

    def demap_packed_device(self, d_rx_ptr, n_groups, mod_type, scale, d_llr4_ptr):
        self._check(self.lib.lnsfaid_demap_packed_device(self.ctx, d_rx_ptr, n_groups, mod_type, scale, d_llr4_ptr),
                    "lnsfaid_demap_packed_device")

    def encode(self, info, n_groups):
        import numpy as np
        K, N = self.code50.K, self.code50.N
        assert info.dtype == np.int8 and info.size == n_groups * GROUP * K and info.flags.c_contiguous
        out = np.empty(n_groups * GROUP * N, dtype=np.int8)
        self._check(self.lib.lnsfaid_encode(self.ctx, info.ctypes.data, n_groups, out.ctypes.data), "lnsfaid_encode")
        return out

    def encode_device(self, d_in_ptr, n_groups, d_out_ptr):
        self._check(self.lib.lnsfaid_encode_device(self.ctx, d_in_ptr, n_groups, d_out_ptr), "lnsfaid_encode_device")

    def random_frames(self, keys):
        buf = (C.c_uint64 * len(keys))(*[int(k) for k in keys])
        self._check(self.lib.lnsfaid_frontend_random_frames(self.ctx, buf, len(keys)), "lnsfaid_frontend_random_frames")

    def comm_init(self, n_ranks, rank, comm_id):
        self._check(self.lib.lnsfaid_comm_init(self.ctx, n_ranks, rank, comm_id), "lnsfaid_comm_init")

    def allreduce_counters(self, counters):
        buf = (C.c_uint64 * 4)(*[int(c) for c in counters])
        self._check(self.lib.lnsfaid_allreduce_counters(self.ctx, buf), "lnsfaid_allreduce_counters")
        return list(buf)

    def select_kernel(self, rows_per_lane):
        self._check(self.lib.lnsfaid_select_kernel(self.ctx, rows_per_lane), "lnsfaid_select_kernel")

    def rows_per_lane(self):
        return self.lib.lnsfaid_kernel_rows_per_lane(self.ctx)

    def select_waves(self, waves_per_codeword):
        self._check(self.lib.lnsfaid_select_waves(self.ctx, waves_per_codeword), "lnsfaid_select_waves")

    def kernel_waves(self):
        return self.lib.lnsfaid_kernel_waves(self.ctx)

    def select_message_store(self, where):
        self._check(self.lib.lnsfaid_select_message_store(self.ctx, where), "lnsfaid_select_message_store")

    def message_store(self):
        return self.lib.lnsfaid_message_store(self.ctx)

    def kernel_residency(self):
        wg, lim = C.c_int32(), C.c_int32()
        self._check(self.lib.lnsfaid_kernel_residency(self.ctx, C.byref(wg), C.byref(lim)), "lnsfaid_kernel_residency")
        return wg.value, lim.value

    def kernel_time(self, reset=False):
        ms = C.c_double()
        n = C.c_uint64()
        self._check(self.lib.lnsfaid_kernel_time(self.ctx, C.byref(ms), C.byref(n), 1 if reset else 0), "lnsfaid_kernel_time")
        return ms.value, n.value

    def close(self):
        if self.ctx:
            self.lib.lnsfaid_destroy(self.ctx)
            self.ctx = C.c_void_p()

    def __del__(self):
        try:
            self.close()
        except Exception:
            pass
```

Measured before the change: 75.27.

## Add zero-shift specialized layer kernel that skips rotations for zero-shift circulants

Reorders each layer's edges so circulants with zero shift come first, and adds a new decode kernel instantiated per degree and zero-group count. For those leading edges it skips the address computation and the byte-align rotations on both load and store. It is enabled by default when the messages-in-registers kernel4 path applies, and adds more kernel instances, per-layer dispatch and extra code-table memory.

```diff
diff --git a/include/lnsfaid.h b/include/lnsfaid.h
--- a/include/lnsfaid.h
+++ b/include/lnsfaid.h
@@ -172,6 +172,12 @@
 int lnsfaid_select_message_store(lnsfaid_ctx* ctx, int32_t where);
 int lnsfaid_message_store(const lnsfaid_ctx* ctx);
 
+#define LNSFAID_ZERO_SHIFT_ON 1
+#define LNSFAID_ZERO_SHIFT_OFF 2
+int lnsfaid_select_zero_shift(lnsfaid_ctx* ctx, int32_t mode);
+int lnsfaid_zero_shift_groups(const lnsfaid_ctx* ctx, int32_t* groups, int32_t n);
+int lnsfaid_code_zero_shift_order(const lnsfaid_code* code, int32_t* groups, int32_t* order);
+
 int lnsfaid_kernel_residency(lnsfaid_ctx* ctx, int32_t* workgroups_per_cu, int32_t* lds_limit);
 
 
diff --git a/mod-interleaveavx_multithreads-faid_amd/csrc/lnsfaid_capi.hip b/mod-interleaveavx_multithreads-faid_amd/csrc/lnsfaid_capi.hip
--- a/mod-interleaveavx_multithreads-faid_amd/csrc/lnsfaid_capi.hip
+++ b/mod-interleaveavx_multithreads-faid_amd/csrc/lnsfaid_capi.hip
@@ -30,6 +30,9 @@
 extern "C" hipError_t lf_launch_pack_bits(const int8_t* d_decoded, uint32_t* d_bits, size_t n_values, hipStream_t stream);
 extern "C" hipError_t lf_launch_count_errors_packed(const uint32_t* d_bits, const uint32_t* d_msg, int n_var, int k_info, size_t n_cw,
                                                     unsigned long long* out, hipStream_t stream);
+extern "C" int lf_decode4z_inst(int deg, int zg);
+extern "C" const void* lf_decode4z_func(int method);
+extern "C" hipError_t lf_launch_decode4z(int method, const LfKernelArgs* args, size_t lds_bytes, hipStream_t stream);
 extern "C" const void* lf_decode5_func(int method);
 extern "C" int lf_decode5_threads(void);
 extern "C" hipError_t lf_launch_decode5(int method, const LfKernelArgs* args, size_t lds_bytes, hipStream_t stream);
@@ -116,6 +119,7 @@
     int rows_per_lane = 0;
     int waves_per_cw = 0;
     int msg_store = 0;
+    int zero_shift = 0;
     struct LfCombiner* comb = nullptr;
     int comb_slot = -1;
     const void* checked_fn[4] = {};
@@ -201,6 +205,19 @@
             }
         }
         e += (size_t)deg * Z;
+        for (int j = 0; j < 32; ++j) out->zsbplain[br][j] = 0u;
+        int n = 0;
+        for (int zero = 1; zero >= 0; --zero)
+            for (int j = 0; j < deg; ++j)
+                if ((out->s4tab[br][j] == 0u) == (zero != 0)) {
+                    out->zsbplain[br][n] = out->sbplain[br][j];
+                    out->zs4tab[br][n] = out->s4tab[br][j];
+                    out->zcbtab[br][n] = out->cbtab[br][j];
+                    ++n;
+                }
+        int n_zero = 0;
+        while (n_zero < deg && out->zs4tab[br][n_zero] == 0u) ++n_zero;
+        out->zinst[br] = lf_decode4z_inst(deg, n_zero / 4);
     }
     {
         const int nw = N / 32, pw = M / 32;
@@ -407,6 +424,8 @@
         ctx->fe_exact = (e[0] == '1') ? 1 : 0;
     if (const char* e = getenv("LNSFAID_MSG_STORE"))
         ctx->msg_store = (e[0] == 'h') ? LNSFAID_MSG_HBM : ((e[0] == 'r') ? LNSFAID_MSG_REGISTERS : 0);
+    if (const char* e = getenv("LNSFAID_ZERO_SHIFT"))
+        ctx->zero_shift = (e[0] == 'o' && e[1] == 'f') ? LNSFAID_ZERO_SHIFT_OFF : 0;
     g_live_contexts.fetch_add(1, std::memory_order_relaxed);
     const int rc = create_impl(ctx, code, cfg);
     if (rc) { lnsfaid_destroy(ctx); return rc; }
@@ -496,6 +515,54 @@
     return ctx->msg_store != LNSFAID_MSG_HBM;
 }
 
+static int layer_zero_groups(const lnsfaid_ctx* ctx, int br) { return (ctx->hcode.zinst[br] >> 8) & 0xff; }
+static bool zero_shift_possible(const lnsfaid_ctx* ctx)
+{
+    if (!use_kernel4(ctx) || use_kernel5(ctx) || !use_msg_registers(ctx)) return false;
+    if (ctx->hcfg.method < 1 || ctx->hcfg.method > 5 || !lf_decode4z_func(ctx->hcfg.method)) return false;
+    for (int br = 0; br < ctx->hcode.nbr; ++br)
+        if (layer_zero_groups(ctx, br) >= 1) return true;
+    return false;
+}
+static bool use_zero_shift(const lnsfaid_ctx* ctx) { return ctx->zero_shift != LNSFAID_ZERO_SHIFT_OFF && zero_shift_possible(ctx); }
+
+extern "C" int lnsfaid_select_zero_shift(lnsfaid_ctx* ctx, int32_t mode)
+{
+    if (!ctx || mode < 0 || mode > LNSFAID_ZERO_SHIFT_OFF) return LNSFAID_E_INVAL;
+    if (mode == LNSFAID_ZERO_SHIFT_ON && !zero_shift_possible(ctx)) return LNSFAID_E_INVAL;
+    ctx->zero_shift = mode;
+    return LNSFAID_OK;
+}
+
+extern "C" int lnsfaid_zero_shift_groups(const lnsfaid_ctx* ctx, int32_t* groups, int32_t n)
+{
+    if (!ctx || n < 0 || (n > 0 && !groups)) return LNSFAID_E_INVAL;
+    const bool on = use_zero_shift(ctx);
+    for (int br = 0; br < n; ++br) groups[br] = (on && br < ctx->hcode.nbr) ? layer_zero_groups(ctx, br) : 0;
+    return on ? 1 : 0;
+}
+
+extern "C" int lnsfaid_code_zero_shift_order(const lnsfaid_code* code, int32_t* groups, int32_t* order)
+{
+    LfDevCode* dc = new (std::nothrow) LfDevCode;
+    if (!dc) return LNSFAID_E_NOMEM;
+    const int rc = build_code(code, dc);
+    if (rc) { delete dc; return rc; }
+    const int nbr = dc->nbr;
+    for (int br = 0; br < nbr; ++br) {
+        int n_zero = 0;
+        while (n_zero < dc->deg[br] && dc->zs4tab[br][n_zero] == 0u) ++n_zero;
+        if (groups) groups[br] = n_zero / 4;
+        for (int j = 0; order && j < LF_MAX_DEG; ++j) {
+            order[br * LF_MAX_DEG + j] = -1;
+            for (int i = 0; j < dc->deg[br] && i < dc->deg[br]; ++i)
+                if (dc->cbtab[br][i] == dc->zcbtab[br][j] && dc->s4tab[br][i] == dc->zs4tab[br][j]) order[br * LF_MAX_DEG + j] = i;
+        }
+    }
+    delete dc;
+    return nbr;
+}
+
 static bool cw_possible(const lnsfaid_ctx* ctx) { return ctx->waves_per_cw != 2 && use_kernel4(ctx); }
 
 static bool packed_kernel(const lnsfaid_ctx* ctx) { return use_kernel4(ctx) && !use_kernel5(ctx); }
@@ -513,6 +580,10 @@
     if (use_kernel5(ctx)) {
         *threads = lf_decode5_threads();
         return lf_decode5_func(ctx->hcfg.method);
+    }
+    if (use_zero_shift(ctx)) {
+        *threads = lf_decode4_threads();
+        return lf_decode4z_func(ctx->hcfg.method);
     }
     if (use_kernel4(ctx)) {
         *threads = lf_decode4_threads();
@@ -684,6 +755,7 @@
             HIP_TRY(hipEventRecord(ctx->ev_chain[j], ctx->stream));
             if (packed) HIP_TRY(lf_launch_decode4p(ctx->hcfg.method, ctx->hcfg.ef, use_msg_registers(ctx) ? 1 : 0, &a, ctx->lds_bytes, ctx->stream));
             else if (use_kernel5(ctx)) HIP_TRY(lf_launch_decode5(ctx->hcfg.method, &a, ctx->lds_bytes, ctx->stream));
+            else if (use_zero_shift(ctx)) HIP_TRY(lf_launch_decode4z(ctx->hcfg.method, &a, ctx->lds_bytes, ctx->stream));
             else if (use_kernel4(ctx)) HIP_TRY(lf_launch_decode4(ctx->hcfg.method, ctx->hcfg.ef, use_msg_registers(ctx) ? 1 : 0, &a, ctx->lds_bytes, ctx->stream));
             else HIP_TRY(lf_launch_decode(ctx->hcfg.method, ctx->hcfg.uniform_w, &a, ctx->lds_bytes, ctx->stream));
             cur ^= 1;
@@ -973,7 +1045,7 @@
 
 static int comb_decode(lnsfaid_ctx* ctx, const int8_t* fixInput, int8_t* decodedBits, lnsfaid_group_stats* stats, int rule, int* rc_out)
 {
-    if (ctx->comb_slot < 0 || ctx->rows_per_lane != 0 || ctx->msg_store != 0 || ctx->waves_per_cw != 0) return 0;
+    if (ctx->comb_slot < 0 || ctx->rows_per_lane != 0 || ctx->msg_store != 0 || ctx->waves_per_cw != 0 || ctx->zero_shift != 0) return 0;
     LfCombiner* cb = ctx->comb;
     const int slot = ctx->comb_slot;
     {
diff --git a/mod-interleaveavx_multithreads-faid_amd/csrc/lnsfaid_device.h b/mod-interleaveavx_multithreads-faid_amd/csrc/lnsfaid_device.h
--- a/mod-interleaveavx_multithreads-faid_amd/csrc/lnsfaid_device.h
+++ b/mod-interleaveavx_multithreads-faid_amd/csrc/lnsfaid_device.h
@@ -37,6 +37,10 @@
     int32_t wcol[LF_MAX_BC];
     uint32_t era_edges[LF_MAX_BR];
     uint32_t colcirc[LF_MAX_BC][LF_MAX_COLW];
+    uint32_t zsbplain[LF_MAX_BR][32];
+    uint32_t zs4tab[LF_MAX_BR][LF_MAX_DEG];
+    uint32_t zcbtab[LF_MAX_BR][LF_MAX_DEG];
+    int32_t zinst[LF_MAX_BR];
 };
 
 struct LfDevCfg {
diff --git a/mod-interleaveavx_multithreads-faid_amd/csrc/lnsfaid_kernel4z.hip b/mod-interleaveavx_multithreads-faid_amd/csrc/lnsfaid_kernel4z.hip
--- /dev/null
+++ b/mod-interleaveavx_multithreads-faid_amd/csrc/lnsfaid_kernel4z.hip
@@ -0,0 +1,227 @@
+#include <hip/hip_runtime.h>
+
+#define LF4_MAIN_STEP main_step4z
+#include "lnsfaid_rows4.h"
+
+#ifdef LF4Z_SMALL_SET
+#define LF4Z_INSTANCES(X) X(0, 23, 0) X(1, 23, 4) X(2, 22, 5) X(3, 22, 0)
+#else
+#define LF4Z_INSTANCES(X) X(0, 23, 0) X(1, 23, 1) X(2, 23, 2) X(3, 23, 4) X(4, 22, 5) X(5, 22, 0)
+#endif
+
+extern "C" int lf_decode4z_inst(int deg, int zg)
+{
+    int best = -1, way = -1;
+#define LF4Z_ROUND(W, D, G) if (deg == (D) && (G) <= zg && (G) > best) { best = (G); way = (W); }
+    LF4Z_INSTANCES(LF4Z_ROUND)
+#undef LF4Z_ROUND
+    return (deg << 16) | ((best < 0 ? 0 : best) << 8) | (way < 0 ? 0 : 1 << way);
+}
+
+struct DevTab4Z {
+    CCode c;
+    int br;
+    uint32_t sbv;
+    __device__ __forceinline__ uint32_t s4(int j) const { return c->zs4tab[br][j]; }
+    __device__ __forceinline__ uint32_t cb256(int j) const { return c->zcbtab[br][j]; }
+    __device__ __forceinline__ uint32_t sb_dyn4(uint32_t idx4) const
+    {
+        return (uint32_t)__builtin_amdgcn_ds_bpermute((int)idx4, (int)sbv);
+    }
+};
+
+template <int METHOD, bool ERA, bool RM>
+__device__ __forceinline__ void main_step4z(CCode c, CCfg f, const LfDevCode* gc, SwRow* __restrict__ rows, SwRegs& R, int lane, int it, const uint32_t* sP,
+                                            bool have_par, bool lme, uint32_t era_plane)
+{
+    static_assert(RM && !ERA, "built for the messages-in-registers, non-erasing instances only");
+    (void)rows; (void)era_plane;
+    it = __builtin_amdgcn_readfirstlane(it);
+    const SwK K = sw_consts((uint32_t)it);
+    const bool fresh = (it == 1);
+    const int rem = f->max_iter - it;
+    const int itx = (it >= 1 && it <= 5) ? it - 1 : 5;
+    SwParams p;
+    p.lut_lo = f->lut_lo[itx][0]; p.lut_hi = f->lut_hi[itx][0];
+    p.ef_lo = f->lut_ef_lo[itx][0]; p.ef_hi = f->lut_ef_hi[itx][0];
+    p.f1 = f->factor_1; p.f2 = f->factor_2;
+    p.window = rem <= f->floor_iter_thresh;
+    p.ef_tables = f->ef >= 1;
+    if (LF4_OMS(METHOD)) sw_oms_tables(p);
+    const int nbr = c->nbr;
+    const SwLds lds = SwLds();
+    uint32_t tabv = gc->zsbplain[0][lane & 31];
+#pragma nounroll
+    for (int br = 0; br < nbr; ++br) {
+        const int brn = br + 1 < nbr ? br + 1 : 0;
+        const uint32_t tabn = gc->zsbplain[brn][lane & 31];
+        const int inst = c->zinst[br];
+        uint32_t rowpar = 0;
+        if (have_par) {
+#pragma unroll
+            for (int k = 0; k < 4; ++k) {
+                const uint32_t wv = sP[br * 8 + 2 * k + (lane >> 5)];
+                rowpar |= ((wv >> (lane & 31)) & 1u) ? (0xffu << (8 * k)) : 0u;
+            }
+        }
+        DevTab4Z tab;
+        tab.c = c; tab.br = br; tab.sbv = tabv;
+        const SwRow cur = regs_get(R, br);
+        SwRow st;
+#define LF4Z_WAY(W, D, G) if (inst & (1 << (W))) st = sw_layer_step<METHOD, D, false, 1, 0, G>(lds, tab, p, K, (uint32_t)lane, D, cur, fresh, rowpar, lme); else
+        LF4Z_INSTANCES(LF4Z_WAY)
+#undef LF4Z_WAY
+            st = sw_layer_step<METHOD, 0>(lds, tab, p, K, (uint32_t)lane, inst >> 16, cur, fresh, rowpar, lme);
+        __builtin_amdgcn_sched_barrier(0);
+        regs_put(R, br, st);
+        __builtin_amdgcn_sched_barrier(0);
+        tabv = tabn;
+    }
+}
+
+#define LF4_ON_FRONT prog >= kmax
+#define LF4_CLEAN_STOPS(t) prog >= kmax && !group_passed(a.live, g, prog, t)
+#define LF4_ON_STOP(t) if (RM && prog >= 2) regs_store(R, g_rows, c->nbr, t);
+#define LF4_ON_PASS(t) publish_pass(a.live, cw, prog, t);
+
+template <int METHOD>
+__global__ __launch_bounds__(LF_T4, 2) void lnsfaid_decode4z_kernel(LfKernelArgs a)
+{
+    constexpr bool RM = true, EF2 = false;
+    extern __shared__ __align__(16) unsigned char smem[];
+    CCode c = (CCode)a.code;
+    CCfg f = (CCfg)a.cfg;
+    const int tid = (int)threadIdx.x;
+    const int cw = (int)blockIdx.x;
+    const int N = c->n_var, M = c->n_check, K = c->k_info, nw = c->n_words, pw = c->p_words;
+    uint32_t* sHard0 = (uint32_t*)smem;
+    uint32_t* sHard2 = (uint32_t*)smem + nw;
+    uint32_t* sHard = (uint32_t*)(smem + lf_lds_off_hard(N));
+    uint32_t* sP = (uint32_t*)(smem + lf_lds_off_p(N, nw));
+    int* sStat = (int*)(smem + lf_lds_off_stat(N, nw, pw));
+    int* sRed = sStat + LNSFAID_GROUP;
+
+    const int max_iter = f->max_iter, max_bf = f->max_bf;
+    const int t_bf0 = max_iter + 1;
+    const int t_end = t_bf0 + max_bf;
+
+    const int g = cw >> 5, lane_in_group = cw & 31;
+    const int sv = a.status_cur ? a.status_cur[g * LNSFAID_GROUP + (tid & 31)] : 0;
+    const int my_status = __builtin_amdgcn_readlane(sv, lane_in_group);
+    if (my_status & LF_DONE) {
+        if (tid == 0) a.status_next[cw] = my_status;
+        return;
+    }
+    if (tid == LNSFAID_GROUP) sRed[LF_ZERO_SLOT] = 0;
+    int kmax;
+    {
+        int v = sv & LF_PROG_MASK;
+        v = imax(v, __builtin_amdgcn_update_dpp(0, v, 0x111, 0xf, 0xf, false));
+        v = imax(v, __builtin_amdgcn_update_dpp(0, v, 0x112, 0xf, 0xf, false));
+        v = imax(v, __builtin_amdgcn_update_dpp(0, v, 0x114, 0xf, 0xf, false));
+        v = imax(v, __builtin_amdgcn_update_dpp(0, v, 0x118, 0xf, 0xf, false));
+        v = imax(v, __builtin_amdgcn_update_dpp(0, v, 0x142, 0xa, 0xf, false));
+        kmax = __builtin_amdgcn_readlane(v, 31);
+    }
+    const int all_same = __ballot(sv != my_status) == 0ull;
+    LF_WG_SYNC();
+    int prog = my_status & LF_PROG_MASK;
+
+    uint32_t* g_en = (uint32_t*)(a.st_en + (size_t)cw * (size_t)N);
+    SwRow* g_rows = (SwRow*)(a.st_rows + (size_t)cw * (size_t)(c->nbr * LF_T));
+    uint32_t* g_bits = a.st_bits + (size_t)cw * (size_t)(3 * nw);
+    int8_t* g_out = a.decoded + (size_t)cw * (size_t)N;
+
+    if (prog != 0 && prog == kmax && !all_same) {
+        if (tid == 0) { a.status_next[cw] = my_status; atomicAdd(a.remaining, 1u); }
+        return;
+    }
+
+    if (my_status != 0 && all_same) {
+        if (tid == 0) {
+            a.status_next[cw] = my_status | LF_DONE;
+            if (a.stats && lane_in_group == 0) {
+                lnsfaid_group_stats st;
+                st.iterations = prog <= max_iter ? prog - 1 : max_iter;
+                st.bf_iterations = prog <= max_iter ? 0 : prog - t_bf0;
+                a.stats[g] = st;
+            }
+        }
+        return;
+    }
+
+    bool in_bf = max_bf > 0 && prog >= t_bf0 && prog != 0;
+    LfLaneState ls = { 0, 0, 0, 0 };
+    SwRegs R;
+    if (RM) regs_clear(R);
+
+    if (prog == 0) {
+        LF4_STAGE_INPUT()
+        LF_WG_SYNC();
+        prog = 1;
+    } else if (!in_bf) {
+        copy_in<23>((uint32_t*)smem, g_en, N >> 2, tid);
+        if (RM && prog >= 2) regs_load(R, g_rows, c->nbr, tid);
+        LF_WG_SYNC();
+    } else {
+        copy_in<9>(sHard, g_bits, nw, tid);
+        copy_in<9>(sHard0, g_bits + nw, nw, tid);
+        copy_in<9>(sHard2, g_bits + 2 * nw, nw, tid);
+        ls = a.st_lane[cw];
+        LF_WG_SYNC();
+    }
+
+    bool parked = false;
+    uint32_t pA = 0, pB = 0;
+    if (!in_bf) {
+        LF4_LAYERED_LOOP()
+        LF4_ENTER_BF()
+    }
+    LF4_BF_LOOPS()
+
+    const bool finished = prog >= t_end;
+    if (finished) {
+        if (!in_bf) build_plane4<false>(c, sHard, 0, tid);
+        write_decoded(sHard, g_out, N, tid);
+        if (tid == 0) {
+            a.status_next[cw] = prog | LF_DONE;
+            if (a.stats && lane_in_group == 0) {
+                lnsfaid_group_stats st;
+                st.iterations = prog <= max_iter ? prog - 1 : max_iter;
+                st.bf_iterations = prog <= max_iter ? 0 : prog - t_bf0;
+                a.stats[g] = st;
+            }
+        }
+    } else {
+        if (!in_bf) {
+            copy_out<23>(g_en, (const uint32_t*)smem, N >> 2, tid);
+        } else {
+            copy_out<9>(g_bits, sHard, nw, tid);
+            copy_out<9>(g_bits + nw, sHard0, nw, tid);
+            copy_out<9>(g_bits + 2 * nw, sHard2, nw, tid);
+            if (tid == 0) a.st_lane[cw] = ls;
+        }
+        write_decoded(sHard, g_out, N, tid);
+        if (tid == 0) { a.status_next[cw] = prog; atomicAdd(a.remaining, 1u); }
+    }
+}
+
+extern "C" const void* lf_decode4z_func(int method)
+{
+    switch (method) {
+    case 1: return (const void*)lnsfaid_decode4z_kernel<1>;
+    case 2: return (const void*)lnsfaid_decode4z_kernel<2>;
+    case 3: return (const void*)lnsfaid_decode4z_kernel<3>;
+    case 4: return (const void*)lnsfaid_decode4z_kernel<4>;
+    case 5: return (const void*)lnsfaid_decode4z_kernel<5>;
+    default: return nullptr;
+    }
+}
+
+extern "C" hipError_t lf_launch_decode4z(int method, const LfKernelArgs* args, size_t lds_bytes, hipStream_t stream)
+{
+    const void* fn = lf_decode4z_func(method);
+    if (!fn) return hipErrorInvalidValue;
+    void* kargs[] = { (void*)args };
+    return hipLaunchKernel(fn, dim3((unsigned)args->n_cw), dim3(LF_T4), kargs, lds_bytes, stream);
+}
diff --git a/mod-interleaveavx_multithreads-faid_amd/csrc/lnsfaid_rows4.h b/mod-interleaveavx_multithreads-faid_amd/csrc/lnsfaid_rows4.h
--- a/mod-interleaveavx_multithreads-faid_amd/csrc/lnsfaid_rows4.h
+++ b/mod-interleaveavx_multithreads-faid_amd/csrc/lnsfaid_rows4.h
@@ -303,6 +303,9 @@
     R.x0 = z; R.x1 = z; R.x2 = z; R.cw = z; R.pa0 = z; R.pa1 = z;
 }
 
+#ifndef LF4_MAIN_STEP
+#define LF4_MAIN_STEP main_step4
+#endif
 #define LF4_STAGE_INPUT() \
                                                  \
         const int8_t* gi = a.fix_input + (size_t)g * (size_t)LNSFAID_GROUP * (size_t)N;                                                                   \
@@ -361,7 +364,7 @@
             int tid_i = tid;                                                                                                                                                                             \
             asm volatile("" : "+v"(tid_i));                                                                                                                                                              \
             if (METHOD == 0) {                                                                                           \
-                main_step4<METHOD, false, RM>(c, f, a.code, g_rows, R, tid_i, prog, sP, false, false, 0u);                                                                                               \
+                LF4_MAIN_STEP<METHOD, false, RM>(c, f, a.code, g_rows, R, tid_i, prog, sP, false, false, 0u);                                                                                            \
                 prog++;                                                                                                                                                                                  \
                 continue;                                                                                                                                                                                \
             }                                                                                                                                                                                            \
@@ -395,9 +398,9 @@
             if (EF2 && f->ef == 2 && needs_checksums && have_par && lme) {                                                                                                                               \
                                                                                       \
                 build_erasure_plane4(c, a.code, sHard, sP, f->W, tid_i);                                                                                                                                 \
-                main_step4<METHOD, EF2, RM>(c, f, a.code, g_rows, R, tid_i, prog, sP, true, lme, lf_lds_off_hard(N));                                                                                    \
+                LF4_MAIN_STEP<METHOD, EF2, RM>(c, f, a.code, g_rows, R, tid_i, prog, sP, true, lme, lf_lds_off_hard(N));                                                                                 \
             } else {                                                                                                                                                                                     \
-                main_step4<METHOD, false, RM>(c, f, a.code, g_rows, R, tid_i, prog, sP, have_par && needs_checksums, lme, 0u);                                                                           \
+                LF4_MAIN_STEP<METHOD, false, RM>(c, f, a.code, g_rows, R, tid_i, prog, sP, have_par && needs_checksums, lme, 0u);                                                                        \
             }                                                                                                                                                                                            \
             prog++;                                                                                                                                                                                      \
         }                                                                                                                                                                                                \
diff --git a/mod-interleaveavx_multithreads-faid_amd/csrc/lnsfaid_swar.h b/mod-interleaveavx_multithreads-faid_amd/csrc/lnsfaid_swar.h
--- a/mod-interleaveavx_multithreads-faid_amd/csrc/lnsfaid_swar.h
+++ b/mod-interleaveavx_multithreads-faid_amd/csrc/lnsfaid_swar.h
@@ -387,12 +387,14 @@
 };
 #define SW_OWN(j) (WAVES == 1 || (((j) & 1) == WAVE))
 
-template <int METHOD, int DEG, bool ERA = false, int WAVES = 1, int WAVE = 0, class Tab, class Xch = SwNoXch>
+template <int METHOD, int DEG, bool ERA = false, int WAVES = 1, int WAVE = 0, int ZG = 0, class Tab, class Xch = SwNoXch>
 SW_FN SwRow sw_layer_step(const SwLds& lds, const Tab& tab, const SwParams& p, const SwK& K, uint32_t lane, int deg, SwRow cur, bool fresh,
                           uint32_t rowpar, bool lme, uint32_t era_edges = 0u, uint32_t era_plane = 0u, const Xch& xch = Xch())
 {
     static_assert(WAVES == 1 || !ERA, "the erasing variant is built for one wave per codeword only");
     static_assert(!ERA || METHOD == 2, "the erasure exists in Decode_FAID only");
+    static_assert(ZG == 0 || (DEG > 0 && WAVES == 1 && !ERA && SW_ILP * ZG <= DEG), "rotation-free groups: per-degree, one-wave, non-erasing instances");
+    constexpr int NZ = SW_ILP * ZG;
     constexpr int NJ = DEG > 0 ? DEG : SW_MAX_DEG;
     constexpr bool MINSUM = SW_MINSUM(METHOD);
     constexpr bool QUADS = WAVES == 1 && SW_ILP == 4 && DEG > 0;
@@ -432,7 +434,9 @@
 
 #pragma unroll
     for (int j = 0; j < NJ; ++j) {
-        if ((DEG > 0 || j < deg) && SW_OWN(j)) {
+        if (j < NZ) {
+            ad[j] = tid4 | cbj[j];
+        } else if ((DEG > 0 || j < deg) && SW_OWN(j)) {
             const uint32_t x4 = tid4 + s4j[j];
 #if SW_DEV
             uint32_t a;
@@ -451,11 +455,12 @@
     for (int j0 = 0; j0 < NJ; j0 += SW_ILP) {
         uint32_t r_[SW_ILP], x_[SW_ILP], s_[SW_ILP], k_[SW_ILP], a_[SW_ILP], i_[SW_ILP], u_[SW_ILP];
 #define SW_EDGES(...) _Pragma("unroll") for (int g = 0; g < SW_ILP; ++g) { const int j = j0 + g; if (j < NJ && (DEG > 0 || j < deg) && SW_OWN(j)) { __VA_ARGS__ } }
-        _Pragma("unroll") for (int g = SW_ILP - 1; g >= 0; --g) { const int j = j0 + g; if (j < NJ && (DEG > 0 || j < deg) && SW_OWN(j)) r_[g] = sw_alignbyte(ld[j], ld[j], rq[j]); }
+        _Pragma("unroll") for (int g = SW_ILP - 1; g >= 0; --g) { const int j = j0 + g; if (j < NJ && (DEG > 0 || j < deg) && SW_OWN(j)) r_[g] = j < NZ ? ld[j] : sw_alignbyte(ld[j], ld[j], rq[j]); }
         SW_EDGES(x_[g] = (j & 7) ? cur.x[j >> 3] >> (j & 7) : cur.x[j >> 3];)
         SW_EDGES(s_[g] = sw_bitop3<SW_TT_ANDOR>(x_[g], c01, c0642);)
         SW_EDGES(k_[g] = sw_perm(kt_hi, kt_lo, s_[g]);)
-        SW_EDGES(tb[j] = r_[g] + k_[g];)
+        if (j0 < NZ) { _Pragma("unroll") for (int g = SW_ILP - 1; g >= 0; --g) tb[j0 + g] = r_[g] + k_[g]; }
+        else { SW_EDGES(tb[j] = r_[g] + k_[g];) }
         if (ERA) {
             SW_EDGES(x_[g] &= c01;)
             SW_EDGES(
@@ -584,7 +589,7 @@
         SW_EDGES(mo[g] = sw_mask7(mo[g], sel_sign);)                                              \
         SW_EDGES(lm[g] = sw_upd2_limit<MINSUM>(ms[j], d_[g], u2, c80);)                                              \
         SW_EDGES(EN[g] = sw_upd2_en(mo[g], lm[g], zb[g], d_[g], cm27);)                                              \
-        SW_EDGES(EN[g] = sw_alignbyte(EN[g], EN[g], 4u - rq[j]);)                                                    \
+        SW_EDGES(if (j >= NZ) EN[g] = sw_alignbyte(EN[g], EN[g], 4u - rq[j]);)                                       \
         if (NSTREE) sw_sign_quad<NJ>(ns, ms, j0, deg, DEG > 0, K.c55, K.c33, K.c0f);                                 \
         else SW_EDGES(sw_sign_edge(ns, ms[j], j, cbit[j & 7]);)                                                      \
     }
diff --git a/mod-interleaveavx_multithreads-faid_amd/pyabi.py b/mod-interleaveavx_multithreads-faid_amd/pyabi.py
--- a/mod-interleaveavx_multithreads-faid_amd/pyabi.py
+++ b/mod-interleaveavx_multithreads-faid_amd/pyabi.py
@@ -6,6 +6,7 @@
 
 GROUP = 32
 MSG_REGISTERS, MSG_HBM = 1, 2
+ZERO_SHIFT_ON, ZERO_SHIFT_OFF = 1, 2
 STOP_GROUP, STOP_CODEWORD = 0, 1
 
 
@@ -111,6 +112,9 @@
     "lnsfaid_kernel_waves": (C.c_int, [C.c_void_p]),
     "lnsfaid_select_message_store": (C.c_int, [C.c_void_p, C.c_int32]),
     "lnsfaid_message_store": (C.c_int, [C.c_void_p]),
+    "lnsfaid_select_zero_shift": (C.c_int, [C.c_void_p, C.c_int32]),
+    "lnsfaid_zero_shift_groups": (C.c_int, [C.c_void_p, C.POINTER(C.c_int32), C.c_int32]),
+    "lnsfaid_code_zero_shift_order": (C.c_int, [C.POINTER(Code), C.POINTER(C.c_int32), C.POINTER(C.c_int32)]),
     "lnsfaid_kernel_residency": (C.c_int, [C.c_void_p, C.POINTER(C.c_int32), C.POINTER(C.c_int32)]),
     "lnsfaid_kernel_time": (C.c_int, [C.c_void_p, C.POINTER(C.c_double), C.POINTER(C.c_uint64), C.c_int32]),
     "lnsfaid_stream": (C.c_void_p, [C.c_void_p]),
@@ -167,6 +171,15 @@
         return self.code.n_var - self.code.n_check
 
 
+def code_zero_shift_order(code, lib=None):
+    lib = lib or load()
+    groups, order = (C.c_int32 * 32)(), (C.c_int32 * (32 * 24))()
+    nbr = lib.lnsfaid_code_zero_shift_order(C.byref(code), groups, order)
+    if nbr < 0:
+        raise ValueError("lnsfaid_code_zero_shift_order failed: %d" % nbr)
+    return list(groups[:nbr]), [[j for j in order[br * 24:br * 24 + 24] if j >= 0] for br in range(nbr)]
+
+
 def default_cfg(method, max_iter, lib=None):
     lib = lib or load()
     cfg = Cfg()
@@ -384,6 +397,15 @@
     def message_store(self):
         return self.lib.lnsfaid_message_store(self.ctx)
 
+    def select_zero_shift(self, mode):
+        self._check(self.lib.lnsfaid_select_zero_shift(self.ctx, mode), "lnsfaid_select_zero_shift")
+
+    def zero_shift_groups(self, n_layers=32):
+        zg = (C.c_int32 * n_layers)()
+        on = self.lib.lnsfaid_zero_shift_groups(self.ctx, zg, n_layers)
+        self._check(min(on, 0), "lnsfaid_zero_shift_groups")
+        return on == 1, list(zg)
+
     def kernel_residency(self):
         wg, lim = C.c_int32(), C.c_int32()
         self._check(self.lib.lnsfaid_kernel_residency(self.ctx, C.byref(wg), C.byref(lim)), "lnsfaid_kernel_residency")
```

Measured after the change: 77.58 (median of 6 runs). +3.1%, better.
